# Zhijian-Mei/py-debruijn

Hardware: AMD Instinct MI355X
Metric: k-mers/s hashed+graph-built at k=31 (higher is better)
Workload: dtype u64; 1 GPU; 10000000 x 150 bp synthetic reads (10000000 per GPU): BASELINE.json configs[1]; k=31, 30x coverage of a 50000000 bp uniform genome, 1% substitutions, seed 1; k=31, reads_per_gpu=10000000, reads_total=10000000, read_len=150, parallelism=single table

## Files before the change

### py-debruijn_amd/_dbg.py

```python
from __future__ import annotations

import ctypes as C
import os

import numpy as np

_HERE = os.path.dirname(os.path.abspath(__file__))
LIB_PATH = os.environ.get("DBG_LIB") or os.path.join(_HERE, "libdbg_hip.so")

DBG_OK, DBG_E_ARG, DBG_E_HIP, DBG_E_ALPHABET, DBG_E_CAPACITY, DBG_E_NOMEM = 0, -1, -2, -3, -4, -5
F_INDEG, F_KEEP_MASK, F_KEEP_SHIFT, F_BRANCH, F_PULLED = 0x01, 0x1E, 1, 0x20, 0x40
NO_NODE = 0xFFFFFFFF
ABI_VERSION = 6

SYMBOLS = (
    "dbg_create", "dbg_destroy", "dbg_last_error", "dbg_abi_version", "dbg_set_option", "dbg_set_reads", "dbg_set_reads_fasta",
    "dbg_set_reads_fasta_file", "dbg_fasta_ingest_stats", "dbg_set_reads_device",
    "dbg_synth_reads", "dbg_reads_checksum", "dbg_copy_reads", "dbg_reads_device", "dbg_build", "dbg_refine_edge_order", "dbg_export_orders",
    "dbg_get_alphabet", "dbg_export_keepmask", "dbg_export_dict_order",
    "dbg_prune", "dbg_remove_tips",
    "dbg_mark_pull_reads", "dbg_walk", "dbg_get_sizes", "dbg_get_stats", "dbg_get_counter", "dbg_export_nodes", "dbg_export_keys_hi",
    "dbg_export_succ",
    "dbg_export_csr", "dbg_export_pull_ranks", "dbg_export_pull_reads", "dbg_export_contigs",
    "dbg_export_contig_index", "dbg_export_contig_text", "dbg_device_views", "dbg_shard_extract", "dbg_shard_bucket_counts", "dbg_shard_record_layout", "dbg_shard_build", "dbg_shard_answer", "dbg_shard_apply",
    "dbg_import_graph", "dbg_device_keys_hi",
    "dbg_support_read_scores", "dbg_export_sorted_fasta", "dbg_build_multipass", "dbg_part_count", "dbg_part_sizes", "dbg_export_part", "dbg_part_device_views",
    "dbg_shard_build_multipass", "dbg_shard_build_multipass_from", "dbg_shard_extract_part", "dbg_part_queries", "dbg_part_answer", "dbg_part_apply", "dbg_multipass_finish",
    "dbg_export_marked", "dbg_part_keys_hi", "dbg_take_reads",
    "dbg_part_prune", "dbg_part_select", "dbg_part_gather", "dbg_part_mark", "dbg_part_clear", "dbg_part_cross_targets",
    "dbg_part_segments", "dbg_part_pflags", "dbg_scan_reads_for_keys", "dbg_set_orders", "dbg_part_segment_text",
    "dbg_build_from_walk", "dbg_build_from_walks",
    "dbg_lookup_nodes", "dbg_lookup_nodes_device", "dbg_gather_nodes", "dbg_score_sequences",
    "dbg_part_lookup_nodes", "dbg_part_lookup_nodes_device", "dbg_part_score_sequences",
    "dbg_export_contig_texts", "dbg_write_contigs_fasta", "dbg_contig_output_stats",
    "dbg_part_set_skeleton", "dbg_part_contig_window", "dbg_part_export_contig_texts", "dbg_part_write_contigs_fasta",
)


class Sizes(C.Structure):
    _fields_ = [("k", C.c_int32), ("abi_version", C.c_int32)] + [
        (n, C.c_uint64) for n in (
            "n_reads", "n_bytes", "n_kmer_instances", "n_edge_instances", "table_capacity", "n_nodes", "n_edges",
            "n_branch", "n_pulled", "n_pull_reads", "n_starts", "n_contigs", "contig_chars", "tip_rounds",
            "contigs_materialised", "max_degree")]

    def as_dict(self):
        return {n: getattr(self, n) for n, _ in self._fields_}


class Stats(C.Structure):
    _fields_ = [(n, C.c_double) for n in (
        "ms_startbits", "ms_table_init", "ms_count", "ms_compact", "ms_succ", "ms_csr", "ms_build_total", "ms_prune",
        "ms_tips", "ms_pull_reads", "ms_walk", "ms_h2d", "ms_extract", "ms_partition")] + [
        (n, C.c_uint64) for n in ("count_launches", "n_records", "n_buckets", "n_queries")]

    def as_dict(self):
        return {n: getattr(self, n) for n, _ in self._fields_}


class IngestStats(C.Structure):
    _fields_ = [(n, C.c_uint64) for n in (
        "bytes_read", "chunks", "chunk_bytes", "peak_device_bytes", "n_reads", "n_bases")] + [
        (n, C.c_double) for n in ("ms_total", "ms_io_wait", "ms_h2d", "ms_parse")]

    def as_dict(self):
        return {n: getattr(self, n) for n, _ in self._fields_}


class ContigOutStats(C.Structure):
    _fields_ = [(n, C.c_uint64) for n in (
        "bytes_written", "chunks", "chunk_bytes", "peak_device_bytes", "lift_bytes")] + [
        (n, C.c_double) for n in ("ms_total", "ms_io_wait", "ms_fill", "ms_d2h")]

    def as_dict(self):
        return {n: getattr(self, n) for n, _ in self._fields_}


class WalkBlock(C.Structure):
    _fields_ = [("src", C.c_void_p), ("contigs", C.c_void_p), ("n", C.c_uint64)]


COUNTERS = ("extract_presplit_fallbacks", "extract_presplit_rehists", "resolve_direct_hits", "resolve_keyed",
            "refine_crowded", "pull_crowded", "lookup_index_builds", "lookup_dir_calls", "lookup_index_calls",
            "part_lookup_calls")


class DbgError(RuntimeError):
    def __init__(self, code, msg):
        super().__init__(f"dbg error {code}: {msg}")
        self.code = code


class AlphabetError(DbgError, ValueError):
    pass


_lib = None


def load_library():
    global _lib
    if _lib is not None:
        return _lib
    if not os.path.exists(LIB_PATH):
        raise OSError(f"{LIB_PATH} not found: build it with py-debruijn_amd/csrc/build.sh "
                      f"(there is no CPU fallback for the device path)")
    try:
        import torch
    except ImportError:
        pass
    lib = C.CDLL(LIB_PATH)
    H = C.c_void_p
    u64p, u32p, u8p = C.POINTER(C.c_uint64), C.POINTER(C.c_uint32), C.POINTER(C.c_uint8)
    vp = C.c_void_p
    sig = {
        "dbg_create": (C.c_int, [C.c_int, C.POINTER(H)]),
        "dbg_destroy": (None, [H]),
        "dbg_last_error": (C.c_char_p, [H]),
        "dbg_abi_version": (C.c_int, []),
        "dbg_set_option": (C.c_int, [H, C.c_char_p, C.c_int64]),
        "dbg_set_reads": (C.c_int, [H, vp, vp, C.c_uint64]),
        "dbg_set_reads_fasta": (C.c_int, [H, vp, C.c_uint64]),
        "dbg_set_reads_fasta_file": (C.c_int, [H, C.c_char_p, C.c_uint64, C.c_uint64, C.c_uint64]),
        "dbg_fasta_ingest_stats": (C.c_int, [H, C.POINTER(IngestStats)]),
        "dbg_set_reads_device": (C.c_int, [H, vp, C.c_uint64, vp, C.c_uint64]),
        "dbg_synth_reads": (C.c_int, [H, C.c_uint64, C.c_uint64, C.c_uint64, C.c_uint64, C.c_uint32, C.c_uint32]),
        "dbg_reads_checksum": (C.c_int, [H, u64p]),
        "dbg_copy_reads": (C.c_int, [H, vp, vp]),
        "dbg_build": (C.c_int, [H, C.c_int, C.c_uint64]),
        "dbg_refine_edge_order": (C.c_int, [H]),
        "dbg_export_orders": (C.c_int, [H, vp, vp]),
        "dbg_get_alphabet": (C.c_int, [H, vp, C.POINTER(C.c_int), C.POINTER(C.c_int)]),
        "dbg_export_keepmask": (C.c_int, [H, vp]),
        "dbg_prune": (C.c_int, [H, C.c_double]),
        "dbg_remove_tips": (C.c_int, [H]),
        "dbg_mark_pull_reads": (C.c_int, [H]),
        "dbg_walk": (C.c_int, [H, C.c_int, C.c_uint64]),
        "dbg_get_sizes": (C.c_int, [H, C.POINTER(Sizes)]),
        "dbg_get_stats": (C.c_int, [H, C.POINTER(Stats)]),
        "dbg_get_counter": (C.c_int, [H, C.c_char_p, C.POINTER(C.c_uint64)]),
        "dbg_export_nodes": (C.c_int, [H, vp, vp, vp, vp]),
        "dbg_export_keys_hi": (C.c_int, [H, vp]),
        "dbg_export_dict_order": (C.c_int, [H, vp]),
        "dbg_export_succ": (C.c_int, [H, vp]),
        "dbg_export_csr": (C.c_int, [H, vp, vp, vp]),
        "dbg_export_pull_ranks": (C.c_int, [H, vp]),
        "dbg_export_pull_reads": (C.c_int, [H, vp]),
        "dbg_export_contigs": (C.c_int, [H, vp, vp, vp, vp, vp]),
        "dbg_export_contig_index": (C.c_int, [H, vp, vp, vp, vp]),
        "dbg_export_contig_text": (C.c_int, [H, C.c_uint64, vp, C.c_uint64]),
        "dbg_device_views": (C.c_int, [H] + [C.POINTER(vp)] * 5),
        "dbg_shard_extract": (C.c_int, [H, C.c_int, C.c_int, u64p, C.POINTER(vp), C.POINTER(vp), C.POINTER(vp)]),
        "dbg_shard_bucket_counts": (C.c_int, [H, u64p]),
        "dbg_shard_record_layout": (C.c_int, [H, C.POINTER(C.c_int), C.POINTER(C.c_int)]),
        "dbg_shard_build": (C.c_int, [H, C.c_int, C.c_int, C.c_int, vp, vp, vp, u64p, u64p, u64p, u64p, C.POINTER(vp), u64p, C.c_int]),
        "dbg_shard_answer": (C.c_int, [H, vp, C.c_uint64, vp]),
        "dbg_build_multipass": (C.c_int, [H, C.c_int, C.c_int]),
        "dbg_export_sorted_fasta": (C.c_int, [H, vp, vp, C.c_uint64, u64p]),
        "dbg_support_read_scores": (C.c_int, [H, vp, vp, C.c_uint64, vp, vp, vp, vp, C.c_uint64, vp, vp]),
        "dbg_part_count": (C.c_int, [H, C.POINTER(C.c_int)]),
        "dbg_shard_build_multipass": (C.c_int, [H, C.c_int, C.c_int, C.c_int, C.c_int, vp, vp, vp, C.c_int, u64p, u64p, u64p]),
        "dbg_shard_build_multipass_from": (C.c_int, [H, C.c_int, C.c_int, C.c_int, C.c_int, C.c_int, vp, vp, vp, C.c_int, u64p, u64p, u64p]),
        "dbg_shard_extract_part": (C.c_int, [H, C.c_int, C.c_int, C.c_int, C.c_int, u64p, C.POINTER(C.c_void_p), C.POINTER(C.c_void_p), C.POINTER(C.c_void_p)]),
        "dbg_part_queries": (C.c_int, [H, C.c_int, u64p, u64p, C.POINTER(vp)]),
        "dbg_part_answer": (C.c_int, [H, C.c_int, vp, C.c_uint64, vp]),
        "dbg_part_apply": (C.c_int, [H, C.c_int, C.c_int, vp]),
        "dbg_multipass_finish": (C.c_int, [H]),
# ... 825 lines not shown
```

### py-debruijn_amd/csrc/dbg_hip.hip

```cpp
#include <hip/hip_runtime.h>

#include <algorithm>
#include <chrono>
#include <cstdlib>
#include <cstdio>
#include <cstring>
#include <string>
#include <vector>

#include <cerrno>
#include <fcntl.h>
#include <sys/stat.h>
#include <unistd.h>

#include <rocprim/device/device_radix_sort.hpp>

#include "../../include/dbg.h"
#include "dbg_device.h"
#include "dbg_sk.h"
#include "dbg_sk2.h"
#include "dbg_sk3.h"
#include "dbg_wsk2.h"
#include "dbg_generic.h"
#include "dbg_genref.h"
#include "dbg_wide.h"
#include "dbg_support.h"
#include "dbg_wsk.h"
#include "dbg_fasta.h"
#include "dbg_lookup.h"
#include "dbg_ctgout.h"

using namespace dbgk;

enum MiscSlot {
    MISC_SEGMENTS,
    MISC_L1_CHILDREN,
    MISC_MS_SCPRE,
    MISC_MS_CMAT,
    MISC_MS_OFFS,
    MISC_BUCKETS,
    MISC_RANGES,
    MISC_QUERY_SEGS,
    MISC_ESTIMATE_SET,
    MISC_SLOTS
};

#ifndef DBG_L1_WIDE_FROM
#define DBG_L1_WIDE_FROM 20
#endif
#ifndef DBG_PS_WG_PER_CU
#define DBG_PS_WG_PER_CU DBG_EXW_WAVES
#endif
#ifndef DBG_EXTRACT_PRESPLIT
#define DBG_EXTRACT_PRESPLIT 4
#endif

struct dbg {
    int device = 0;
    hipStream_t stream = nullptr;
    std::string err;

    char *d_bases = nullptr;
    bool own_bases = false;
    uint64_t n_bytes = 0;
    uint64_t *d_offsets = nullptr;
    bool own_offsets = false;
    uint64_t n_reads = 0;
    uint32_t *d_startbits = nullptr;
    uint64_t startbits_words = 0;

    int k = 0;
    Slot *d_tab = nullptr;
    uint64_t cap = 0;
    int cap_log2 = 0;
    uint32_t *d_occ = nullptr;
    uint64_t *d_scalars = nullptr;
    uint64_t n_kmer_inst = 0, n_edge_inst = 0;
    uint64_t n_nodes = 0, n_edges = 0;
    uint64_t *d_keys = nullptr, *d_stamps = nullptr;
    uint64_t *d_keys_hi = nullptr;
    uint32_t *d_cnt = nullptr;
    uint8_t *d_flags = nullptr;
    uint8_t *d_order = nullptr;
    uint8_t *d_deg = nullptr;
    uint8_t *d_fsorder = nullptr;
    bool order_exact = false;
    uint32_t *d_succ = nullptr;
    bool nodes_in_arena = false;
    bool csr_built = false;
    uint64_t *d_rowptr = nullptr;
    uint32_t *d_col = nullptr, *d_ecnt = nullptr;
    bool dense_pending = false;
    uint32_t *d_rowptr32 = nullptr;
    void *d_stamps_st = nullptr;
    int stamps_st_bytes = 0;

    bool pruned = false, tipped = false;
    uint64_t n_branch = 0, n_pulled = 0, tip_rounds = 0;
    uint64_t *d_pull_rank = nullptr;

    uint8_t *d_read_flags = nullptr;
    uint64_t n_pull_reads = 0;
    bool pull_reads_done = false;

    uint64_t n_starts = 0, n_contigs = 0, contig_chars = 0;
    bool starts_known = false;
    struct { const uint64_t *w0 = nullptr, *w1 = nullptr; const void *st = nullptr; int st_bytes = 0;
             const uint64_t *b_start = nullptr, *b_cnt = nullptr; bool valid = false; } sk_src;
    uint64_t *d_ctg_off = nullptr;
    char *d_ctg_chars = nullptr;
    uint64_t *d_ctg_score = nullptr, *d_ctg_stamp = nullptr;
    uint32_t *d_ctg_seq = nullptr;
    uint32_t *d_ctg_start = nullptr;
    uint32_t *d_lift = nullptr;
    int lift_levels = 0;
    bool walked = false;
    bool walk_final = false;
    bool walk_indexed = false;
    bool walk_sizes_only = false;
    uint64_t walk_jump_min = 1ull << 14;

    int D = 4, sym_bits = 2, n_sym = 0;
    bool alpha_known = false, is_dna = true;
    uint8_t alphabet[32] = {0};
    uint8_t *d_lut = nullptr;
    char *d_alpha = nullptr;
    uint32_t *d_keepmask = nullptr;
    uint8_t *d_rank_mc = nullptr, *d_rank_fs = nullptr;

    int engine = 0;
    int bucket_bits = 0;
    int lds_slots = 4096;
    int phase_limit = 0;
    int est_scale_pct = 100;
    int wide_engine = 1;
    int count_kernel_u64 = 3;
    int stamp64 = 0;
    int resolve_sorted = 0;
    int resolve_direct = 1;
    int resolve_count = 0;
    uint64_t resolve_direct_hits = 0, resolve_keyed = 0;
    int wcount_kernel = 2;
    int count_kernel = 2;

    struct Buf {
        void *p = nullptr;
        uint64_t bytes = 0;
    };
    Buf ar_rec[2][3], ar_q[2][3], ar_node[8], ar_misc[MISC_SLOTS], ar_csr[4], ar_dir, ar_l2, ar_scan, ar_shard[6], ar_walk[3], ar_wide[6], ar_refine[4], ar_tips[4], ar_part[4][3] ;
    int sk_T = 0, sk_l1 = 0, sk_l2 = 0, sk_nb2 = 0 , sk_cap = 0;
    bool refine_streaming = false;
    int target_distinct = 0;
    int shard_stamp64 = 0;
    int extract_generic = 0;
    int extract_presplit = DBG_EXTRACT_PRESPLIT;
    uint64_t presplit_rehists = 0;
    uint64_t presplit_fallbacks = 0;
    uint64_t refine_crowded = 0, pull_crowded = 0;
    uint64_t sk_n_ranges = 0, sk_n_buckets = 0;
    SkGeom sk_geom{};
    void *shard_state = nullptr;
    void *multipass = nullptr;
    bool dropping_parts = false;
    dbg *spare_part = nullptr;
    bool wide_owner = false;
    bool borrowed_stream = false;
    bool arena_freed = false;
    std::vector<uint64_t> host_seg_cnt;
    std::vector<uint64_t> host_scpre;
    uint64_t shard_node_limit = 0;
    bool partial_graph = false;
    uint64_t *d_btab = nullptr;
    uint64_t btab_cap = 0;
    struct NkBlock {
        uint64_t n_src = 0, n_reads = 0;
        uint32_t *next = nullptr, *z = nullptr, *start = nullptr;
    };
    bool nk_graph = false;
    uint64_t nk_reads = 0, nk_bytes = 0;
    std::vector<NkBlock> nk_blocks;
    uint8_t *d_nk_read_flags = nullptr;

    bool dir_valid = false;
    int lookup_index = 0;
    Buf ar_lookup[3];
    bool lookup_built = false;
    uint64_t lookup_index_builds = 0, lookup_dir_calls = 0, lookup_index_calls = 0;
    bool part_dir_ok = false;
    uint64_t part_lookup_calls = 0;

    dbg_stats_t stats{};
    dbg_ingest_stats_t ingest{};
    dbg_contig_out_stats_t ctgout{};
    uint64_t ctgout_chunk = 0;
};

struct ShardState {
    int n_shards = 0, my_shard = 0, shard_bits = 0, k = 0;
    std::vector<uint64_t> q_start, q_cnt;
    uint64_t n_remote = 0;
    uint64_t n_kmer_inst_local = 0;
    std::vector<uint64_t> l1_counts;
    int rec_words = 1, rec_stamp_bytes = 4;
};
static ShardState &shard_of(dbg *h);
static void multipass_free(dbg *h);
static void drop_spare_part(dbg *h);

static int buf_ensure(dbg *h, dbg::Buf &b, uint64_t bytes) {
    if (bytes == 0) bytes = 16;
    if (b.bytes >= bytes) return DBG_OK;
    if (b.p) { (void)hipFreeAsync(b.p, h->stream); h->arena_freed = true; }
    b.p = nullptr;
    b.bytes = 0;
    static const bool trace = getenv("DBG_TRACE_ALLOC") != nullptr;
    const auto t_alloc = std::chrono::steady_clock::now();
    hipError_t e = hipMallocAsync(&b.p, bytes, h->stream);
    if (trace) {
        const double ms = std::chrono::duration<double, std::milli>(std::chrono::steady_clock::now() - t_alloc).count();
        if (ms > 5.0) fprintf(stderr, "[dbg] hipMallocAsync(%.3f GB) took %.1f ms (buffer %p of handle %p)\n", bytes / 1e9, ms, (void *)&b, (void *)h);
    }
    if (e != hipSuccess) {
        (void)hipGetLastError();
        (void)hipStreamSynchronize(h->stream);
        hipMemPool_t pool;
        if (hipDeviceGetDefaultMemPool(&pool, h->device) == hipSuccess) (void)hipMemPoolTrimTo(pool, 0);
        e = hipMallocAsync(&b.p, bytes, h->stream);
    }
    if (e != hipSuccess) {
        (void)hipGetLastError();
        h->err = std::string("hipMallocAsync(") + std::to_string(bytes) + "): " + hipGetErrorString(e);
        b.p = nullptr;
        return DBG_E_NOMEM;
    }
    b.bytes = bytes;
    return DBG_OK;
}
static void buf_free(dbg *h, dbg::Buf &b) {
    if (b.p) { (void)hipFreeAsync(b.p, h->stream); h->arena_freed = true; }
    b.p = nullptr;
    b.bytes = 0;
}
static void pool_trim(dbg *h) {
    if (!h->arena_freed) return;
    (void)hipStreamSynchronize(h->stream);
    hipMemPool_t pool;
    if (hipDeviceGetDefaultMemPool(&pool, h->device) == hipSuccess) (void)hipMemPoolTrimTo(pool, 0);
    (void)hipGetLastError();
    h->arena_freed = false;
}

#define HIPCHK(h, call)                                                                      \
    do {                                                                                     \
        hipError_t e_ = (call);                                                              \
        if (e_ != hipSuccess) {                                                              \
            (h)->err = std::string(#call) + ": " + hipGetErrorString(e_);                    \
            return e_ == hipErrorOutOfMemory ? DBG_E_NOMEM : DBG_E_HIP;                      \
        }                                                                                    \
    } while (0)

#define CHK(expr)                 \
    do {                          \
        int rc_ = (expr);         \
        if (rc_ != DBG_OK) return rc_; \
    } while (0)

template <class T>
static int dev_alloc(dbg *h, T **p, uint64_t count) {
    *p = nullptr;
    if (count == 0) count = 1;
    HIPCHK(h, hipMalloc((void **)p, count * sizeof(T)));
    return DBG_OK;
}
template <class T>
static void dev_free(T *&p) {
    if (p) (void)hipFree(p);
    p = nullptr;
}

static inline unsigned grid_for(uint64_t n, unsigned block) { return (unsigned)((n + block - 1) / block); }

struct Timer {
    hipEvent_t a = nullptr, b = nullptr;
    hipStream_t s;
    explicit Timer(hipStream_t st) : s(st) {
        (void)hipEventCreate(&a);
        (void)hipEventCreate(&b);
        (void)hipEventRecord(a, s);
    }
    double stop() {
        (void)hipEventRecord(b, s);
        (void)hipEventSynchronize(b);
        float ms = 0;
        (void)hipEventElapsedTime(&ms, a, b);
        return ms;
    }
    ~Timer() {
        (void)hipEventDestroy(a);
        (void)hipEventDestroy(b);
    }
};

constexpr int SCAN_ITEMS = 16;
constexpr int SCAN_TILE = 256 * SCAN_ITEMS;

template <class F>
__global__ __launch_bounds__(256) void k_scan_reduce(uint64_t n, F f, uint64_t *partial) {
    uint64_t base = (uint64_t)blockIdx.x * SCAN_TILE + (uint64_t)threadIdx.x * SCAN_ITEMS;
    uint64_t s = 0;
#pragma unroll
    for (int i = 0; i < SCAN_ITEMS; ++i)
        if (base + i < n) s += f(base + i);
    uint64_t tot;
    (void)block_exscan_256(s, &tot);
    if (threadIdx.x == 0) partial[blockIdx.x] = tot;
}

__global__ __launch_bounds__(256) void k_scan_partials(uint64_t *partial, uint64_t nblk, uint64_t *total) {
    uint64_t carry = 0;
    for (uint64_t base = 0; base < nblk; base += 256) {
        uint64_t i = base + threadIdx.x;
        uint64_t v = i < nblk ? partial[i] : 0;
        uint64_t tot;
        uint64_t ex = block_exscan_256(v, &tot);
        if (i < nblk) partial[i] = carry + ex;
        carry += tot;
    }
    if (threadIdx.x == 0) *total = carry;
}

template <class F, class OutT>
__global__ __launch_bounds__(256) void k_scan_write(uint64_t n, F f, const uint64_t *partial, OutT *out) {
    uint64_t base = (uint64_t)blockIdx.x * SCAN_TILE + (uint64_t)threadIdx.x * SCAN_ITEMS;
    uint64_t v[SCAN_ITEMS];
    uint64_t s = 0;
#pragma unroll
    for (int i = 0; i < SCAN_ITEMS; ++i) {
        v[i] = (base + i < n) ? f(base + i) : 0;
        s += v[i];
    }
    uint64_t tot;
    uint64_t run = partial[blockIdx.x] + block_exscan_256(s, &tot);
#pragma unroll
    for (int i = 0; i < SCAN_ITEMS; ++i) {
        if (base + i < n) out[base + i] = (OutT)run;
        run += v[i];
    }
}

template <class F, class OutT>
static int exclusive_scan(dbg *h, uint64_t n, F f, OutT *out, uint64_t *h_total) {
    uint64_t nblk = (n + SCAN_TILE - 1) / SCAN_TILE;
    if (nblk == 0) nblk = 1;
    CHK(buf_ensure(h, h->ar_scan, (nblk + 1) * 8));
    uint64_t *partial = (uint64_t *)h->ar_scan.p;
    uint64_t *d_total = partial + nblk;
    hipLaunchKernelGGL(HIP_KERNEL_NAME(k_scan_reduce<F>), dim3((unsigned)nblk), dim3(256), 0, h->stream, n, f, partial);
    hipLaunchKernelGGL(k_scan_partials, dim3(1), dim3(256), 0, h->stream, partial, nblk, d_total);
    hipLaunchKernelGGL(HIP_KERNEL_NAME(k_scan_write<F, OutT>), dim3((unsigned)nblk), dim3(256), 0, h->stream, n, f,
                       partial, out);
    if (!h_total) return DBG_OK;
    hipError_t e = hipMemcpyAsync(h_total, d_total, 8, hipMemcpyDeviceToHost, h->stream);
    if (e == hipSuccess) e = hipStreamSynchronize(h->stream);
    if (e != hipSuccess) {
        h->err = std::string("exclusive_scan: ") + hipGetErrorString(e);
        return DBG_E_HIP;
    }
    return DBG_OK;
}

template <class F>
static int reduce_sum(dbg *h, uint64_t n, F f, uint64_t *h_total) {
    uint64_t nblk = (n + SCAN_TILE - 1) / SCAN_TILE;
    if (nblk == 0) nblk = 1;
    CHK(buf_ensure(h, h->ar_scan, (nblk + 1) * 8));
    uint64_t *partial = (uint64_t *)h->ar_scan.p;
    hipLaunchKernelGGL(HIP_KERNEL_NAME(k_scan_reduce<F>), dim3((unsigned)nblk), dim3(256), 0, h->stream, n, f, partial);
    hipLaunchKernelGGL(k_scan_partials, dim3(1), dim3(256), 0, h->stream, partial, nblk, partial + nblk);
    hipError_t e = hipMemcpyAsync(h_total, partial + nblk, 8, hipMemcpyDeviceToHost, h->stream);
    if (e == hipSuccess) e = hipStreamSynchronize(h->stream);
    if (e != hipSuccess) {
        h->err = std::string("reduce_sum: ") + hipGetErrorString(e);
        return DBG_E_HIP;
    }
    return DBG_OK;
}

struct OccBytes32 {
    const uint8_t *occ;
    __device__ uint64_t operator()(uint64_t w) const {
        const uint4 a = reinterpret_cast<const uint4 *>(occ)[2 * w], b = reinterpret_cast<const uint4 *>(occ)[2 * w + 1];
        return __popc(a.x) + __popc(a.y) + __popc(a.z) + __popc(a.w) + __popc(b.x) + __popc(b.y) + __popc(b.z) + __popc(b.w);
    }
};
struct PopcWords {
    const uint32_t *w;
    __device__ uint64_t operator()(uint64_t i) const { return __popc(w[i]); }
};
struct DegOf {
    const uint8_t *deg;
    __device__ uint64_t operator()(uint64_t i) const { return deg[i]; }
};
struct U64At {
    const uint64_t *p;
    __device__ uint64_t operator()(uint64_t i) const { return p[i]; }
};
struct KmerInstances {
    const uint64_t *off;
    uint64_t k;
    __device__ uint64_t operator()(uint64_t i) const { const uint64_t len = off[i + 1] - off[i]; return len >= k ? len - k + 1 : 0; }
};
struct WRecLenAt {
    const uint64_t *w1;
    __device__ uint64_t operator()(uint64_t i) const { return (uint64_t)wrec_len(w1[i]); }
};
struct WRecSuccAt {
    const uint64_t *w1;
    __device__ uint64_t operator()(uint64_t i) const { return (uint64_t)wrec_has_succ(w1[i]); }
};
struct FlagSet {
    const uint8_t *f;
    uint8_t mask, want;
    __device__ uint64_t operator()(uint64_t i) const { return (f[i] & mask) == want; }
};

__device__ inline uint64_t synth_draw(uint64_t key, uint64_t ctr) { return mix64(key ^ (ctr * 0xD6E8FEB86659FD93ull)); }

__global__ __launch_bounds__(256) void k_synth(char *bases, uint64_t *offsets, uint64_t kg, uint64_t ks, uint64_t ke,
                                               uint64_t genome_len, uint64_t first_read, uint64_t n_reads,
                                               uint32_t read_len, uint32_t err_thr) {
    const uint64_t total = n_reads * read_len;
    for (uint64_t i = (uint64_t)blockIdx.x * blockDim.x + threadIdx.x; i < total; i += (uint64_t)gridDim.x * blockDim.x) {
        const uint64_t r = i / read_len, j = i - r * read_len, gr = first_read + r;
        const uint64_t start = synth_draw(ks, gr) % (genome_len - read_len + 1);
        uint32_t code = (uint32_t)(synth_draw(kg, start + j) & 3);
        if (err_thr) {
            const uint64_t e = synth_draw(ke, gr * read_len + j);
            if ((uint32_t)(e & 0xFFFFFFu) < err_thr) code = (code + 1 + (uint32_t)((e >> 24) % 3)) & 3;
        }
        bases[i] = "ACGT"[code];
        if (j == 0) offsets[r] = i;
    }
    if (blockIdx.x == 0 && threadIdx.x == 0) offsets[n_reads] = total;
}
// ... 1008 lines not shown
    h->d_rowptr32 = nullptr; h->d_stamps_st = nullptr; h->stamps_st_bytes = 0;
    h->dense_pending = false;
    h->csr_built = false;
    h->d_pull_rank = nullptr;
    dev_free(h->d_read_flags);
    dev_free(h->d_ctg_off); dev_free(h->d_ctg_chars); dev_free(h->d_ctg_score); dev_free(h->d_ctg_stamp);
    dev_free(h->d_ctg_seq); dev_free(h->d_ctg_start); dev_free(h->d_lift);
    h->lift_levels = 0;
    h->partial_graph = false;
    h->sk_src.valid = false;
    h->k = 0; h->cap = 0; h->n_nodes = h->n_edges = 0;
    h->pruned = h->tipped = h->pull_reads_done = h->walked = h->walk_indexed = h->walk_sizes_only = false;
    h->n_branch = h->n_pulled = h->tip_rounds = h->n_pull_reads = 0;
    h->n_starts = h->n_contigs = h->contig_chars = 0;
    h->starts_known = false;
    h->n_kmer_inst = h->n_edge_inst = 0;
    for (auto &b : h->nk_blocks) { dev_free(b.next); dev_free(b.z); dev_free(b.start); }
    h->nk_blocks.clear();
    dev_free(h->d_nk_read_flags);
    h->nk_graph = false;
    h->nk_reads = h->nk_bytes = 0;
}

static void free_reads(dbg *h) {
    if (h->own_bases) dev_free(h->d_bases);
    if (h->own_offsets) dev_free(h->d_offsets);
    h->d_bases = nullptr; h->d_offsets = nullptr;
    h->own_bases = h->own_offsets = false;
    dev_free(h->d_startbits);
    dev_free(h->d_lut); dev_free(h->d_alpha);
    h->alpha_known = false;
    h->n_bytes = h->n_reads = 0;
}

extern "C" int dbg_abi_version(void) { return DBG_ABI_VERSION; }

extern "C" int dbg_create(int device, dbg_t **out) {
    if (!out) return DBG_E_ARG;
    *out = nullptr;
    int n = 0;
    if (hipGetDeviceCount(&n) != hipSuccess || device < 0 || device >= n) return DBG_E_HIP;
    dbg *h = new (std::nothrow) dbg();
    if (!h) return DBG_E_NOMEM;
    h->device = device;
    if (hipSetDevice(device) != hipSuccess || hipStreamCreate(&h->stream) != hipSuccess ||
        hipMalloc((void **)&h->d_scalars, 128 * sizeof(uint64_t)) != hipSuccess) {
        delete h;
        return DBG_E_HIP;
    }
    {
        hipMemPool_t pool;
        if (hipDeviceGetDefaultMemPool(&pool, device) == hipSuccess) {
            uint64_t keep = ~0ull;
            (void)hipMemPoolSetAttribute(pool, hipMemPoolAttrReleaseThreshold, &keep);
        }
        (void)hipGetLastError();
    }
    *out = h;
    return DBG_OK;
}

extern "C" void dbg_destroy(dbg_t *h) {
    if (!h) return;
    (void)hipSetDevice(h->device);
    (void)hipStreamSynchronize(h->stream);
    h->dropping_parts = true;
    free_build(h);
    if (h->spare_part) { dbg_destroy(h->spare_part); h->spare_part = nullptr; }
    free_reads(h);
    for (auto &lvl : h->ar_rec) for (auto &b : lvl) buf_free(h, b);
    for (auto &lvl : h->ar_q) for (auto &b : lvl) buf_free(h, b);
    for (auto &b : h->ar_node) buf_free(h, b);
    for (auto &b : h->ar_misc) buf_free(h, b);
    for (auto &b : h->ar_csr) buf_free(h, b);
    buf_free(h, h->ar_dir);
    buf_free(h, h->ar_l2);
    for (auto &b : h->ar_shard) buf_free(h, b);
    for (auto &b : h->ar_walk) buf_free(h, b);
    for (auto &b : h->ar_wide) buf_free(h, b);
    for (auto &b : h->ar_refine) buf_free(h, b);
    for (auto &b : h->ar_tips) buf_free(h, b);
    for (auto &lvl : h->ar_part) for (auto &b : lvl) buf_free(h, b);
    buf_free(h, h->ar_scan);
    dev_free(h->d_scalars);
    delete (ShardState *)h->shard_state;
    (void)hipStreamSynchronize(h->stream);
    if (!h->borrowed_stream) (void)hipStreamDestroy(h->stream);
    delete h;
}

extern "C" const char *dbg_last_error(const dbg_t *h) { return h ? h->err.c_str() : "null handle"; }

static int make_startbits(dbg *h) {
    Timer t(h->stream);
    dev_free(h->d_startbits);
    h->startbits_words = (h->n_bytes + 1 + 31) / 32 + SB_WORDS + 2;
    CHK(dev_alloc(h, &h->d_startbits, h->startbits_words));
    HIPCHK(h, hipMemsetAsync(h->d_startbits, 0, h->startbits_words * 4, h->stream));
    hipLaunchKernelGGL(k_startbits, dim3(grid_for(h->n_reads + 1, 256)), dim3(256), 0, h->stream, h->d_offsets,
                       h->n_reads, h->d_startbits);
    HIPCHK(h, hipGetLastError());
    h->stats.ms_startbits = t.stop();
    return DBG_OK;
}

extern "C" int dbg_set_reads(dbg_t *h, const char *bases, const uint64_t *offsets, uint64_t n_reads) {
    if (!h || !offsets || (n_reads && !bases && offsets[n_reads] != 0)) return DBG_E_ARG;
    HIPCHK(h, hipSetDevice(h->device));
    if (offsets[0] != 0) { h->err = "offsets[0] must be 0"; return DBG_E_ARG; }
    for (uint64_t i = 0; i < n_reads; ++i)
        if (offsets[i + 1] < offsets[i]) { h->err = "offsets must be non-decreasing"; return DBG_E_ARG; }
    free_build(h);
    free_reads(h);
    const uint64_t nb = offsets[n_reads];
    Timer t(h->stream);
    CHK(dev_alloc(h, &h->d_bases, nb + 64));
    h->own_bases = true;
    CHK(dev_alloc(h, &h->d_offsets, n_reads + 1));
    h->own_offsets = true;
    if (nb) HIPCHK(h, hipMemcpyAsync(h->d_bases, bases, nb, hipMemcpyHostToDevice, h->stream));
    HIPCHK(h, hipMemcpyAsync(h->d_offsets, offsets, (n_reads + 1) * 8, hipMemcpyHostToDevice, h->stream));
    h->stats.ms_h2d = t.stop();
    h->n_bytes = nb;
    h->n_reads = n_reads;
    return make_startbits(h);
}

extern "C" int dbg_set_reads_fasta(dbg_t *h, const char *text, uint64_t n_text) {
    if (!h || (n_text && !text)) return DBG_E_ARG;
    HIPCHK(h, hipSetDevice(h->device));
    free_build(h);
    free_reads(h);
    char *d_text = nullptr;
    uint32_t *bits = nullptr, *word_rank = nullptr, *len = nullptr;
    uint64_t *line_start = nullptr, *read_idx = nullptr, *byte_off = nullptr;
    uint8_t *is_read = nullptr;
    auto cleanup = [&]() {
        dev_free(d_text); dev_free(bits); dev_free(word_rank); dev_free(len); dev_free(line_start); dev_free(read_idx);
        dev_free(byte_off); dev_free(is_read);
    };
    int rc = DBG_OK;
    uint64_t n_lines = 0, n_reads = 0, n_bases = 0;
    do {
        Timer t(h->stream);
        if ((rc = dev_alloc(h, &d_text, n_text + 64)) != DBG_OK) break;
        if (n_text && hipMemcpyAsync(d_text, text, n_text, hipMemcpyHostToDevice, h->stream) != hipSuccess) { h->err = "H2D copy failed"; rc = DBG_E_HIP; break; }
        h->stats.ms_h2d = t.stop();
        const uint64_t n_words = (n_text + 31) / 32;
        if ((rc = dev_alloc(h, &bits, n_words)) != DBG_OK) break;
        if ((rc = dev_alloc(h, &word_rank, n_words)) != DBG_OK) break;
        if (n_words) {
            hipLaunchKernelGGL(k_fa_mark, dim3(grid_for(n_words, 256)), dim3(256), 0, h->stream, d_text, n_text, bits);
            if ((rc = exclusive_scan(h, n_words, PopcWords{bits}, word_rank, &n_lines)) != DBG_OK) break;
        }
        if ((rc = dev_alloc(h, &line_start, n_lines)) != DBG_OK) break;
        if ((rc = dev_alloc(h, &is_read, n_lines)) != DBG_OK) break;
        if ((rc = dev_alloc(h, &len, n_lines)) != DBG_OK) break;
        if ((rc = dev_alloc(h, &read_idx, n_lines)) != DBG_OK) break;
        if ((rc = dev_alloc(h, &byte_off, n_lines)) != DBG_OK) break;
        if (n_lines) {
            hipLaunchKernelGGL(k_fa_line_starts, dim3(grid_for(n_words, 256)), dim3(256), 0, h->stream, bits, word_rank, n_words,
                               line_start);
            hipLaunchKernelGGL(k_fa_lines, dim3(grid_for(n_lines, 256)), dim3(256), 0, h->stream, d_text, n_text, line_start,
                               n_lines, is_read, len);
            if ((rc = exclusive_scan(h, n_lines, ByteSet{is_read}, read_idx, &n_reads)) != DBG_OK) break;
            if ((rc = exclusive_scan(h, n_lines, U32At{len}, byte_off, &n_bases)) != DBG_OK) break;
        }
        if ((rc = dev_alloc(h, &h->d_bases, n_bases + 64)) != DBG_OK) break;
        h->own_bases = true;
// ... 601 lines not shown
    unsigned long long *estamp = nullptr;
    auto cleanup = [&]() { dev_free(nodes); dev_free(edges); dev_free(occ); dev_free(eocc); dev_free(word_rank); dev_free(estamp); };
    int rc = DBG_OK;
    do {
        if ((rc = dev_alloc(h, &nodes, cap)) != DBG_OK) break;
        if ((rc = dev_alloc(h, &edges, cap)) != DBG_OK) break;
        if ((rc = dev_alloc(h, &occ, cap / 32)) != DBG_OK) break;
        if ((rc = dev_alloc(h, &eocc, cap / 32)) != DBG_OK) break;
        (void)hipMemsetAsync(occ, 0, cap / 8, h->stream);
        (void)hipMemsetAsync(eocc, 0, cap / 8, h->stream);
        (void)hipMemsetAsync(h->d_scalars, 0, 64 * 8, h->stream);
        hipLaunchKernelGGL(k_g_init_tables, dim3(grid_for(cap, 256)), dim3(256), 0, h->stream, nodes, edges, cap);
        if (h->n_bytes) {
            const unsigned grid = (unsigned)std::min<uint64_t>((h->n_bytes + 255) / 256, 1u << 16);
            hipLaunchKernelGGL(k_g_insert, dim3(grid), dim3(256), 0, h->stream, h->d_bases, h->n_bytes, h->d_startbits, k,
                               h->d_lut, nodes, occ, edges, eocc, cap - 1, (unsigned long long *)h->d_scalars);
        }
        uint64_t sc[4] = {0, 0, 0, 0};
        if (hipMemcpyAsync(sc, h->d_scalars, 32, hipMemcpyDeviceToHost, h->stream) != hipSuccess ||
            hipStreamSynchronize(h->stream) != hipSuccess) { h->err = "generic count failed"; rc = DBG_E_HIP; break; }
        if (sc[0] & STATUS_TABLE_FULL) { h->err = "generic engine: hash table full"; rc = DBG_E_CAPACITY; break; }
        h->n_kmer_inst = sc[1];
        h->n_edge_inst = sc[2];
        h->stats.ms_count = t_count.stop();
        h->stats.count_launches = 1;
        Timer t_c(h->stream);
        const uint64_t n_words = cap / 32;
        if ((rc = dev_alloc(h, &word_rank, n_words)) != DBG_OK) break;
        uint64_t n = 0;
        if ((rc = exclusive_scan(h, n_words, PopcWords{occ}, word_rank, &n)) != DBG_OK) break;
        h->n_nodes = n;
        if ((rc = dev_alloc(h, &h->d_keys, n)) != DBG_OK) break;
        if ((rc = dev_alloc(h, &h->d_stamps, n)) != DBG_OK) break;
        if ((rc = dev_alloc(h, &h->d_flags, n)) != DBG_OK) break;
        if ((rc = dev_alloc(h, &h->d_cnt, n * GEN_D)) != DBG_OK) break;
        if ((rc = dev_alloc(h, &h->d_succ, n * GEN_D)) != DBG_OK) break;
        if ((rc = dev_alloc(h, &h->d_deg, n)) != DBG_OK) break;
        if ((rc = dev_alloc(h, &h->d_keepmask, n)) != DBG_OK) break;
        if ((rc = dev_alloc(h, &h->d_rank_mc, n * GEN_D)) != DBG_OK) break;
        if ((rc = dev_alloc(h, &h->d_rank_fs, n * GEN_D)) != DBG_OK) break;
        if ((rc = dev_alloc(h, &estamp, n * GEN_D)) != DBG_OK) break;
        if (n) {
            (void)hipMemsetAsync(h->d_cnt, 0, n * GEN_D * 4, h->stream);
            (void)hipMemsetAsync(h->d_succ, 0xFF, n * GEN_D * 4, h->stream);
            (void)hipMemsetAsync(estamp, 0xFF, n * GEN_D * 8, h->stream);
            (void)hipMemsetAsync(h->d_keepmask, 0, n * 4, h->stream);
            hipLaunchKernelGGL(k_g_gather, dim3(grid_for(n_words, 256)), dim3(256), 0, h->stream, nodes, occ, word_rank, n_words,
                               h->d_keys, h->d_stamps, h->d_flags);
            hipLaunchKernelGGL(k_g_edges, dim3(grid_for(cap, 256)), dim3(256), 0, h->stream, edges, cap, nodes, cap - 1, k,
                               h->d_cnt, h->d_succ, estamp, (unsigned long long *)h->d_scalars);
            hipLaunchKernelGGL(k_g_rank, dim3(grid_for(n, 256)), dim3(256), 0, h->stream, n, h->d_cnt, estamp, h->d_rank_mc,
                               h->d_rank_fs, h->d_deg);
        }
        if (hipMemcpyAsync(sc, h->d_scalars, 8, hipMemcpyDeviceToHost, h->stream) != hipSuccess ||
            hipStreamSynchronize(h->stream) != hipSuccess) { h->err = "generic graph assembly failed"; rc = DBG_E_HIP; break; }
        if (sc[0] & STATUS_SUCC_MISSING) { h->err = "internal: edge endpoint missing from the node table"; rc = DBG_E_HIP; break; }
        h->stats.ms_succ = t_c.stop();
        h->order_exact = true;
    } while (0);
    cleanup();
    return rc;
}

extern "C" int dbg_set_option(dbg_t *h, const char *name, int64_t value) {
    if (!h || !name) return DBG_E_ARG;
    const std::string n(name);
    if (n == "engine" && (value == 0 || value == 1)) { h->engine = (int)value; return DBG_OK; }
    if (n == "bucket_bits" && value >= 0 && value <= SK_BUCKET_BITS) { h->bucket_bits = (int)value; return DBG_OK; }
    if (n == "lds_slots" && (value == 2048 || value == 4096)) { h->lds_slots = (int)value; return DBG_OK; }
    if (n == "phase_limit" && value >= 0 && value <= 5) { h->phase_limit = (int)value; return DBG_OK; }
    if (n == "estimate_scale_pct" && value >= 1 && value <= 1000) { h->est_scale_pct = (int)value; return DBG_OK; }
    if (n == "target_distinct" && value >= 0 && value <= 4096) { h->target_distinct = (int)value; return DBG_OK; }
    if (n == "shard_stamp64" && (value == 0 || value == 1)) { h->shard_stamp64 = (int)value; return DBG_OK; }
    if (n == "extract_generic" && (value == 0 || value == 1)) { h->extract_generic = (int)value; return DBG_OK; }
    if (n == "extract_presplit" && value >= 0 && value <= SK_PS_MAX_F0) { h->extract_presplit = (int)value; return DBG_OK; }
    if (n == "refine_streaming" && (value == 0 || value == 1)) { h->refine_streaming = value != 0; return DBG_OK; }
    if (n == "walk_jump_min_nodes" && value >= 0) { h->walk_jump_min = (uint64_t)value; return DBG_OK; }
    if (n == "wide_engine" && (value == 0 || value == 1)) { h->wide_engine = (int)value; return DBG_OK; }
    if (n == "count_kernel" && value >= 1 && value <= 3) { h->count_kernel = (int)value; return DBG_OK; }
    if (n == "stamp64" && (value == 0 || value == 1)) { h->stamp64 = (int)value; return DBG_OK; }
    if (n == "resolve_sorted" && value >= 0 && value <= 2) { h->resolve_sorted = (int)value; return DBG_OK; }
    if (n == "resolve_direct" && (value == 0 || value == 1)) { h->resolve_direct = (int)value; return DBG_OK; }
    if (n == "resolve_count" && (value == 0 || value == 1)) { h->resolve_count = (int)value; return DBG_OK; }
    if (n == "wcount_kernel" && (value == 1 || value == 2)) { h->wcount_kernel = (int)value; return DBG_OK; }
    if (n == "count_kernel_u64" && value >= 1 && value <= 3) { h->count_kernel_u64 = (int)value; return DBG_OK; }
    if (n == "lookup_index" && (value == 0 || value == 1)) { h->lookup_index = (int)value; return DBG_OK; }
    if (n == "ctgout_chunk_bytes" && value >= 0 && dbgk::co_chunk_ok((uint64_t)value)) { h->ctgout_chunk = (uint64_t)value; return DBG_OK; }
    if (n == "shard_node_limit" && value >= 0 && value < (1ll << 29)) { h->shard_node_limit = (uint64_t)value; return DBG_OK; }
    h->err = "unknown option or value out of range: " + n;
    return DBG_E_ARG;
}

static int build_wide_once(dbg *h, int k, uint64_t table_capacity_hint, bool packed, bool *overflow) {
    if (h->n_bytes >= (1ull << 43)) { h->err = "reads too large for the 44-bit positions of the table's protocol word"; return DBG_E_CAPACITY; }
    uint64_t want = table_capacity_hint;
    if (!want) {
        uint64_t inst = 0;
        CHK(reduce_sum(h, h->n_reads, KmerInstances{h->d_offsets, (uint64_t)k}, &inst));
        want = (uint64_t)((double)(inst + 1) / 0.7);
    }
    const uint64_t cap = std::max<uint64_t>(1024, (want + 1023) / 1024 * 1024);
    const uint64_t pk_words = (h->n_bytes + 31) / 32, n_occ = cap / 32;
    uint64_t *pk = nullptr;
    WSlot *tab = nullptr;
    uint32_t *tcnt = nullptr, *word_rank = nullptr;
    uint8_t *occ = nullptr;
    auto cleanup = [&]() {};
    int rc = DBG_OK;
    uint64_t sc[4] = {0, 0, 0, 0};
    do {
        Timer t(h->stream);
        if ((rc = buf_ensure(h, h->ar_wide[0], (pk_words + 3) * 8)) != DBG_OK) break;
        if ((rc = buf_ensure(h, h->ar_wide[1], cap * sizeof(WSlot))) != DBG_OK) break;
        if (!packed && (rc = buf_ensure(h, h->ar_wide[2], cap * 16)) != DBG_OK) break;
        if ((rc = buf_ensure(h, h->ar_wide[3], cap)) != DBG_OK) break;
        if ((rc = buf_ensure(h, h->ar_wide[4], n_occ * 4)) != DBG_OK) break;
        pk = (uint64_t *)h->ar_wide[0].p;
        tab = (WSlot *)h->ar_wide[1].p;
        tcnt = packed ? nullptr : (uint32_t *)h->ar_wide[2].p;
        occ = (uint8_t *)h->ar_wide[3].p;
        word_rank = (uint32_t *)h->ar_wide[4].p;
        (void)hipMemsetAsync(pk + pk_words, 0, 3 * 8, h->stream);
        hipLaunchKernelGGL(k_wtab_init, dim3(grid_for(cap, 256)), dim3(256), 0, h->stream, tab, cap);
        if (tcnt) (void)hipMemsetAsync(tcnt, 0, cap * 16, h->stream);
        (void)hipMemsetAsync(occ, 0, cap, h->stream);
        (void)hipMemsetAsync(h->d_scalars, 0, 64 * 8, h->stream);
        if (pk_words)
            hipLaunchKernelGGL(k_wpack, dim3(grid_for(pk_words, 256)), dim3(256), 0, h->stream, h->d_bases, h->n_bytes,
                               pk_words, pk);
        h->stats.ms_table_init = t.stop();
        Timer tc(h->stream);
        const uint64_t tiles = (h->n_bytes + TILE - 1) / TILE;
        if (tiles)
            hipLaunchKernelGGL(k_wcount, dim3((unsigned)tiles), dim3(256), 0, h->stream, h->d_bases, h->n_bytes,
                               h->d_startbits, k, pk, tab, tcnt, cap, occ, (unsigned long long *)h->d_scalars);
        h->stats.count_launches = tiles ? 1 : 0;
        hipError_t e = hipMemcpyAsync(sc, h->d_scalars, 32, hipMemcpyDeviceToHost, h->stream);
        h->stats.ms_count = tc.stop();
        if (e != hipSuccess || hipGetLastError() != hipSuccess) { h->err = "k_wcount failed"; rc = DBG_E_HIP; break; }
        if (sc[0] & STATUS_BAD_BASE) { h->err = "reads hold a byte outside ACGT"; rc = DBG_E_ALPHABET; break; }
        if (sc[0] & STATUS_TABLE_FULL) { h->err = "hash table capacity exceeded"; rc = DBG_E_CAPACITY; break; }
        if (sc[0] & STATUS_WIDE_COUNTER16) { *overflow = true; rc = DBG_E_CAPACITY; h->err = "successor counter overflow"; break; }
        h->n_kmer_inst = sc[1];
        h->n_edge_inst = sc[2];

        Timer tg(h->stream);
        uint64_t total = 0;
        if ((rc = exclusive_scan(h, n_occ, OccBytes32{occ}, word_rank, &total)) != DBG_OK) break;
        if (total >= 0xFFFFFFFFull) { h->err = "more than 2^32-1 nodes"; rc = DBG_E_CAPACITY; break; }
        h->n_nodes = total;
        if ((rc = buf_ensure(h, h->ar_node[0], total * 8)) != DBG_OK) break;
        if ((rc = buf_ensure(h, h->ar_node[1], total * 8)) != DBG_OK) break;
        if ((rc = buf_ensure(h, h->ar_node[2], total * 16)) != DBG_OK) break;
        if ((rc = buf_ensure(h, h->ar_node[3], total)) != DBG_OK) break;
        if ((rc = buf_ensure(h, h->ar_node[4], total)) != DBG_OK) break;
        if ((rc = buf_ensure(h, h->ar_node[5], total * 16)) != DBG_OK) break;
        if ((rc = buf_ensure(h, h->ar_node[6], total)) != DBG_OK) break;
        if ((rc = buf_ensure(h, h->ar_wide[5], total * 8)) != DBG_OK) break;
        h->d_keys = (uint64_t *)h->ar_node[0].p;
        h->d_stamps = (uint64_t *)h->ar_node[1].p;
        h->d_cnt = (uint32_t *)h->ar_node[2].p;
        h->d_flags = (uint8_t *)h->ar_node[3].p;
        h->d_order = (uint8_t *)h->ar_node[4].p;
        h->d_succ = (uint32_t *)h->ar_node[5].p;
        h->d_deg = (uint8_t *)h->ar_node[6].p;
        h->d_keys_hi = (uint64_t *)h->ar_wide[5].p;
        h->nodes_in_arena = true;
        hipLaunchKernelGGL(k_wgather, dim3(grid_for(n_occ * 32, 256)), dim3(256), 0, h->stream, tab, tcnt, occ, word_rank, n_occ,
                           h->d_keys, h->d_keys_hi, h->d_stamps, h->d_cnt, h->d_flags, 1);
        h->stats.ms_compact = tg.stop();
        Timer ts(h->stream);
        if (total)
            hipLaunchKernelGGL(k_wsucc, dim3(grid_for(total, 256)), dim3(256), 0, h->stream, tab, cap, k, total,
                               h->d_keys, h->d_keys_hi, h->d_cnt, h->d_succ, h->d_order, h->d_deg);
        e = hipStreamSynchronize(h->stream);
        h->stats.ms_succ = ts.stop();
        if (e != hipSuccess || hipGetLastError() != hipSuccess) { h->err = std::string("wide build: ") + hipGetErrorString(e); rc = DBG_E_HIP; break; }
    } while (false);
    cleanup();
    return rc;
}

static int build_wide(dbg *h, int k, uint64_t table_capacity_hint) {
    bool overflow = false;
    int rc = build_wide_once(h, k, table_capacity_hint, true, &overflow);
    if (rc != DBG_OK && overflow) {
        rc = build_wide_once(h, k, table_capacity_hint, false, &overflow);
        if (rc == DBG_OK) h->err.clear();
    }
    return rc;
}

extern "C" int dbg_build(dbg_t *h, int k, uint64_t table_capacity_hint) {
    if (!h) return DBG_E_ARG;
    if (k < 1 || k > 63) { h->err = "k must be in 1..63 (k-mers of at most two 64-bit words)"; return DBG_E_ARG; }
    if (!h->d_offsets) { h->err = "no reads set"; return DBG_E_ARG; }
    HIPCHK(h, hipSetDevice(h->device));
    h->dropping_parts = true;
    free_build(h);
    h->dropping_parts = false;
    drop_spare_part(h);
    h->k = k;
    h->stats = dbg_stats_t{};
    const bool tentative = !h->alpha_known && h->engine == 0 && h->n_bytes > 0;
    if (tentative) h->is_dna = true;
    else CHK(compute_alphabet(h));
    if (tentative) {
        Timer t_total(h->stream);
        int rc;
        bool lds_engine = true;
        if (k > 31) {
            bool fallback = true;
            rc = h->wide_engine == 1 ? build_wsk(h, k, &fallback) : DBG_E_CAPACITY;
            if (fallback && rc != DBG_E_ALPHABET) {
                lds_engine = false;
                free_build(h);
                h->k = k;
                h->stats = dbg_stats_t{};
                CHK(compute_alphabet(h));
                rc = h->is_dna ? build_wide(h, k, table_capacity_hint) : DBG_E_ALPHABET;
            }
        } else {
            rc = build_sk(h, k, table_capacity_hint);
        }
        if (rc == DBG_OK) {
            rc = finish_graph(h);
            if (rc != DBG_OK) { const std::string keep = h->err; free_build(h); h->err = keep; return rc; }
            h->alpha_known = true;
            h->is_dna = true;
            h->dir_valid = lds_engine;
            h->stats.ms_build_total = t_total.stop();
            if (k <= 31) pool_trim(h);
            return DBG_OK;
        }
        if (rc != DBG_E_ALPHABET) { const std::string keep = h->err; free_build(h); h->err = keep; return rc; }
        free_build(h);
        h->k = k;
        h->stats = dbg_stats_t{};
        h->err.clear();
        CHK(compute_alphabet(h));
        if (h->is_dna) { h->err = "internal: the extraction refused reads the alphabet scan calls ACGT"; return DBG_E_HIP; }
    }
    if (!h->is_dna) {
        Timer t_total(h->stream);
        int rc = build_generic(h, k);
        if (rc == DBG_OK) rc = finish_graph(h);
        if (rc != DBG_OK) { const std::string keep = h->err; free_build(h); h->err = keep; return rc; }
        h->stats.ms_build_total = t_total.stop();
        return DBG_OK;
    }
    if (k > 31) {
        Timer t_total(h->stream);
        int rc;
        bool fallback = true;
        if (h->wide_engine == 1 && h->engine == 0) rc = build_wsk(h, k, &fallback);
        if (fallback) {
            free_build(h);
            h->k = k;
            h->stats = dbg_stats_t{};
            rc = build_wide(h, k, table_capacity_hint);
        }
        if (rc == DBG_OK) rc = finish_graph(h);
        if (rc != DBG_OK) { const std::string keep = h->err; free_build(h); h->err = keep; return rc; }
        h->dir_valid = !fallback;
        h->stats.ms_build_total = t_total.stop();
        return DBG_OK;
    }
    if (h->engine == 0) {
        Timer t_total(h->stream);
        int rc = build_sk(h, k, table_capacity_hint);
        if (rc == DBG_OK) rc = finish_graph(h);
        if (rc != DBG_OK) { const std::string keep = h->err; free_build(h); h->err = keep; return rc; }
        h->dir_valid = true;
        h->stats.ms_build_total = t_total.stop();
        pool_trim(h);
        return DBG_OK;
    }
    Timer t_total(h->stream);

    uint64_t want = table_capacity_hint ? table_capacity_hint : (uint64_t)((double)(h->n_bytes + 1) / 0.7);
    uint64_t cap = 1024;
    int lg = 10;
    while (cap < want) { cap <<= 1; ++lg; }
    h->cap = cap;
    h->cap_log2 = lg;
    {
        Timer t(h->stream);
        CHK(dev_alloc(h, &h->d_tab, cap));
        CHK(dev_alloc(h, &h->d_occ, cap / 32));
        HIPCHK(h, hipMemsetAsync(h->d_occ, 0, cap / 8, h->stream));
        HIPCHK(h, hipMemsetAsync(h->d_scalars, 0, 64 * 8, h->stream));
        hipLaunchKernelGGL(k_table_init, dim3(grid_for(cap, 256)), dim3(256), 0, h->stream, h->d_tab, cap);
        HIPCHK(h, hipGetLastError());
        h->stats.ms_table_init = t.stop();
    }
    uint64_t sc[4] = {0, 0, 0, 0};
    {
        Timer t(h->stream);
        const uint64_t tiles = (h->n_bytes + TILE - 1) / TILE;
        if (tiles) {
            hipLaunchKernelGGL(k_count, dim3((unsigned)tiles), dim3(256), 0, h->stream, h->d_bases, h->n_bytes,
                               h->d_startbits, k, h->d_tab, cap - 1, 64 - lg, h->d_occ,
                               (unsigned long long *)h->d_scalars);
            HIPCHK(h, hipGetLastError());
        }
        h->stats.count_launches = tiles ? 1 : 0;
        HIPCHK(h, hipMemcpyAsync(sc, h->d_scalars, 32, hipMemcpyDeviceToHost, h->stream));
        h->stats.ms_count = t.stop();
    }
    if (sc[0] & STATUS_BAD_BASE) { h->err = "reads hold a byte outside ACGT"; free_build(h); return DBG_E_ALPHABET; }
    if (sc[0] & STATUS_TABLE_FULL) { h->err = "hash table capacity exceeded"; free_build(h); return DBG_E_CAPACITY; }
    h->n_kmer_inst = sc[1];
    h->n_edge_inst = sc[2];

    {
        Timer t(h->stream);
        uint32_t *word_rank = nullptr;
        const uint64_t n_words = cap / 32;
        CHK(dev_alloc(h, &word_rank, n_words));
        uint64_t total = 0;
        int rc = exclusive_scan(h, n_words, PopcWords{h->d_occ}, word_rank, &total);
        if (rc != DBG_OK) { (void)hipFree(word_rank); return rc; }
        if (total >= 0xFFFFFFFFull) { (void)hipFree(word_rank); h->err = "more than 2^32-1 nodes"; return DBG_E_CAPACITY; }
        h->n_nodes = total;
        CHK(dev_alloc(h, &h->d_keys, total));
        CHK(dev_alloc(h, &h->d_stamps, total));
        CHK(dev_alloc(h, &h->d_cnt, total * 4));
        CHK(dev_alloc(h, &h->d_flags, total));
        CHK(dev_alloc(h, &h->d_order, total));
        CHK(dev_alloc(h, &h->d_succ, total * 4));
        CHK(dev_alloc(h, &h->d_deg, total));
        hipLaunchKernelGGL(k_gather, dim3(grid_for(n_words, 256)), dim3(256), 0, h->stream, h->d_tab, h->d_occ,
                           word_rank, n_words, h->d_keys, h->d_stamps, h->d_cnt, h->d_flags);
        HIPCHK(h, hipGetLastError());
        h->stats.ms_compact = t.stop();
        (void)hipFree(word_rank);
    }
    {
        Timer t(h->stream);
        if (h->n_nodes) {
            hipLaunchKernelGGL(k_succ, dim3(grid_for(h->n_nodes, 256)), dim3(256), 0, h->stream, h->d_tab, cap - 1,
                               64 - lg, k, h->n_nodes, h->d_keys, h->d_cnt, h->d_succ, h->d_order, h->d_deg);
            HIPCHK(h, hipGetLastError());
        }
        h->stats.ms_succ = t.stop();
    }
    CHK(finish_graph(h));
    h->stats.ms_build_total = t_total.stop();
    return DBG_OK;
}

extern "C" int dbg_refine_edge_order(dbg_t *h) {
    if (!h || !h->k) return DBG_E_ARG;
    if (h->partial_graph) { h->err = kPartialGraph; return DBG_E_ARG; }
    HIPCHK(h, hipSetDevice(h->device));
    CHK(ensure_dense(h));
    if (h->D == GEN_D) return DBG_OK;
// ... 539 lines not shown
            h->walk_indexed = true;
            if (n_chr > max_chars) break;
            const uint64_t longest = h->n_nodes + (uint64_t)h->k;
            int levels = 1;
            while ((1ull << levels) <= longest) ++levels;
            if (n_ctg && (uint64_t)levels * h->n_nodes * 4 <= (8ull << 30)) {
                if ((rc = dev_alloc(h, &h->d_ctg_chars, n_chr)) != DBG_OK) break;
                if ((rc = dev_alloc(h, &lift, (uint64_t)levels * h->n_nodes)) != DBG_OK) break;
                const dim3 ngrid(grid_for(h->n_nodes, 256));
                hipLaunchKernelGGL(HIP_KERNEL_NAME(k_lift_init<G>), ngrid, dim3(256), 0, h->stream, h->n_nodes, g, lift);
                for (int l = 1; l < levels; ++l)
                    hipLaunchKernelGGL(k_lift_step, ngrid, dim3(256), 0, h->stream, h->n_nodes, lift + (uint64_t)(l - 1) * h->n_nodes,
                                       lift + (uint64_t)l * h->n_nodes);
                hipLaunchKernelGGL(HIP_KERNEL_NAME(k_text_fill<G>), dim3(grid_for(n_chr, 256)), dim3(256), 0, h->stream, n_chr, g,
                                   h->d_ctg_off, n_ctg, ctg_start, lift, h->n_nodes, levels, h->d_ctg_chars);
                text_done = true;
            }
        }
        if (!text_done) {
            if ((rc = dev_alloc(h, &h->d_ctg_chars, n_chr)) != DBG_OK) break;
            launch(1);
        }
        if (hipGetLastError() != hipSuccess) { h->err = "walk pass 1 launch failed"; rc = DBG_E_HIP; break; }
        hipError_t e = hipStreamSynchronize(h->stream);
        if (e != hipSuccess) { h->err = std::string("walk: ") + hipGetErrorString(e); rc = DBG_E_HIP; break; }
        h->walked = true;
        h->walk_indexed = true;
    } while (0);
    cleanup();
    h->stats.ms_walk = t.stop();
    return rc;
}

extern "C" int dbg_walk(dbg_t *h, int final_mode, uint64_t max_chars) {
    if (!h || !h->pruned) { if (h) h->err = "dbg_prune must run first"; return DBG_E_ARG; }
    HIPCHK(h, hipSetDevice(h->device));
    if (h->D == GEN_D) return walk_impl(h, gen_view(h), final_mode, max_chars);
    return walk_impl(h, dna_view(h), final_mode, max_chars);
}

extern "C" int dbg_get_sizes(dbg_t *h, dbg_sizes_t *o) {
    if (!h || !o) return DBG_E_ARG;
    if (h->k && h->n_nodes && !h->starts_known) {
        HIPCHK(h, hipSetDevice(h->device));
        CHK(ensure_starts(h));
    }
    memset(o, 0, sizeof(*o));
    o->k = h->k;
    o->abi_version = DBG_ABI_VERSION;
    o->n_reads = h->n_reads + h->nk_reads;
    o->n_bytes = h->n_bytes + h->nk_bytes;
    o->n_kmer_instances = h->n_kmer_inst;
    o->n_edge_instances = h->n_edge_inst;
    o->table_capacity = h->cap;
    o->n_nodes = h->n_nodes;
    o->n_edges = h->n_edges;
    o->n_branch = h->n_branch;
    o->n_pulled = h->n_pulled;
    o->n_pull_reads = h->n_pull_reads;
    o->n_starts = h->n_starts;
    o->n_contigs = h->n_contigs;
    o->contig_chars = h->contig_chars;
    o->tip_rounds = h->tip_rounds;
    o->contigs_materialised = h->walked ? 1 : 0;
    o->max_degree = (uint64_t)h->D;
    return DBG_OK;
}

extern "C" int dbg_get_stats(dbg_t *h, dbg_stats_t *o) {
    if (!h || !o) return DBG_E_ARG;
    *o = h->stats;
    return DBG_OK;
}

extern "C" int dbg_get_counter(dbg_t *h, const char *name, uint64_t *out) {
    if (!h || !name || !out) return DBG_E_ARG;
    const std::string n(name);
    if (n == "extract_presplit_rehists") { *out = h->presplit_rehists; return DBG_OK; }
    if (n == "extract_presplit_fallbacks") { *out = h->presplit_fallbacks; return DBG_OK; }
    if (n == "refine_crowded") { *out = h->refine_crowded; return DBG_OK; }
    if (n == "pull_crowded") { *out = h->pull_crowded; return DBG_OK; }
    if (n == "resolve_direct_hits") { *out = h->resolve_direct_hits; return DBG_OK; }
    if (n == "resolve_keyed") { *out = h->resolve_keyed; return DBG_OK; }
    if (n == "lookup_index_builds") { *out = h->lookup_index_builds; return DBG_OK; }
    if (n == "lookup_dir_calls") { *out = h->lookup_dir_calls; return DBG_OK; }
    if (n == "lookup_index_calls") { *out = h->lookup_index_calls; return DBG_OK; }
    if (n == "part_lookup_calls") { *out = h->part_lookup_calls; return DBG_OK; }
    h->err = "unknown counter: " + n;
    return DBG_E_ARG;
}

#define D2H(h, dst, src, bytes)                                                                       do {                                                                                                  if ((dst) && (bytes)) HIPCHK(h, hipMemcpyAsync((dst), (src), (bytes), hipMemcpyDeviceToHost, (h)->stream));     } while (0)

extern "C" int dbg_export_nodes(dbg_t *h, uint64_t *keys, uint64_t *stamps, uint32_t *counts, uint8_t *flags) {
    if (!h || !h->k) return DBG_E_ARG;
    HIPCHK(h, hipSetDevice(h->device));
    CHK(ensure_dense(h));
    if (keys && !h->d_keys) memset(keys, 0, h->n_nodes * 8);
    else D2H(h, keys, h->d_keys, h->n_nodes * 8);
    D2H(h, stamps, h->d_stamps, h->n_nodes * 8);
    D2H(h, counts, h->d_cnt, h->n_nodes * 4 * h->D);
    D2H(h, flags, h->d_flags, h->n_nodes);
    HIPCHK(h, hipStreamSynchronize(h->stream));
    return DBG_OK;
}

extern "C" int dbg_export_keys_hi(dbg_t *h, uint64_t *keys_hi) {
    if (!h || !h->k || !keys_hi) return DBG_E_ARG;
    HIPCHK(h, hipSetDevice(h->device));
    if (!h->d_keys_hi) {
        memset(keys_hi, 0, h->n_nodes * 8);
        return DBG_OK;
    }
    D2H(h, keys_hi, h->d_keys_hi, h->n_nodes * 8);
    HIPCHK(h, hipStreamSynchronize(h->stream));
    return DBG_OK;
}

extern "C" int dbg_export_succ(dbg_t *h, uint32_t *succ) {
    if (!h || !h->k) return DBG_E_ARG;
    HIPCHK(h, hipSetDevice(h->device));
    CHK(ensure_dense(h));
    D2H(h, succ, h->d_succ, h->n_nodes * 4 * h->D);
    HIPCHK(h, hipStreamSynchronize(h->stream));
    return DBG_OK;
}

extern "C" int dbg_export_csr(dbg_t *h, uint64_t *row_ptr, uint32_t *col, uint32_t *cnt) {
    if (!h || !h->k) return DBG_E_ARG;
    HIPCHK(h, hipSetDevice(h->device));
    CHK(ensure_dense(h));
    D2H(h, row_ptr, h->d_rowptr, (h->n_nodes + 1) * 8);
    D2H(h, col, h->d_col, h->n_edges * 4);
    D2H(h, cnt, h->d_ecnt, h->n_edges * 4);
    HIPCHK(h, hipStreamSynchronize(h->stream));
    return DBG_OK;
}

extern "C" int dbg_export_pull_ranks(dbg_t *h, uint64_t *ranks) {
    if (!h || !h->tipped) { if (h) h->err = "dbg_remove_tips must run first"; return DBG_E_ARG; }
    HIPCHK(h, hipSetDevice(h->device));
    D2H(h, ranks, h->d_pull_rank, h->n_nodes * 8);
    HIPCHK(h, hipStreamSynchronize(h->stream));
    return DBG_OK;
}

extern "C" int dbg_export_pull_reads(dbg_t *h, uint8_t *read_flags) {
    if (!h || !h->pull_reads_done) { if (h) h->err = "dbg_mark_pull_reads must run first"; return DBG_E_ARG; }
    HIPCHK(h, hipSetDevice(h->device));
    if (h->nk_graph) {
        D2H(h, read_flags, h->d_nk_read_flags, h->nk_reads);
        if (read_flags) read_flags += h->nk_reads;
    }
    D2H(h, read_flags, h->d_read_flags, h->n_reads);
    HIPCHK(h, hipStreamSynchronize(h->stream));
    return DBG_OK;
}

extern "C" int dbg_export_contig_index(dbg_t *h, uint64_t *offsets, uint64_t *scores, uint64_t *start_stamp,
                                       uint32_t *seq_in_start) {
    if (!h || !h->walk_indexed) { if (h) h->err = "dbg_walk must run first"; return DBG_E_ARG; }
    HIPCHK(h, hipSetDevice(h->device));
    D2H(h, offsets, h->d_ctg_off, (h->n_contigs + 1) * 8);
    D2H(h, scores, h->d_ctg_score, h->n_contigs * 8);
    D2H(h, start_stamp, h->d_ctg_stamp, h->n_contigs * 8);
    D2H(h, seq_in_start, h->d_ctg_seq, h->n_contigs * 4);
// ... 274 lines not shown
        auto dev = [&](int i) -> void * { return outs[i].host ? (void *)(blk + outs[i].at) : nullptr; };
        LkGatherArgs a{h->d_keys, h->d_keys_hi, h->d_stamps, h->d_cnt, h->d_flags, gen ? h->d_keepmask : nullptr,
                       gen ? h->d_rank_mc : h->d_order, gen ? h->d_rank_fs : h->d_fsorder,
                       (uint64_t *)dev(0), (uint64_t *)dev(1), (uint64_t *)dev(2), (uint32_t *)dev(3), (uint8_t *)dev(5),
                       (uint32_t *)dev(4), (uint8_t *)dev(6), (uint8_t *)dev(7), h->n_nodes, h->D};
        hipLaunchKernelGGL(k_gather_nodes, dim3(grid_for(n, 256)), dim3(256), 0, h->stream, a, (const uint32_t *)(blk + 16), n,
                           (unsigned long long *)blk);
        unsigned long long bad = 0;
        e = hipGetLastError();
        if (e == hipSuccess) e = hipMemcpyAsync(&bad, blk, 8, hipMemcpyDeviceToHost, h->stream);
        if (e == hipSuccess) e = hipStreamSynchronize(h->stream);
        if (e != hipSuccess) { h->err = std::string("dbg_gather_nodes: ") + hipGetErrorString(e); rc = DBG_E_HIP; break; }
        if (bad) { h->err = "dbg_gather_nodes: a node id is not below n_nodes"; rc = DBG_E_ARG; break; }
        for (auto &o : outs)
            if (o.host && e == hipSuccess) e = hipMemcpyAsync(o.host, blk + o.at, o.bytes, hipMemcpyDeviceToHost, h->stream);
        if (e == hipSuccess) e = hipStreamSynchronize(h->stream);
        if (e != hipSuccess) { h->err = std::string("dbg_gather_nodes: ") + hipGetErrorString(e); rc = DBG_E_HIP; }
    } while (0);
    dev_free(blk);
    return rc;
}

extern "C" int dbg_score_sequences(dbg_t *h, const char *chars, const uint64_t *offsets, uint64_t n_seq, uint64_t *scores,
                                   uint64_t *first_missing) {
    if (!h) return DBG_E_ARG;
    if (!n_seq) return DBG_OK;
    if (!offsets || !scores || !first_missing) { h->err = "dbg_score_sequences: null offsets, scores or first_missing"; return DBG_E_ARG; }
    if (offsets[0] != 0) { h->err = "offsets[0] must be 0"; return DBG_E_ARG; }
    for (uint64_t i = 0; i < n_seq; ++i)
        if (offsets[i + 1] < offsets[i]) { h->err = "offsets must be non-decreasing"; return DBG_E_ARG; }
    const uint64_t n_chars = offsets[n_seq];
    if (n_chars && !chars) { h->err = "dbg_score_sequences: null chars"; return DBG_E_ARG; }
    CHK(lookup_ready(h));
    HIPCHK(h, hipSetDevice(h->device));
    CHK(ensure_dense(h));
    for (uint64_t i = 0; i < n_seq; ++i) { scores[i] = 0; first_missing[i] = ~0ull; }
    if (n_chars <= (uint64_t)h->k) return DBG_OK;
    uint8_t lut[256];
    memset(lut, LK_BAD_CODE, sizeof(lut));
    if (h->D == GEN_D) for (int c = 0; c < h->n_sym && c < 32; ++c) lut[h->alphabet[c]] = (uint8_t)c;
    else { lut['A'] = 0; lut['C'] = 1; lut['T'] = 2; lut['G'] = 3; }
    const uint64_t at_miss = n_seq * 8, at_off = at_miss + n_seq * 8, at_lut = at_off + (n_seq + 1) * 8, at_txt = at_lut + 256;
    uint8_t *blk = nullptr;
    CHK(dev_alloc(h, &blk, at_txt + n_chars));
    int rc = DBG_OK;
    do {
        hipError_t e = hipMemsetAsync(blk, 0, n_seq * 8, h->stream);
        if (e == hipSuccess) e = hipMemsetAsync(blk + at_miss, 0xFF, n_seq * 8, h->stream);
        if (e == hipSuccess) e = hipMemcpyAsync(blk + at_off, offsets, (n_seq + 1) * 8, hipMemcpyHostToDevice, h->stream);
        if (e == hipSuccess) e = hipMemcpyAsync(blk + at_lut, lut, 256, hipMemcpyHostToDevice, h->stream);
        if (e == hipSuccess) e = hipMemcpyAsync(blk + at_txt, chars, n_chars, hipMemcpyHostToDevice, h->stream);
        if (e != hipSuccess) { h->err = std::string("dbg_score_sequences: ") + hipGetErrorString(e); rc = DBG_E_HIP; break; }
        const unsigned grid = grid_for(n_chars - (uint64_t)h->k, LK_TILE);
        rc = with_finder(h, [&](auto f) -> int {
            hipLaunchKernelGGL(HIP_KERNEL_NAME(k_score_sequences<decltype(f)>), dim3(grid), dim3(LK_NT), 0, h->stream, f,
                               (const char *)(blk + at_txt), n_chars, (const uint64_t *)(blk + at_off), n_seq,
                               (const uint8_t *)(blk + at_lut), h->k, h->sym_bits, h->D, (const uint32_t *)h->d_cnt,
                               (unsigned long long *)blk, (unsigned long long *)(blk + at_miss));
            HIPCHK(h, hipGetLastError());
            return DBG_OK;
        });
        if (rc != DBG_OK) break;
        e = hipMemcpyAsync(scores, blk, n_seq * 8, hipMemcpyDeviceToHost, h->stream);
        if (e == hipSuccess) e = hipMemcpyAsync(first_missing, blk + at_miss, n_seq * 8, hipMemcpyDeviceToHost, h->stream);
        if (e == hipSuccess) e = hipStreamSynchronize(h->stream);
        if (e != hipSuccess) { h->err = std::string("dbg_score_sequences: ") + hipGetErrorString(e); rc = DBG_E_HIP; }
    } while (0);
    dev_free(blk);
    return rc;
}

struct CeilDiv {
    const uint64_t *cnt;
    uint64_t d;
    __device__ uint64_t operator()(uint64_t i) const { return (cnt[i] + d - 1) / d; }
};

template <class ST, bool HAS_ST, class STI = ST, int STHI = 0>
static int multisplit_level(dbg *h, const uint64_t *p_start, const uint64_t *p_cnt, uint32_t n_seg, uint32_t spg,
                            uint64_t total, const uint64_t *in_w0, const uint64_t *in_w1, const STI *in_st,
                            uint64_t *out_w0, uint64_t *out_w1, ST *out_st, int shift, int nb, uint64_t *c_start,
                            uint64_t *c_cnt, dbg::Buf &b_scpre, dbg::Buf &b_cmat, dbg::Buf &b_offs, int fbits = 0,
                            const uint64_t *seg_add = nullptr, unsigned long long *d_sums = nullptr,
                            const uint64_t *host_cnt = nullptr, const uint32_t *ready_cmat = nullptr) {
    CHK(buf_ensure(h, b_scpre, (uint64_t)(n_seg + 1) * 8));
    uint64_t *sc_pre = (uint64_t *)b_scpre.p;
    uint64_t nsc = 0;
    if (ready_cmat) {
        std::vector<uint64_t> &pre = h->host_scpre;
        pre.resize((size_t)n_seg + 1);
        for (uint32_t i = 0; i <= n_seg; ++i) pre[i] = i;
        nsc = n_seg;
        HIPCHK(h, hipMemcpyAsync(sc_pre, pre.data(), pre.size() * 8, hipMemcpyHostToDevice, h->stream));
    } else if (host_cnt) {
        std::vector<uint64_t> &pre = h->host_scpre;
        pre.resize((size_t)n_seg + 1);
        for (uint32_t i = 0; i < n_seg; ++i) { pre[i] = nsc; nsc += (host_cnt[i] + MS_SC - 1) / MS_SC; }
        pre[n_seg] = nsc;
        HIPCHK(h, hipMemcpyAsync(sc_pre, pre.data(), pre.size() * 8, hipMemcpyHostToDevice, h->stream));
    } else {
        CHK(exclusive_scan(h, n_seg, CeilDiv{p_cnt, (uint64_t)MS_SC}, sc_pre, &nsc));
        HIPCHK(h, hipMemcpyAsync(sc_pre + n_seg, &nsc, 8, hipMemcpyHostToDevice, h->stream));
    }
    MsParents P{p_start, p_cnt, sc_pre, n_seg, spg};
    const uint64_t n_log = nsc * (uint64_t)nb;
    if (!ready_cmat) CHK(buf_ensure(h, b_cmat, n_log * 4));
    CHK(buf_ensure(h, b_offs, n_log * 8));
    const uint32_t *cmat = ready_cmat ? ready_cmat : (const uint32_t *)b_cmat.p;
    uint64_t *offs = (uint64_t *)b_offs.p;
    if (nsc) {
        if (ready_cmat)
            ;
        else if (d_sums)
            hipLaunchKernelGGL(HIP_KERNEL_NAME(k_ms_hist<true>), dim3((unsigned)nsc), dim3(256), 0, h->stream, P, in_w1, shift, nb,
                               fbits, (uint32_t *)b_cmat.p, d_sums);
        else
            hipLaunchKernelGGL(HIP_KERNEL_NAME(k_ms_hist<false>), dim3((unsigned)nsc), dim3(256), 0, h->stream, P, in_w1, shift, nb,
                               fbits, (uint32_t *)b_cmat.p, (unsigned long long *)nullptr);
        HIPCHK(h, hipGetLastError());
        CHK(exclusive_scan(h, n_log, MsLogical{P, cmat, nb}, offs, (uint64_t *)nullptr));
    }
    const uint64_t n_child = (uint64_t)(n_seg / spg) * nb;
    hipLaunchKernelGGL(k_ms_children, dim3(grid_for(n_child, 256)), dim3(256), 0, h->stream, P, offs, nb, total, c_start,
                       c_cnt);
    if (nsc) {
        auto kern = k_ms_scatter<ST, HAS_ST, STI, STHI>;
        const size_t lds = sizeof(MsLds<ST>);
        HIPCHK(h, hipFuncSetAttribute((const void *)kern, hipFuncAttributeMaxDynamicSharedMemorySize, (int)lds));
        hipLaunchKernelGGL(kern, dim3((unsigned)nsc), dim3(MS_NT), lds, h->stream, P, in_w0, in_w1, in_st, seg_add, shift, nb,
                           fbits, offs, out_w0, out_w1, out_st);
    }
    HIPCHK(h, hipGetLastError());
    return DBG_OK;
}

static void sk_provisional_bits(const dbg *h, uint64_t n_inst, double own, double target, int shard_bits, bool presplit_senders,
                                int l1_wide_from, int *T_out, int *l1_out) {
    constexpr int T_MAX = 20;
    int T = h->bucket_bits;
    if (T == 0) {
        const double want = (double)n_inst * own * 0.4 / target;
        while (T < T_MAX && (double)(1ull << T) < want) ++T;
    }
    if (T < shard_bits) T = shard_bits;
    if (presplit_senders) T = std::max(9, T);
    *T_out = T;
    *l1_out = T < 9 ? T : (T >= l1_wide_from && !presplit_senders ? 10 : 9);
}

template <int CAP> constexpr double SK_TARGET_DISTINCT = CAP * 0.36;

struct ExtractSplit {
    double target = 0.0;
    int f0 = 0;
    uint32_t n_wg = 0;
    int l1 = 0;
    const uint32_t *cmat = nullptr;
};

template <class ST>
static int sk_extract(dbg *h, int k, uint64_t *w0[2], uint64_t *w1[2], ST *st[2], uint64_t **seg_start_out,
                      uint64_t **seg_cnt_out, uint32_t *n_seg_out, uint64_t *n_rec_out, int part = 0, int n_parts = 1,
                      ExtractSplit *xs = nullptr) {
    const int m = sk_m_for_k(k), w = k - m + 1;
    unsigned long long *sc_dev = (unsigned long long *)h->d_scalars;
    const uint64_t all_tiles = (h->n_bytes + TILE - 1) / TILE;
    const uint64_t tile_first = all_tiles * (uint64_t)part / (uint64_t)n_parts;
    const uint64_t tiles = all_tiles * (uint64_t)(part + 1) / (uint64_t)n_parts - tile_first;
    uint64_t sc[8] = {0};
    uint32_t n_wg = (uint32_t)std::min<uint64_t>(std::max<uint64_t>(tiles, 1), 2048);
    uint64_t tiles_per_wg = (tiles + n_wg - 1) / n_wg;
    const double density = std::min(1.0, 2.6 / (double)(w + 1) + 1.3 * (double)(h->n_reads + 1) / (double)(h->n_bytes + 1) + 0.01);
    uint64_t seg_cap = (w == 1) ? tiles_per_wg * TILE : (uint64_t)((double)(tiles_per_wg * TILE) * density) + 256;
    int f0 = (xs && n_parts == 1 && tiles && m == SK_MAX_M && w <= 19 && !h->extract_generic) ? h->extract_presplit : 0;
    constexpr double PS_SLACK = 1.5;
    const uint32_t n_wg_plain = n_wg;
    const uint64_t seg_cap_plain = seg_cap;
    uint64_t n_seg = n_wg;
    int ps_l1 = 0;
    if (f0) {
        const uint64_t F0 = 1ull << f0;
        const double per_tile = (w == 1 ? 1.0 : density) * TILE * PS_SLACK / (double)F0;
        const uint64_t tpw_max = std::max<uint64_t>(1, (uint64_t)((double)(MS_SC - 64) / per_tile));
        int n_cu = 0;
        HIPCHK(h, hipDeviceGetAttribute(&n_cu, hipDeviceAttributeMultiprocessorCount, h->device));
        n_wg = (uint32_t)std::max<uint64_t>(std::min<uint64_t>(tiles, (uint64_t)n_cu * DBG_PS_WG_PER_CU), (tiles + tpw_max - 1) / tpw_max);
        tiles_per_wg = (tiles + n_wg - 1) / n_wg;
        seg_cap = std::min<uint64_t>(MS_SC, (uint64_t)((double)tiles_per_wg * per_tile) + 64);
        n_seg = (uint64_t)n_wg * F0;
        const uint64_t cut = h->n_reads * (uint64_t)(k - 1);
        int T_guess = 0;
        sk_provisional_bits(h, h->n_bytes > cut ? h->n_bytes - cut : 0, 1.0, xs->target, 0, false, DBG_L1_WIDE_FROM, &T_guess, &ps_l1);
        if (ps_l1 < f0) ps_l1 = 0;
    }
    std::vector<uint64_t> hseg;
    uint64_t *seg_start = nullptr, *seg_cnt = nullptr, *seg_nk = nullptr, *seg_ne = nullptr;
    uint32_t *ps_cmat = nullptr;
    uint64_t n_rec = 0;
    Timer t(h->stream);
    for (int attempt = 0; attempt < 3; ++attempt) {
        CHK(buf_ensure(h, h->ar_misc[MISC_SEGMENTS], (n_seg * 2 + (uint64_t)n_wg * 2) * 8));
        seg_start = (uint64_t *)h->ar_misc[MISC_SEGMENTS].p; seg_cnt = seg_start + n_seg; seg_nk = seg_cnt + n_seg; seg_ne = seg_nk + n_wg;
        hseg.assign((size_t)(n_seg * 2 + (uint64_t)n_wg * 2), 0);
        if (f0 && ps_l1) {
            CHK(buf_ensure(h, h->ar_misc[MISC_MS_CMAT], n_seg * 4 << (ps_l1 - f0)));
            ps_cmat = (uint32_t *)h->ar_misc[MISC_MS_CMAT].p;
        }
        const uint64_t rec_cap = seg_cap * n_seg;
        for (int set = 0; set < 2; ++set) {
            CHK(buf_ensure(h, h->ar_rec[set][0], rec_cap * 8));
            CHK(buf_ensure(h, h->ar_rec[set][1], rec_cap * 8));
            CHK(buf_ensure(h, h->ar_rec[set][2], rec_cap * sizeof(ST)));
            w0[set] = (uint64_t *)h->ar_rec[set][0].p;
            w1[set] = (uint64_t *)h->ar_rec[set][1].p;
            st[set] = (ST *)h->ar_rec[set][2].p;
        }
        for (uint64_t g = 0; g < n_seg; ++g) hseg[g] = g * seg_cap;
        HIPCHK(h, hipMemcpyAsync(seg_start, hseg.data(), (size_t)n_seg * 8, hipMemcpyHostToDevice, h->stream));
        HIPCHK(h, hipMemsetAsync(seg_cnt, 0, (size_t)(n_seg + (uint64_t)n_wg * 2) * 8, h->stream));
        HIPCHK(h, hipMemsetAsync(h->d_scalars, 0, 64 * 8, h->stream));
        if (tiles) {
            bool launched = false;
            if (m == SK_MAX_M && !h->extract_generic) {
#define DBG_EXW_CASE(W_) case W_: \
                if (f0) hipLaunchKernelGGL(HIP_KERNEL_NAME(k_sk_extract_w<ST, W_, true>), dim3(n_wg), dim3(256), 0, h->stream, \
                                           h->d_bases, h->n_bytes, h->d_startbits, tiles, w0[0], w1[0], st[0], seg_cap, seg_cnt, \
                                           seg_nk, seg_ne, sc_dev, tile_first, f0, ps_l1, ps_l1 ? ps_cmat : (uint32_t *)nullptr); \
                else hipLaunchKernelGGL(HIP_KERNEL_NAME(k_sk_extract_w<ST, W_, false>), dim3(n_wg), dim3(256), 0, h->stream, \
                                        h->d_bases, h->n_bytes, h->d_startbits, tiles, w0[0], w1[0], st[0], seg_cap, seg_cnt, \
                                        seg_nk, seg_ne, sc_dev, tile_first, 0, 0, (uint32_t *)nullptr); \
                launched = true; break;
                switch (w) {
                    DBG_EXW_CASE(1) DBG_EXW_CASE(2) DBG_EXW_CASE(3) DBG_EXW_CASE(4) DBG_EXW_CASE(5) DBG_EXW_CASE(6) DBG_EXW_CASE(7)
                    DBG_EXW_CASE(8) DBG_EXW_CASE(9) DBG_EXW_CASE(10) DBG_EXW_CASE(11) DBG_EXW_CASE(12) DBG_EXW_CASE(13)
                    DBG_EXW_CASE(14) DBG_EXW_CASE(15) DBG_EXW_CASE(16) DBG_EXW_CASE(17) DBG_EXW_CASE(18) DBG_EXW_CASE(19)
                    default: break;
                }
#undef DBG_EXW_CASE
            }
            if (!launched)
                hipLaunchKernelGGL(HIP_KERNEL_NAME(k_sk_extract<ST>), dim3(n_wg), dim3(256), 0, h->stream, h->d_bases,
                                   h->n_bytes, h->d_startbits, k, m, tiles, w0[0], w1[0], st[0], seg_cap, seg_cnt, seg_nk,
                                   seg_ne, sc_dev, tile_first);
            HIPCHK(h, hipGetLastError());
        }
        HIPCHK(h, hipMemcpyAsync(sc, h->d_scalars, 8, hipMemcpyDeviceToHost, h->stream));
        HIPCHK(h, hipMemcpyAsync(hseg.data() + n_seg, seg_cnt, (size_t)(n_seg + (uint64_t)n_wg * 2) * 8, hipMemcpyDeviceToHost,
                                 h->stream));
        HIPCHK(h, hipStreamSynchronize(h->stream));
        if (sc[0] & STATUS_BAD_BASE) { h->err = "reads hold a byte outside ACGT"; return DBG_E_ALPHABET; }
        if (!(sc[0] & STATUS_SEGMENT_FULL)) break;
        if (f0) {
            f0 = 0; ps_l1 = 0; ps_cmat = nullptr;
            ++h->presplit_fallbacks;
            n_wg = n_wg_plain; n_seg = n_wg;
            tiles_per_wg = (tiles + n_wg - 1) / n_wg;
            seg_cap = seg_cap_plain;
            continue;
        }
        if (seg_cap == tiles_per_wg * TILE) { h->err = "super-k-mer record buffer overflow"; return DBG_E_CAPACITY; }
        seg_cap = tiles_per_wg * TILE;
    }
    h->n_kmer_inst = h->n_edge_inst = 0;
    for (uint64_t g = 0; g < n_seg; ++g) n_rec += hseg[n_seg + g];
    for (uint32_t g = 0; g < n_wg; ++g) {
        h->n_kmer_inst += hseg[2 * n_seg + g];
        h->n_edge_inst += hseg[2 * n_seg + n_wg + g];
    }
    h->stats.ms_extract = t.stop();
    h->stats.n_records = n_rec;
    h->host_seg_cnt.assign(hseg.begin() + n_seg, hseg.begin() + 2 * (size_t)n_seg);
    if (xs) { xs->f0 = f0; xs->n_wg = n_wg; xs->l1 = ps_l1; xs->cmat = ps_l1 ? ps_cmat : nullptr; }
    *seg_start_out = seg_start;
    *seg_cnt_out = seg_cnt;
    *n_seg_out = (uint32_t)n_seg;
    *n_rec_out = n_rec;
    return DBG_OK;
}


struct Presplit {
    int n_senders = 0;
    const uint64_t *counts = nullptr;
    const uint64_t *recv_off = nullptr;
    const uint64_t *stamp_add = nullptr;
    const void *in_st = nullptr;
};

template <class Est>
struct SkPartitionParams {
    double target;
    int l1_wide_from;
    bool probe_first_owned;
    bool sum_instances;
    Est estimate;
};

struct SkPartition {
    uint64_t *b_start = nullptr, *b_cnt = nullptr;
    uint64_t n_buckets = 0;
    int where = 0;
    int l1 = 0, nb2 = 1, fb2 = 0, l2_pow = 0, nb3 = 1, fb3 = 0;
    double est_distinct = 0.0;
    uint64_t n_inst = 0, n_edge_inst = 0;
};

template <class ST, class STI, int STHI, class Est>
static int sk_partition(dbg *h, const SkPartitionParams<Est> &pp, const uint64_t *seg_start, const uint64_t *seg_cnt,
                        uint32_t n_seg, const uint64_t *host_cnt, const Presplit *pre, const ExtractSplit *xs, const uint64_t *in_w0,
                        const uint64_t *in_w1, const ST *in_st, uint64_t *w0[2], uint64_t *w1[2], ST *st[2], int shard_bits,
                        int my_shard, uint64_t n_rec, uint64_t n_inst, uint64_t n_edge_inst, SkPartition *out) {
    const double own = shard_bits ? (double)(1 << shard_bits) : 1.0;
    const bool auto_T = (h->bucket_bits == 0);
    int T = 0, l1 = 0;
    sk_provisional_bits(h, n_inst, own, pp.target, shard_bits, pre != nullptr, pp.l1_wide_from, &T, &l1);
    int l2 = std::min(10, T - l1);
    int nb2 = 0;
    int nb3 = (T - l1 - l2) > 0 ? 1 << (T - l1 - l2) : 1;
    const int nb1 = 1 << l1;
    CHK(buf_ensure(h, h->ar_misc[MISC_L1_CHILDREN], (uint64_t)nb1 * 16));
    uint64_t *c1_start = (uint64_t *)h->ar_misc[MISC_L1_CHILDREN].p, *c1_cnt = c1_start + nb1;
    dbg::Buf &ms_scpre = h->ar_misc[MISC_MS_SCPRE], &ms_cmat = h->ar_misc[MISC_MS_CMAT], &ms_offs = h->ar_misc[MISC_MS_OFFS];
    int where = 0;
    double est_distinct = 0.0;
    const int top = 6 + SK_BUCKET_BITS;
    Timer t_part(h->stream);
    const int bps = pre ? nb1 >> shard_bits : 0;
    const uint64_t b_lo = pre ? (uint64_t)my_shard * bps : 0;
    uint64_t *ps_start = nullptr, *ps_cnt = nullptr, *ps_add = nullptr;
    uint32_t ps_n = 0;
    if (pre) {
        ps_n = (uint32_t)(bps * pre->n_senders);
        std::vector<uint64_t> &hs = h->host_scpre;
        hs.assign((size_t)ps_n * 3, 0);
        for (int r = 0; r < pre->n_senders; ++r) {
            uint64_t at = pre->recv_off[r];
            for (int b = 0; b < bps; ++b) {
                const size_t i = (size_t)b * pre->n_senders + r;
                hs[i] = at;
                hs[ps_n + i] = pre->counts[(size_t)r * bps + b];
                hs[2 * (size_t)ps_n + i] = pre->stamp_add[r];
                at += pre->counts[(size_t)r * bps + b];
            }
        }
        CHK(buf_ensure(h, h->ar_misc[MISC_SEGMENTS], (uint64_t)ps_n * 3 * 8));
        ps_start = (uint64_t *)h->ar_misc[MISC_SEGMENTS].p; ps_cnt = ps_start + ps_n; ps_add = ps_cnt + ps_n;
        HIPCHK(h, hipMemcpyAsync(ps_start, hs.data(), hs.size() * 8, hipMemcpyHostToDevice, h->stream));
        HIPCHK(h, hipStreamSynchronize(h->stream));
    } else {
        if (xs && xs->f0 && l1 >= xs->f0) {
            if (xs->l1 != l1) ++h->presplit_rehists;
            CHK((multisplit_level<ST, true>(h, seg_start, seg_cnt, n_seg, xs->n_wg, n_rec, in_w0, in_w1, in_st, w0[1], w1[1], st[1],
                                            top - l1, nb1 >> xs->f0, c1_start, c1_cnt, ms_scpre, ms_cmat, ms_offs, 0, nullptr, nullptr,
                                            host_cnt, xs->l1 == l1 ? xs->cmat : nullptr)));
        } else {
            CHK((multisplit_level<ST, true>(h, seg_start, seg_cnt, n_seg, n_seg, n_rec, in_w0, in_w1, in_st, w0[1], w1[1], st[1],
                                            top - l1, nb1, c1_start, c1_cnt, ms_scpre, ms_cmat, ms_offs, 0, nullptr, nullptr, host_cnt)));
        }
        where = 1;
    }
    if (auto_T && l1 >= 9 && n_rec) {
        const uint32_t probe_bucket = (pp.probe_first_owned && shard_bits) ? (uint32_t)my_shard << (l1 - shard_bits) : 0u;
        const uint64_t inst_bucket = (uint64_t)((double)n_inst * own / nb1) * 2 + 1024;
        uint64_t set_cap = 1024;
        while (set_cap < inst_bucket * 2) set_cap <<= 1;
        CHK(buf_ensure(h, h->ar_misc[MISC_ESTIMATE_SET], set_cap * 8));
        unsigned long long *set = (unsigned long long *)h->ar_misc[MISC_ESTIMATE_SET].p;
        unsigned long long *d_est = (unsigned long long *)(h->d_scalars + SC_ESTIMATE);
        HIPCHK(h, hipMemsetAsync(set, 0xFF, set_cap * 8, h->stream));
        HIPCHK(h, hipMemsetAsync(d_est, 0, 16, h->stream));
        if (pre) {
            for (int r = 0; r < pre->n_senders; ++r) pp.estimate(128u, ps_start, ps_cnt, (uint32_t)r, in_w0, in_w1, set, set_cap - 1, d_est);
        } else {
            pp.estimate(512u, c1_start, c1_cnt, probe_bucket, w0[1], w1[1], set, set_cap - 1, d_est);
        }
        uint64_t est[2] = {0, 0};
        HIPCHK(h, hipMemcpyAsync(est, d_est, 16, hipMemcpyDeviceToHost, h->stream));
        HIPCHK(h, hipStreamSynchronize(h->stream));
        if (est[0]) {
            double distinct = (double)n_inst * own * (double)est[1] / (double)est[0];
            if (pre) {
                uint64_t probe_recs = 0;
                for (int r = 0; r < pre->n_senders; ++r) probe_recs += pre->counts[(size_t)r * bps];
                distinct = probe_recs ? (double)est[1] * (double)n_rec / (double)probe_recs * own : 0.0;
            }
            est_distinct = distinct / own;
            const double want = distinct / ((double)h->target_distinct > 0 ? (double)h->target_distinct : pp.target);
            const double want2 = std::max<double>(1.0, std::ceil(want / nb1));
            if (want2 <= 1024.0) {
                nb2 = (int)want2;
                nb3 = 1;
            } else {
                nb2 = 1024;
                nb3 = (int)std::min<double>((double)(1 << (SK_BUCKET_BITS - l1 - 10)), std::ceil(want2 / 1024.0));
            }
            l2 = nb2 > 1 ? 1 : 0;
        }
    }
    if (nb2 == 0 && l2 > 0) nb2 = 1 << l2;
    if (pre && l2 == 0) { l2 = 1; nb2 = 1; }
    if (l2 == 0) nb3 = 1;
    const int fb2 = (nb3 == 1 && ((nb2 > 0 && (nb2 & (nb2 - 1)) != 0) || (auto_T && l1 >= 9 && nb2 > 1))) ? SK_BUCKET_BITS - l1 : 0;
    const uint64_t n_l2 = l2 > 0 ? (uint64_t)nb1 * (uint64_t)nb2 : (uint64_t)nb1;
    const uint64_t n_buckets = n_l2 * (uint64_t)nb3;
    const int l2_pow = (fb2 || l2 == 0) ? 0 : (int)std::lround(std::log2((double)nb2));
    const int fb3 = nb3 > 1 ? SK_BUCKET_BITS - l1 - l2_pow : 0;
    CHK(buf_ensure(h, h->ar_misc[MISC_BUCKETS], n_buckets * 16));
    uint64_t *b_start = (uint64_t *)h->ar_misc[MISC_BUCKETS].p, *b_cnt = b_start + n_buckets;
    uint64_t *l2_start = b_start, *l2_cnt = b_cnt;
    if (nb3 > 1) {
        CHK(buf_ensure(h, h->ar_l2, n_l2 * 16));
        l2_start = (uint64_t *)h->ar_l2.p;
        l2_cnt = l2_start + n_l2;
    }
    if (l2 > 0) {
        const int sh2 = fb2 ? top - SK_BUCKET_BITS : top - l1 - l2_pow;
        if (pre) {
            unsigned long long *d_sums = (unsigned long long *)(h->d_scalars + SC_L2_SUMS);
            HIPCHK(h, hipMemsetAsync(b_start, 0, n_buckets * 16, h->stream));
            if (nb3 > 1) HIPCHK(h, hipMemsetAsync(l2_start, 0, n_l2 * 16, h->stream));
            HIPCHK(h, hipMemsetAsync(d_sums, 0, 16, h->stream));
            CHK((multisplit_level<ST, true, STI, STHI>(h, ps_start, ps_cnt, ps_n, (uint32_t)pre->n_senders, n_rec, in_w0, in_w1,
                                                       (const STI *)pre->in_st, w0[0], w1[0], st[0], sh2, nb2, l2_start + b_lo * nb2,
                                                       l2_cnt + b_lo * nb2, ms_scpre, ms_cmat, ms_offs, fb2, ps_add,
                                                       pp.sum_instances ? d_sums : (unsigned long long *)nullptr)));
            if (pp.sum_instances) {
                uint64_t sums[2] = {0, 0};
                HIPCHK(h, hipMemcpyAsync(sums, d_sums, 16, hipMemcpyDeviceToHost, h->stream));
                HIPCHK(h, hipStreamSynchronize(h->stream));
                n_inst = sums[0];
                n_edge_inst = sums[1];
                h->n_kmer_inst = n_inst;
                h->n_edge_inst = n_edge_inst;
            }
        } else {
            CHK((multisplit_level<ST, true>(h, c1_start, c1_cnt, (uint32_t)nb1, 1, n_rec, w0[1], w1[1], st[1], w0[0], w1[0],
                                            st[0], sh2, nb2, l2_start, l2_cnt, ms_scpre, ms_cmat, ms_offs, fb2)));
        }
        where = 0;
        if (nb3 > 1) {
            if (!w0[1]) {
                CHK(buf_ensure(h, h->ar_rec[1][0], (n_rec + 16) * 8));
                CHK(buf_ensure(h, h->ar_rec[1][1], (n_rec + 16) * 8));
                CHK(buf_ensure(h, h->ar_rec[1][2], (n_rec + 16) * sizeof(ST)));
                w0[1] = (uint64_t *)h->ar_rec[1][0].p; w1[1] = (uint64_t *)h->ar_rec[1][1].p; st[1] = (ST *)h->ar_rec[1][2].p;
            }
            const uint64_t p_lo = pre ? b_lo * nb2 : 0, p_n = pre ? (uint64_t)bps * nb2 : n_l2;
            CHK((multisplit_level<ST, true>(h, l2_start + p_lo, l2_cnt + p_lo, (uint32_t)p_n, 1, n_rec, w0[0], w1[0], st[0], w0[1],
                                            w1[1], st[1], top - SK_BUCKET_BITS, nb3, b_start + p_lo * nb3, b_cnt + p_lo * nb3,
                                            ms_scpre, ms_cmat, ms_offs, fb3)));
            where = 1;
        }
    } else {
        HIPCHK(h, hipMemcpyAsync(b_start, c1_start, (size_t)nb1 * 8, hipMemcpyDeviceToDevice, h->stream));
        HIPCHK(h, hipMemcpyAsync(b_cnt, c1_cnt, (size_t)nb1 * 8, hipMemcpyDeviceToDevice, h->stream));
    }
    h->stats.ms_partition = t_part.stop();
    h->stats.n_buckets = n_buckets;
    *out = SkPartition{b_start, b_cnt, n_buckets, where, l1, l2 > 0 ? nb2 : 1, fb2, l2_pow, nb3, fb3, est_distinct, n_inst, n_edge_inst};
    return DBG_OK;
}

static int resolve_counts_in(dbg *h) {
    if (!h->resolve_count) return DBG_OK;
    uint64_t c[2] = {0, 0};
    HIPCHK(h, hipMemcpyAsync(c, h->d_scalars + SC_RESOLVE_COUNTS, 16, hipMemcpyDeviceToHost, h->stream));
    HIPCHK(h, hipStreamSynchronize(h->stream));
    h->resolve_direct_hits += c[0];
    h->resolve_keyed += c[1];
    return DBG_OK;
}

template <class ST, int CAP, class STI = ST>
static int sk_count_from_segments(dbg *h, int k, const uint64_t *seg_start, const uint64_t *seg_cnt, uint32_t n_seg,
                                  const uint64_t *host_cnt, uint64_t n_rec, uint64_t n_inst, uint64_t n_edge_inst,
                                  const uint64_t *in_w0, const uint64_t *in_w1, const ST *in_st, uint64_t *w0[2], uint64_t *w1[2],
                                  ST *st[2], uint64_t node_capacity_hint, int shard_bits, int my_shard,
                                  const Presplit *pre = nullptr, const ExtractSplit *xs = nullptr) {
    const int m = sk_m_for_k(k);
    unsigned long long *sc_dev = (unsigned long long *)h->d_scalars;
    uint64_t sc[8] = {0};
    auto estimate = [h, k](unsigned grid, const uint64_t *s_start, const uint64_t *s_cnt, uint32_t seg, const uint64_t *rw0,
                           const uint64_t *rw1, unsigned long long *set, uint64_t set_mask, unsigned long long *d_est) {
        hipLaunchKernelGGL(HIP_KERNEL_NAME(k_estimate_distinct<ST>), dim3(grid), dim3(256), 0, h->stream, s_start, s_cnt, seg, rw0,
                           rw1, k, set, set_mask, d_est);
    };
    const SkPartitionParams<decltype(estimate)> pp{SK_TARGET_DISTINCT<CAP>, DBG_L1_WIDE_FROM, true, true, estimate};
    SkPartition P;
    CHK((sk_partition<ST, STI, 0>(h, pp, seg_start, seg_cnt, n_seg, host_cnt, pre, xs, in_w0, in_w1, in_st, w0, w1, st, shard_bits,
                                  my_shard, n_rec, n_inst, n_edge_inst, &P)));
    n_inst = P.n_inst;
    n_edge_inst = P.n_edge_inst;
    uint64_t *const b_start = P.b_start, *const b_cnt = P.b_cnt;
    const uint64_t n_buckets = P.n_buckets;
    const int where = P.where;
    const double est_distinct = P.est_distinct;

    const uint64_t id_limit = (shard_bits && !h->wide_owner) ? (h->shard_node_limit ? h->shard_node_limit : (1ull << 29) - 16)
                                                             : 0xFFFFFFF0ull;
    const uint32_t id_tag = (shard_bits && !h->wide_owner) ? ((uint32_t)my_shard << 29) : 0u;
    const uint64_t node_cap_max = std::min<uint64_t>(n_inst, id_limit);
    const uint64_t edge_cap_max = std::min<uint64_t>(n_edge_inst + 16, 0xFFFFFFF0ull);
    uint64_t node_cap = node_capacity_hint ? std::min<uint64_t>(node_capacity_hint, id_limit) : node_cap_max;
    if (!node_capacity_hint && est_distinct > 0.0)
        node_cap = std::min<uint64_t>(node_cap_max, (uint64_t)(est_distinct * 1.2 * h->est_scale_pct / 100.0) +
                                                        (h->est_scale_pct == 100 ? (1u << 20) : 1024u));
    uint64_t edge_cap = std::min<uint64_t>(edge_cap_max, node_cap + node_cap / 4 + 16);
    auto ensure_node_arrays = [&]() -> int {
        CHK(buf_ensure(h, h->ar_node[0], node_cap * 8));
        CHK(buf_ensure(h, h->ar_node[sizeof(ST) == 8 ? 1 : 7], node_cap * sizeof(ST)));
        CHK(buf_ensure(h, h->ar_node[3], node_cap));
        h->d_keys = (uint64_t *)h->ar_node[0].p;
        h->d_stamps_st = h->ar_node[sizeof(ST) == 8 ? 1 : 7].p;
        h->stamps_st_bytes = (int)sizeof(ST);
        h->d_stamps = sizeof(ST) == 8 ? (uint64_t *)h->d_stamps_st : nullptr;
        h->d_flags = (uint8_t *)h->ar_node[3].p;
        h->nodes_in_arena = true;
        CHK(buf_ensure(h, h->ar_csr[3], (node_cap + 1) * 4));
        CHK(buf_ensure(h, h->ar_csr[1], edge_cap * 4));
        CHK(buf_ensure(h, h->ar_csr[2], edge_cap * 4));
        h->d_rowptr32 = (uint32_t *)h->ar_csr[3].p;
        h->d_col = (uint32_t *)h->ar_csr[1].p;
        h->d_ecnt = (uint32_t *)h->ar_csr[2].p;
        return DBG_OK;
    };
    uint64_t q_cap = n_rec + 1024;
    uint64_t *qk[2], *qm[2];
    uint32_t *qc[2];
    const uint64_t range_cap = n_buckets + 4096 + n_inst / (CAP / 4);
    CHK(buf_ensure(h, h->ar_misc[MISC_RANGES], range_cap * sizeof(SkRange)));
    SkRange *ranges = (SkRange *)h->ar_misc[MISC_RANGES].p;
    const uint64_t own_cnt = n_buckets >> shard_bits, own_lo = (uint64_t)my_shard * own_cnt;
    h->dir_valid = false;
    CHK(buf_ensure(h, h->ar_dir, (own_cnt + (range_cap - n_buckets)) * (CAP / 64) * sizeof(SkDirEnt)));
    SkDirEnt *dirs = (SkDirEnt *)h->ar_dir.p;
    bool use_count2 = CAP == 4096 && h->count_kernel >= 2 && !h->phase_limit && (sizeof(ST) == 4 || h->count_kernel_u64 >= 2);
    const bool use_count3 = use_count2 && ((sizeof(ST) == 8 && h->count_kernel_u64 == 3) || h->count_kernel == 3);
    int extra_attempts = 0;
    for (int attempt = 0; attempt < 3 + extra_attempts; ++attempt) {
        CHK(ensure_node_arrays());
        for (int set = 0; set < 2; ++set) {
            CHK(buf_ensure(h, h->ar_q[set][0], q_cap * 8));
            CHK(buf_ensure(h, h->ar_q[set][2], q_cap * 4));
            if (shard_bits || h->resolve_sorted) CHK(buf_ensure(h, h->ar_q[set][1], q_cap * 8));
            qk[set] = (uint64_t *)h->ar_q[set][0].p;
            qm[set] = (uint64_t *)h->ar_q[set][1].p;
            qc[set] = (uint32_t *)h->ar_q[set][2].p;
            if (!shard_bits && !h->resolve_sorted) break;
        }
        Timer t(h->stream);
        HIPCHK(h, hipMemsetAsync(h->d_scalars, 0, 64 * 8, h->stream));
        HIPCHK(h, hipMemsetAsync(ranges, 0, n_buckets * sizeof(SkRange), h->stream));
        HIPCHK(h, hipMemsetAsync(dirs, 0, own_cnt * (CAP / 64) * sizeof(SkDirEnt), h->stream));
        SkCountOut out{h->d_keys, h->d_stamps_st, h->d_flags, node_cap, h->d_rowptr32, h->d_col, h->d_ecnt, edge_cap,
                       qk[0], qc[0], q_cap, ranges, n_buckets, range_cap, dirs, own_lo, own_cnt, id_tag, sc_dev};
        uint32_t split_recs = 0;
        if (est_distinct > 0.0 && n_rec)
            split_recs = (uint32_t)std::min<double>(1e9, std::max<double>(64.0, (CAP * 0.80) / (est_distinct / (double)n_rec)));
        if (use_count2 && n_rec) {
            auto kern2 = use_count3 ? k_sk_count3<ST> : k_sk_count2<ST>;
            const size_t lds2 = use_count3 ? sizeof(Cnt3Lds<ST>) : sizeof(Cnt2Lds<ST>);
            HIPCHK(h, hipFuncSetAttribute((const void *)kern2, hipFuncAttributeMaxDynamicSharedMemorySize, (int)lds2));
            int n_cu = 256;
            (void)hipDeviceGetAttribute(&n_cu, hipDeviceAttributeMultiprocessorCount, h->device);
            const unsigned grid = (unsigned)std::min<uint64_t>(n_buckets, (uint64_t)n_cu);
            SkCount2Args a2{out, b_start, b_cnt, w0[where], w1[where], (const void *)st[where], n_buckets, split_recs, k};
            SkCount2Args *d_a2 = (SkCount2Args *)(h->d_scalars + SC_DESCRIPTOR);
            static_assert(sizeof(SkCount2Args) <= (SK2_QUERY_CURSOR - SC_DESCRIPTOR) * 8, "the query cursor sits behind the descriptor");
            HIPCHK(h, hipMemcpyAsync(d_a2, &a2, sizeof(a2), hipMemcpyHostToDevice, h->stream));
            HIPCHK(h, hipMemsetAsync(h->d_scalars + SK2_QUERY_CURSOR, 0, 8, h->stream));
            hipLaunchKernelGGL(kern2, dim3(grid), dim3(Cnt2Cfg<ST>::NT), lds2, h->stream, (const SkCount2Args *)d_a2);
            HIPCHK(h, hipGetLastError());
        }
        auto kern = k_sk_count<ST, CAP>;
        const size_t lds = sizeof(CntLds<ST, CAP>);
        HIPCHK(h, hipFuncSetAttribute((const void *)kern, hipFuncAttributeMaxDynamicSharedMemorySize, (int)lds));
        if (n_rec && !use_count2) {
            int n_cu = 256;
            (void)hipDeviceGetAttribute(&n_cu, hipDeviceAttributeMultiprocessorCount, h->device);
            constexpr int NT = CntCfg<ST, CAP>::NT;
            const uint64_t per_cu = std::max<uint64_t>(1, std::min<uint64_t>(2048 / NT, (160 * 1024) / lds));
            const unsigned grid = (unsigned)std::min<uint64_t>(n_buckets, (uint64_t)n_cu * per_cu);
            static_assert(sizeof(SkCountOut) <= 64 * 8, "descriptor slot");
            SkCountOut *d_out = (SkCountOut *)(h->d_scalars + SC_DESCRIPTOR);
            HIPCHK(h, hipMemcpyAsync(d_out, &out, sizeof(out), hipMemcpyHostToDevice, h->stream));
            hipLaunchKernelGGL(kern, dim3(grid), dim3(NT), lds, h->stream, b_start, b_cnt, w0[where], w1[where],
                               st[where], k, m, n_buckets, (const SkCountOut *)d_out, split_recs, h->phase_limit);
            HIPCHK(h, hipGetLastError());
        }
        h->stats.count_launches = n_rec ? (uint64_t)(attempt + 1) : 0;
        HIPCHK(h, hipMemcpyAsync(sc, h->d_scalars, 64, hipMemcpyDeviceToHost, h->stream));
        uint64_t q2 = 0;
        if (use_count2 && n_rec) HIPCHK(h, hipMemcpyAsync(&q2, h->d_scalars + SK2_QUERY_CURSOR, 8, hipMemcpyDeviceToHost, h->stream));
        h->stats.ms_count = t.stop();
        if (use_count2 && n_rec) sc[5] = q2;
        if (h->phase_limit) { h->err = "ablation run (phase_limit set): timing only"; return DBG_E_ARG; }
        if (sc[0] & (STATUS_BUCKET_TOO_BIG | STATUS_RANGE_CAP)) break;
        bool again = false;
        if (use_count2 && (sc[0] & (STATUS_COUNTER16 | STATUS_INCONSISTENT))) {
            if ((sc[0] & STATUS_INCONSISTENT) && !(sc[0] & STATUS_COUNTER16)) { h->err = "internal: k_sk_count2 / k_sk_count3 counted a bucket's nodes, edges or queries inconsistently"; return DBG_E_HIP; }
            use_count2 = false;
            ++extra_attempts;
            again = true;
        }
        if ((sc[0] & STATUS_NODE_EDGE_CAP) && (node_cap < node_cap_max || edge_cap < edge_cap_max) && !node_capacity_hint) {
            node_cap = node_cap_max;
            edge_cap = edge_cap_max;
            again = true;
        }
        if ((sc[0] & STATUS_QUERY_CAP) && q_cap < n_edge_inst + 1024) { q_cap = n_edge_inst + 1024; again = true; }
        if (!again || attempt == 2 + extra_attempts) break;
    }
    if (sc[0] & STATUS_BUCKET_TOO_BIG) { h->err = "a bucket could not be split to fit the LDS table"; return DBG_E_CAPACITY; }
    if (sc[0] & STATUS_NODE_EDGE_CAP) { h->err = "node/edge capacity exceeded"; return DBG_E_CAPACITY; }
    if (sc[0] & (STATUS_RANGE_CAP | STATUS_QUERY_CAP)) { h->err = "range/query list overflow"; return DBG_E_CAPACITY; }
    h->n_nodes = sc[4] & 0xFFFFFFFFull;
    h->n_edges = sc[4] >> 32;
    {
        const uint32_t ne32 = (uint32_t)h->n_edges;
        HIPCHK(h, hipMemcpyAsync(h->d_rowptr32 + h->n_nodes, &ne32, 4, hipMemcpyHostToDevice, h->stream));
    }
    h->csr_built = true;
    h->dense_pending = true;
    uint64_t n_q = sc[5];
    const uint64_t n_ranges = n_buckets + sc[6];
    h->stats.n_queries = n_q;
    SkGeom geom{k, m, P.l1, P.nb2, P.fb2, P.l2_pow, P.nb3, P.fb3, shard_bits, my_shard, own_lo, own_cnt};

    {
        Timer t(h->stream);
        uint64_t root[2] = {0, n_q};
        int qset = 0;
        if (shard_bits && n_q) {
            hipLaunchKernelGGL(k_q_bucket, dim3(grid_for(n_q, 256)), dim3(256), 0, h->stream, qk[0], qm[0], n_q, k, m);
            HIPCHK(h, hipGetLastError());
            CHK(buf_ensure(h, h->ar_misc[MISC_QUERY_SEGS], 512 * 16 + 16));
            uint64_t *q_seg = (uint64_t *)h->ar_misc[MISC_QUERY_SEGS].p;
            const int nsh = 1 << shard_bits;
            HIPCHK(h, hipMemcpyAsync(q_seg, root, 16, hipMemcpyHostToDevice, h->stream));
            uint64_t *o_start = q_seg + 2, *o_cnt = o_start + nsh;
            CHK((multisplit_level<uint32_t, true>(h, q_seg, q_seg + 1, 1, 1, n_q, qk[0], qm[0], qc[0], qk[1], qm[1], qc[1],
                                                  40 + SK_BUCKET_BITS - shard_bits, nsh, o_start, o_cnt, h->ar_misc[MISC_MS_SCPRE],
                                                  h->ar_misc[MISC_MS_CMAT], h->ar_misc[MISC_MS_OFFS])));
            ShardState &sh = shard_of(h);
            sh.q_start.assign(nsh, 0);
            sh.q_cnt.assign(nsh, 0);
            HIPCHK(h, hipMemcpyAsync(sh.q_start.data(), o_start, (size_t)nsh * 8, hipMemcpyDeviceToHost, h->stream));
            HIPCHK(h, hipMemcpyAsync(sh.q_cnt.data(), o_cnt, (size_t)nsh * 8, hipMemcpyDeviceToHost, h->stream));
            HIPCHK(h, hipStreamSynchronize(h->stream));
            CHK(buf_ensure(h, h->ar_shard[0], n_q * 8));
            CHK(buf_ensure(h, h->ar_shard[3], n_q * 4));
            HIPCHK(h, hipMemcpyAsync(h->ar_shard[0].p, qk[1], n_q * 8, hipMemcpyDeviceToDevice, h->stream));
            HIPCHK(h, hipMemcpyAsync(h->ar_shard[3].p, qc[1], n_q * 4, hipMemcpyDeviceToDevice, h->stream));
            root[0] = sh.q_start[my_shard];
            root[1] = sh.q_cnt[my_shard];
            sh.n_remote = n_q - root[1];
            sh.q_cnt[my_shard] = 0;
            n_q = root[1];
            qset = 1;
        }
        const uint64_t *q_meta = nullptr;
        if (!shard_bits && h->resolve_sorted && (n_q >= (1u << 20) || (h->resolve_sorted == 2 && n_q))) {
            hipLaunchKernelGGL(k_q_bucket, dim3(grid_for(n_q, 256)), dim3(256), 0, h->stream, qk[0], qm[0], n_q, k, m);
            HIPCHK(h, hipGetLastError());
            CHK(buf_ensure(h, h->ar_misc[MISC_QUERY_SEGS], 1024 * 16 + 16));
            uint64_t *q_seg = (uint64_t *)h->ar_misc[MISC_QUERY_SEGS].p;
            HIPCHK(h, hipMemcpyAsync(q_seg, root, 16, hipMemcpyHostToDevice, h->stream));
            uint64_t *o_start = q_seg + 2, *o_cnt = o_start + 512;
            CHK((multisplit_level<uint32_t, true>(h, q_seg, q_seg + 1, 1, 1, n_q, qk[0], qm[0], qc[0], qk[1], qm[1], qc[1],
                                                  40 + SK_BUCKET_BITS - 9, 512, o_start, o_cnt, h->ar_misc[MISC_MS_SCPRE], h->ar_misc[MISC_MS_CMAT],
                                                  h->ar_misc[MISC_MS_OFFS])));
            qset = 1;
            q_meta = qm[1];
        }
        if (n_q) {
            const bool direct = !shard_bits && h->resolve_direct;
            auto resolver = direct ? k_succ_resolve<CAP, true, false> : k_succ_resolve<CAP, false, false>;
            if (h->resolve_count) {
                resolver = direct ? k_succ_resolve<CAP, true, true> : k_succ_resolve<CAP, false, true>;
                HIPCHK(h, hipMemsetAsync(sc_dev + SC_RESOLVE_COUNTS, 0, 16, h->stream));
            }
            hipLaunchKernelGGL(resolver, dim3(grid_for(n_q, 256)), dim3(256), 0, h->stream,
                               qk[qset] + root[0], qc[qset] + root[0], n_q, geom, ranges, n_buckets, n_ranges, dirs, h->d_keys,
                               h->n_nodes, h->d_col, id_tag, sc_dev, q_meta, sc_dev + SC_RESOLVE_COUNTS);
            HIPCHK(h, hipGetLastError());
            HIPCHK(h, hipMemcpyAsync(sc, h->d_scalars, 8, hipMemcpyDeviceToHost, h->stream));
            CHK(resolve_counts_in(h));
            HIPCHK(h, hipStreamSynchronize(h->stream));
            if (sc[0] & STATUS_SUCC_MISSING) { h->err = "internal: a successor k-mer was not found in its bucket"; return DBG_E_HIP; }
        }
        h->stats.ms_succ = t.stop();
    }
    int T = 0;
    while ((1ull << T) < n_buckets) ++T;
    h->sk_T = T; h->sk_l1 = P.l1; h->sk_l2 = P.l2_pow; h->sk_nb2 = P.fb2 ? P.nb2 : 0; h->sk_n_ranges = n_ranges; h->sk_cap = CAP;
    h->sk_geom = geom; h->sk_n_buckets = n_buckets;
    if (!shard_bits) {
        h->sk_src.w0 = w0[where]; h->sk_src.w1 = w1[where]; h->sk_src.st = st[where]; h->sk_src.st_bytes = (int)sizeof(ST);
        h->sk_src.b_start = b_start; h->sk_src.b_cnt = b_cnt;
        h->sk_src.valid = n_rec != 0;
    }
    return DBG_OK;
}


__global__ __launch_bounds__(256) void k_wsk_iota128(uint64_t n, uint64_t *w0) {
    const uint64_t i = (uint64_t)blockIdx.x * blockDim.x + threadIdx.x;
    if (i < n) w0[i] = i * 128;
}

template <class ST>
static int wsk_extract(dbg *h, int k, uint64_t **pk_out, uint64_t *w0[2], uint64_t *w1[2], ST *st[2], uint64_t **seg_start_out,
                       uint64_t **seg_cnt_out, uint32_t *n_seg_out, uint64_t *n_rec_out, int part = 0, int n_parts = 1) {
    const int m = SK_MAX_M, w = k - m + 1;
    unsigned long long *sc_dev = (unsigned long long *)h->d_scalars;
    uint64_t sc[8] = {0};
    const uint64_t pk_words = (h->n_bytes + 31) / 32;
    CHK(buf_ensure(h, h->ar_wide[0], (pk_words + 8) * 8));
    uint64_t *pk = (uint64_t *)h->ar_wide[0].p;
    HIPCHK(h, hipMemsetAsync(pk + pk_words, 0, 8 * 8, h->stream));
    if (pk_words)
        hipLaunchKernelGGL(k_wpack, dim3(grid_for(pk_words, 256)), dim3(256), 0, h->stream, h->d_bases, h->n_bytes, pk_words, pk);
    const uint64_t all_tiles = (h->n_bytes + TILE - 1) / TILE;
    const uint64_t tile_first = all_tiles * (uint64_t)part / (uint64_t)n_parts;
    const uint64_t tiles = all_tiles * (uint64_t)(part + 1) / (uint64_t)n_parts - tile_first;
    const bool reg_kernel = (w >= 20 && w <= 51) && !h->extract_generic;
    const uint32_t n_wg = (uint32_t)std::min<uint64_t>(std::max<uint64_t>(tiles, 1), reg_kernel ? 2048 : 1024);
    CHK(buf_ensure(h, h->ar_misc[MISC_SEGMENTS], (uint64_t)n_wg * 4 * 8));
    uint64_t *seg_start = (uint64_t *)h->ar_misc[MISC_SEGMENTS].p, *seg_cnt = seg_start + n_wg, *seg_nk = seg_cnt + n_wg, *seg_ne = seg_nk + n_wg;
    std::vector<uint64_t> hseg((size_t)n_wg * 4);
    uint64_t n_rec = 0;
    Timer t(h->stream);
    const uint64_t tiles_per_wg = (tiles + n_wg - 1) / n_wg;
    const double density = std::min(1.0, 2.6 / (double)(w + 1) + 1.3 * (double)(h->n_reads + 1) / (double)(h->n_bytes + 1) + 0.01);
    uint64_t seg_cap = (uint64_t)((double)(tiles_per_wg * TILE) * density) + 256;
    for (int attempt = 0; attempt < 2; ++attempt) {
        const uint64_t rec_cap = seg_cap * n_wg;
        for (int set = 0; set < 2; ++set) {
            CHK(buf_ensure(h, h->ar_rec[set][0], rec_cap * 8));
            CHK(buf_ensure(h, h->ar_rec[set][1], rec_cap * 8));
            CHK(buf_ensure(h, h->ar_rec[set][2], rec_cap * sizeof(ST)));
            w0[set] = (uint64_t *)h->ar_rec[set][0].p;
            w1[set] = (uint64_t *)h->ar_rec[set][1].p;
            st[set] = (ST *)h->ar_rec[set][2].p;
        }
        for (uint32_t g = 0; g < n_wg; ++g) hseg[g] = (uint64_t)g * seg_cap;
        HIPCHK(h, hipMemcpyAsync(seg_start, hseg.data(), (size_t)n_wg * 8, hipMemcpyHostToDevice, h->stream));
        HIPCHK(h, hipMemsetAsync(seg_cnt, 0, (size_t)n_wg * 3 * 8, h->stream));
        HIPCHK(h, hipMemsetAsync(h->d_scalars, 0, 64 * 8, h->stream));
        if (tiles && reg_kernel) {
#define DBG_WEXW_CASE(W_) case W_: hipLaunchKernelGGL(HIP_KERNEL_NAME(k_wsk_extract_w<ST, W_>), dim3(n_wg), dim3(256), 0, h->stream, \
                                                       h->d_bases, h->n_bytes, h->d_startbits, tiles, w0[0], w1[0], st[0], seg_cap, seg_cnt, \
                                                       seg_nk, seg_ne, sc_dev, tile_first); break;
            switch (w) {
                DBG_WEXW_CASE(20) DBG_WEXW_CASE(21) DBG_WEXW_CASE(22) DBG_WEXW_CASE(23) DBG_WEXW_CASE(24) DBG_WEXW_CASE(25)
                DBG_WEXW_CASE(26) DBG_WEXW_CASE(27) DBG_WEXW_CASE(28) DBG_WEXW_CASE(29) DBG_WEXW_CASE(30) DBG_WEXW_CASE(31)
                DBG_WEXW_CASE(32) DBG_WEXW_CASE(33) DBG_WEXW_CASE(34) DBG_WEXW_CASE(35) DBG_WEXW_CASE(36) DBG_WEXW_CASE(37)
                DBG_WEXW_CASE(38) DBG_WEXW_CASE(39) DBG_WEXW_CASE(40) DBG_WEXW_CASE(41) DBG_WEXW_CASE(42) DBG_WEXW_CASE(43)
                DBG_WEXW_CASE(44) DBG_WEXW_CASE(45) DBG_WEXW_CASE(46) DBG_WEXW_CASE(47) DBG_WEXW_CASE(48) DBG_WEXW_CASE(49)
                DBG_WEXW_CASE(50) DBG_WEXW_CASE(51)
                default: break;
            }
#undef DBG_WEXW_CASE
        } else if (tiles) {
            auto ekern = k_wsk_extract<ST>;
            HIPCHK(h, hipFuncSetAttribute((const void *)ekern, hipFuncAttributeMaxDynamicSharedMemorySize, (int)sizeof(WSkLds)));
            hipLaunchKernelGGL(ekern, dim3(n_wg), dim3(WSK_NT), sizeof(WSkLds), h->stream, h->d_bases, h->n_bytes,
                               h->d_startbits, k, tiles, w0[0], w1[0], st[0], seg_cap, seg_cnt, seg_nk, seg_ne, sc_dev, tile_first);
        }
        HIPCHK(h, hipGetLastError());
        HIPCHK(h, hipMemcpyAsync(sc, h->d_scalars, 8, hipMemcpyDeviceToHost, h->stream));
        HIPCHK(h, hipMemcpyAsync(hseg.data(), seg_start, (size_t)n_wg * 4 * 8, hipMemcpyDeviceToHost, h->stream));
        HIPCHK(h, hipStreamSynchronize(h->stream));
        if (sc[0] & STATUS_BAD_BASE) { h->err = "reads hold a byte outside ACGT"; return DBG_E_ALPHABET; }
// ... 163 lines not shown
            uint64_t *s_lo = (uint64_t *)h->ar_q[1][0].p, *s_meta = (uint64_t *)h->ar_q[1][1].p;
            uint32_t *s_col = (uint32_t *)h->ar_q[1][2].p;
            hipLaunchKernelGGL(k_wq_bucket, dim3(grid_for(n_q, 256)), dim3(256), 0, h->stream, q_lo, q_hi, q_meta, n_q, k, m);
            HIPCHK(h, hipGetLastError());
            CHK(buf_ensure(h, h->ar_misc[MISC_QUERY_SEGS], 512 * 16 + 16));
            uint64_t *q_seg = (uint64_t *)h->ar_misc[MISC_QUERY_SEGS].p;
            const int nsh = 1 << shard_bits;
            const uint64_t root[2] = {0, n_q};
            HIPCHK(h, hipMemcpyAsync(q_seg, root, 16, hipMemcpyHostToDevice, h->stream));
            uint64_t *o_start = q_seg + 2, *o_cnt = o_start + nsh;
            CHK((multisplit_level<uint32_t, true>(h, q_seg, q_seg + 1, 1, 1, n_q, q_lo, q_meta, q_col, s_lo, s_meta, s_col,
                                                  40 + SK_BUCKET_BITS - shard_bits, nsh, o_start, o_cnt, h->ar_misc[MISC_MS_SCPRE],
                                                  h->ar_misc[MISC_MS_CMAT], h->ar_misc[MISC_MS_OFFS])));
            ShardState &sh = shard_of(h);
            sh.q_start.assign(nsh, 0);
            sh.q_cnt.assign(nsh, 0);
            HIPCHK(h, hipMemcpyAsync(sh.q_start.data(), o_start, (size_t)nsh * 8, hipMemcpyDeviceToHost, h->stream));
            HIPCHK(h, hipMemcpyAsync(sh.q_cnt.data(), o_cnt, (size_t)nsh * 8, hipMemcpyDeviceToHost, h->stream));
            CHK(buf_ensure(h, h->ar_shard[0], n_q * 16));
            CHK(buf_ensure(h, h->ar_shard[3], n_q * 4));
            uint64_t *pairs = (uint64_t *)h->ar_shard[0].p;
            hipLaunchKernelGGL(k_wq_park, dim3(grid_for(n_q, 256)), dim3(256), 0, h->stream, n_q, s_lo, s_meta, q_hi, pairs);
            HIPCHK(h, hipGetLastError());
            HIPCHK(h, hipMemcpyAsync(h->ar_shard[3].p, s_col, n_q * 4, hipMemcpyDeviceToDevice, h->stream));
            HIPCHK(h, hipStreamSynchronize(h->stream));
            const uint64_t mine_at = sh.q_start[my_shard], mine_n = sh.q_cnt[my_shard];
            sh.n_remote = n_q - mine_n;
            sh.q_cnt[my_shard] = 0;
            r_lo = pairs + 2 * mine_at;
            r_hi = r_lo + 1;
            r_col = (const uint32_t *)h->ar_shard[3].p + mine_at;
            stride = 2;
            n_q = mine_n;
        }
        if (n_q) {
            const bool direct = !shard_bits && h->resolve_direct;
            auto resolver = direct ? k_wsucc_resolve<true, false> : k_wsucc_resolve<false, false>;
            if (h->resolve_count) {
                resolver = direct ? k_wsucc_resolve<true, true> : k_wsucc_resolve<false, true>;
                HIPCHK(h, hipMemsetAsync(sc_dev + SC_RESOLVE_COUNTS, 0, 16, h->stream));
            }
            hipLaunchKernelGGL(resolver, dim3(grid_for(n_q, 256)), dim3(256), 0, h->stream, r_lo, r_hi, stride, r_col, n_q, geom,
                               ranges, n_buckets, n_ranges, dirs, h->d_keys, h->d_keys_hi, h->n_nodes, h->d_col, id_tag, sc_dev,
                               sc_dev + SC_RESOLVE_COUNTS);
            HIPCHK(h, hipGetLastError());
            HIPCHK(h, hipMemcpyAsync(sc, h->d_scalars, 8, hipMemcpyDeviceToHost, h->stream));
            CHK(resolve_counts_in(h));
            HIPCHK(h, hipStreamSynchronize(h->stream));
            if (sc[0] & STATUS_SUCC_MISSING) { h->err = "internal: a successor k-mer was not found in its bucket"; return DBG_E_HIP; }
        }
        h->stats.ms_succ = t.stop();
    }
    h->sk_geom = geom; h->sk_n_buckets = n_buckets; h->sk_n_ranges = n_ranges; h->sk_cap = WCAP;
    h->sk_src.valid = false;
    (void)w;
    return DBG_OK;
}

template <class ST>
static int build_wsk_t(dbg *h, int k) {
    uint64_t *pk = nullptr, *w0[2], *w1[2], *seg_start = nullptr, *seg_cnt = nullptr, n_rec = 0;
    ST *st[2];
    uint32_t n_seg = 0;
    CHK(wsk_extract<ST>(h, k, &pk, w0, w1, st, &seg_start, &seg_cnt, &n_seg, &n_rec));
    return wsk_count<ST, ST>(h, k, pk, seg_start, seg_cnt, n_seg, h->host_seg_cnt.data(), n_rec, h->n_kmer_inst, h->n_edge_inst, w0[0], w1[0], st[0], w0, w1, st,
                             0, 0, nullptr);
}

static int build_wsk(dbg *h, int k, bool *fallback) {
    *fallback = false;
    int rc = (h->n_bytes >= (1ull << 31) || h->stamp64) ? build_wsk_t<uint64_t>(h, k) : build_wsk_t<uint32_t>(h, k);
    if (rc == DBG_E_CAPACITY && h->err == "16-bit successor counter overflow") *fallback = true;
    return rc;
}

template <class ST, int CAP>
static int build_sk_t(dbg *h, int k, uint64_t node_capacity_hint) {
    uint64_t *w0[2], *w1[2], *seg_start = nullptr, *seg_cnt = nullptr, n_rec = 0;
    ST *st[2];
    uint32_t n_seg = 0;
    ExtractSplit xs;
    xs.target = SK_TARGET_DISTINCT<CAP>;
    CHK(sk_extract<ST>(h, k, w0, w1, st, &seg_start, &seg_cnt, &n_seg, &n_rec, 0, 1, &xs));
    return sk_count_from_segments<ST, CAP>(h, k, seg_start, seg_cnt, n_seg, h->host_seg_cnt.data(), n_rec, h->n_kmer_inst, h->n_edge_inst, w0[0],
                                           w1[0], st[0], w0, w1, st, node_capacity_hint, 0, 0, nullptr, &xs);
}

static int build_sk(dbg *h, int k, uint64_t node_capacity_hint) {
    const bool small = (h->n_bytes < (1ull << 31)) && !h->stamp64;
    if (!small) return build_sk_t<uint64_t, 4096>(h, k, node_capacity_hint);
    if (h->lds_slots == 2048) return build_sk_t<uint32_t, 2048>(h, k, node_capacity_hint);
    return build_sk_t<uint32_t, 4096>(h, k, node_capacity_hint);
}

static ShardState &shard_of(dbg *h) {
    if (!h->shard_state) h->shard_state = new ShardState();
    return *(ShardState *)h->shard_state;
}

__global__ __launch_bounds__(256) void k_stamp_globalize(const uint32_t *__restrict__ st32, const uint64_t *__restrict__ w1,
                                                         uint64_t n, uint64_t base2, uint64_t *st64,
                                                         unsigned long long *sums ) {
    const uint64_t stride = (uint64_t)gridDim.x * blockDim.x;
    uint64_t n_inst = 0, n_edge = 0;
    for (uint64_t i = (uint64_t)blockIdx.x * blockDim.x + threadIdx.x; i < n; i += stride) {
        st64[i] = base2 + st32[i];
        const uint64_t x = w1[i];
        n_inst += ((x >> 1) & 31) + 1;
        n_edge += ((x >> 1) & 31) + (x & 1);
    }
    n_inst = wave_sum_u64(n_inst);
    n_edge = wave_sum_u64(n_edge);
    if ((threadIdx.x & 63) == 0) {
        if (n_inst) atomicAdd(&sums[0], (unsigned long long)n_inst);
        if (n_edge) atomicAdd(&sums[1], (unsigned long long)n_edge);
    }
}

__global__ __launch_bounds__(256) void k_apply_remote(const uint32_t *__restrict__ qcol, const uint32_t *__restrict__ ans,
                                                      uint64_t n, uint32_t tag, uint32_t *col, unsigned long long *scalars) {
    uint64_t i = (uint64_t)blockIdx.x * blockDim.x + threadIdx.x;
    if (i >= n) return;
    const uint32_t a = ans[i];
    if (a == NO_NODE || a >= (1u << 29)) { atomicOr(&scalars[0], STATUS_REMOTE_UNRESOLVED); return; }
    col[qcol[i]] = tag | a;
}

static int shard_args_ok(dbg *h, int k, int n_shards) {
    if (!h) return DBG_E_ARG;
    if (k < 1 || k > 63) { h->err = "k must be in 1..63"; return DBG_E_ARG; }
    if (n_shards < 1 || n_shards > 8 || (n_shards & (n_shards - 1))) {
        h->err = "n_shards must be 1, 2, 4 or 8 (owner = top bits of the bucket hash; node ids keep 29 bits)";
        return DBG_E_ARG;
    }
    if (h->engine != 0) { h->err = "sharded builds use the super-k-mer engine"; return DBG_E_ARG; }
    return DBG_OK;
}

struct HasSuccBit {
    const uint64_t *t_st;
    __device__ uint64_t operator()(uint64_t i) const { return (t_st[i] >> 32) & 1ull; }
};

static int shard_extract_wide(dbg *h, int k, int n_shards, uint64_t *send_counts, const void **d_lo, const void **d_hi,
                              const void **d_st) {
    free_build(h);
    h->stats = dbg_stats_t{};
    CHK(compute_alphabet(h));
    if (!h->is_dna) { h->err = "sharded builds take ACGT reads"; return DBG_E_ALPHABET; }
    int shard_bits = 0;
    while ((1 << shard_bits) < n_shards) ++shard_bits;
    Timer t(h->stream);
    unsigned long long *cursor = (unsigned long long *)(h->d_scalars + 48);
    HIPCHK(h, hipMemsetAsync(h->d_scalars, 0, 64 * 8, h->stream));
    const uint64_t tiles = (h->n_bytes + TILE - 1) / TILE;
    if (tiles)
        hipLaunchKernelGGL(HIP_KERNEL_NAME(k_ws_extract<false>), dim3((unsigned)tiles), dim3(256), 0, h->stream, h->d_bases,
                           h->n_bytes, h->d_startbits, k, shard_bits, cursor, (uint64_t *)nullptr, (uint64_t *)nullptr,
                           (uint64_t *)nullptr, (unsigned long long *)h->d_scalars);
    uint64_t sc[64];
    HIPCHK(h, hipMemcpyAsync(sc, h->d_scalars, 64 * 8, hipMemcpyDeviceToHost, h->stream));
    HIPCHK(h, hipStreamSynchronize(h->stream));
    HIPCHK(h, hipGetLastError());
    if (sc[0] & STATUS_BAD_BASE) { h->err = "reads hold a byte outside ACGT"; return DBG_E_ALPHABET; }
    h->n_kmer_inst = sc[1];
    h->n_edge_inst = sc[2];
    uint64_t offs[8] = {0}, total = 0;
// ... 2628 lines not shown
```

### py-debruijn_amd/csrc/dbg_sk.h

```cpp
#pragma once
#include <cstddef>
#include "dbg_device.h"
#include "dbg_dir.h"
#include "dbg_minwin.h"

namespace dbgk {

constexpr int SK_MAX_M = 13;
constexpr int SK_BUCKET_BITS = 22;
constexpr int SK_META_BITS = 28;

__host__ __device__ inline int sk_m_for_k(int k) { return k < SK_MAX_M ? k : SK_MAX_M; }

__host__ __device__ inline uint32_t fmix32(uint32_t x) {
    x ^= x >> 16; x *= 0x85EBCA6Bu;
    x ^= x >> 13; x *= 0xC2B2AE35u;
    x ^= x >> 16;
    return x;
}
__device__ inline uint32_t bucket_hash22(uint32_t mmer) { return fmix32(mmer * 0x9E3779B1u + 0x7F4A7C15u) >> (32 - SK_BUCKET_BITS); }

__device__ inline uint32_t kmer_bucket22(uint64_t kmer, int k, int m) {
    const int w = k - m + 1;
    const uint32_t mmask = (uint32_t)((1ull << (2 * m)) - 1);
// ... 297 lines not shown
            uint64_t w0 = window32(s.t, j);
            uint64_t hi = window32(s.t, j + 32);
            if (nb < 32) { w0 &= ~0ull << (64 - 2 * nb); hi = 0; }
            else if (nb == 32) hi = 0;
            else hi &= ~0ull << (64 - 2 * (nb - 32));
            const uint32_t mp = (j & ~31) + s.minp[(j & ~31) + index_byte_at(j & 31)];
            const uint32_t bh = bucket_hash22((uint32_t)(window32(s.t, mp) >> (64 - 2 * M)));
            const uint64_t w1 = (hi & (~0ull << SK_META_BITS)) | ((uint64_t)bh << 6) | ((uint64_t)(len - 1) << 1) | has_succ;
            uint64_t o = gbase + r;
            if constexpr (PS) {
                const uint32_t c = bh >> (SK_BUCKET_BITS - f0);
                const uint32_t rk = atomicAdd(&ps.cur[c], 1u);
                if (cmat) atomicAdd(&ps.h1[bh >> (SK_BUCKET_BITS - l1)], 1u);
                if (rk >= seg_cap) { ps.ovf = 1; continue; }
                o = ((uint64_t)c * gridDim.x + blockIdx.x) * seg_cap + rk;
            }
            rec_w0[o] = w0;
            rec_w1[o] = w1;
            rec_st[o] = (ST)((p << 1) | (s0 ^ 1u));
        }
    }
    n_k = wave_sum_u64(n_k);
    n_e = wave_sum_u64(n_e);
    __syncthreads();
    if constexpr (PS) {
        if (ps.ovf) overflow = true;
        if (threadIdx.x < (1 << f0))
            seg_cnt[(uint64_t)threadIdx.x * gridDim.x + blockIdx.x] = min(ps.cur[threadIdx.x], (uint32_t)seg_cap);
        if (cmat) {
            const int nbg = 1 << (l1 - f0);
            for (int d = threadIdx.x; d < (1 << l1); d += 256)
                cmat[((uint64_t)(d >> (l1 - f0)) * gridDim.x + blockIdx.x) * nbg + (d & (nbg - 1))] = ps.h1[d];
        }
    }
    if (overflow && threadIdx.x == 0) atomicOr(&scalars[0], STATUS_SEGMENT_FULL);
    if ((threadIdx.x & 63) == 0) { red[threadIdx.x >> 6] = n_k; red[4 + (threadIdx.x >> 6)] = n_e; }
    __syncthreads();
    if (threadIdx.x == 0) {
        if constexpr (!PS) seg_cnt[blockIdx.x] = cursor;
        seg_nk[blockIdx.x] = red[0] + red[1] + red[2] + red[3];
        seg_ne[blockIdx.x] = red[4] + red[5] + red[6] + red[7];
    }
}

#ifndef DBG_MS_CH
#define DBG_MS_CH 4096
#endif
constexpr int MS_CH = DBG_MS_CH;
template <class ST> struct MsChunk { static constexpr int CH = sizeof(ST) == 8 ? MS_CH : MS_CH + MS_CH / 2; };
constexpr int MS_SC = 32768;
constexpr int MS_MAX_NB = 1024;
#ifndef DBG_MS_NT
#define DBG_MS_NT 512
#endif
constexpr int MS_NT = DBG_MS_NT;

struct MsParents {
    const uint64_t *start;
    const uint64_t *cnt;
    const uint64_t *sc_pre;
    uint32_t n_seg;
    uint32_t spg;
};

__device__ inline void ms_locate(const MsParents &P, uint64_t g, uint32_t *seg, uint64_t *sidx) {
    uint32_t lo = 0, hi = P.n_seg;
    while (hi - lo > 1) {
        const uint32_t mid = (lo + hi) >> 1;
        if (P.sc_pre[mid] <= g) lo = mid; else hi = mid;
    }
    *seg = lo;
    *sidx = g - P.sc_pre[lo];
}

__device__ inline uint32_t ms_child(uint64_t w1, int shift, int nb, int fbits) {
    const uint32_t v = (uint32_t)(w1 >> shift);
    return fbits ? (uint32_t)(((uint64_t)(v & ((1u << fbits) - 1u)) * (uint32_t)nb) >> fbits) : (v & (uint32_t)(nb - 1));
}

template <bool SUMS>
__global__ __launch_bounds__(256) void k_ms_hist(MsParents P, const uint64_t *__restrict__ w1, int shift, int nb, int fbits,
                                                 uint32_t *cmat, unsigned long long *sums) {
    __shared__ uint32_t hist[MS_MAX_NB];
    uint32_t seg;
    uint64_t sidx;
    ms_locate(P, blockIdx.x, &seg, &sidx);
    for (int b = threadIdx.x; b < nb; b += 256) hist[b] = 0;
    __syncthreads();
    const uint64_t beg = P.start[seg] + sidx * MS_SC;
    const uint64_t end = min(P.start[seg] + P.cnt[seg], beg + (uint64_t)MS_SC);
    uint64_t n_inst = 0, n_edge = 0;
    for (uint64_t i = beg + threadIdx.x; i < end; i += 256) {
        const uint64_t x = w1[i];
        atomicAdd(&hist[ms_child(x, shift, nb, fbits)], 1u);
        if (SUMS) { n_inst += ((x >> 1) & 31) + 1; n_edge += ((x >> 1) & 31) + (x & 1); }
    }
    __syncthreads();
    for (int b = threadIdx.x; b < nb; b += 256) cmat[(uint64_t)blockIdx.x * nb + b] = hist[b];
    if (SUMS) {
        n_inst = wave_sum_u64(n_inst);
        n_edge = wave_sum_u64(n_edge);
        if ((threadIdx.x & 63) == 0) {
            if (n_inst) atomicAdd(&sums[0], (unsigned long long)n_inst);
            if (n_edge) atomicAdd(&sums[1], (unsigned long long)n_edge);
        }
    }
}

struct MsLogical {
    MsParents P;
    const uint32_t *cmat;
    int nb;
    __device__ uint64_t operator()(uint64_t L) const {
        const uint32_t n_groups = P.n_seg / P.spg;
        uint32_t lo = 0, hi = n_groups;
        while (hi - lo > 1) {
            const uint32_t mid = (lo + hi) >> 1;
            if ((uint64_t)nb * P.sc_pre[mid * P.spg] <= L) lo = mid; else hi = mid;
        }
        const uint64_t g_lo = P.sc_pre[lo * P.spg];
        const uint64_t nsc = P.sc_pre[(lo + 1) * P.spg] - g_lo;
        const uint64_t r = L - (uint64_t)nb * g_lo;
        const uint64_t b = r / nsc, sidx = r - b * nsc;
        return cmat[(g_lo + sidx) * nb + b];
    }
};

__global__ __launch_bounds__(256) void k_ms_children(MsParents P, const uint64_t *__restrict__ offs, int nb,
                                                     uint64_t total, uint64_t *c_start, uint64_t *c_cnt) {
    const uint64_t i = (uint64_t)blockIdx.x * blockDim.x + threadIdx.x;
    const uint32_t n_groups = P.n_seg / P.spg;
    const uint64_t n_child = (uint64_t)n_groups * nb;
    if (i >= n_child) return;
    const uint32_t g = (uint32_t)(i / nb), b = (uint32_t)(i % nb);
    const uint64_t g_lo = P.sc_pre[g * P.spg], g_hi = P.sc_pre[(g + 1) * P.spg];
    const uint64_t nsc = g_hi - g_lo;
    const uint64_t L = (uint64_t)nb * g_lo + (uint64_t)b * nsc;
    const uint64_t Ln = L + nsc;
    const uint64_t total_L = (uint64_t)nb * P.sc_pre[P.n_seg];
    const uint64_t a = (L < total_L) ? offs[L] : total;
    const uint64_t e = (Ln < total_L) ? offs[Ln] : total;
    c_start[i] = a;
    c_cnt[i] = (nsc == 0) ? 0 : e - a;
}

template <class ST>
struct MsLds {
    uint64_t w0[MsChunk<ST>::CH];
    uint64_t w1[MsChunk<ST>::CH];
    ST st[MsChunk<ST>::CH];
    uint32_t hist[MS_MAX_NB];
    uint32_t start[MS_MAX_NB];
    uint64_t run[MS_MAX_NB];
};

#ifdef DBG_MS_PROF
__device__ unsigned long long g_ms_prof[8];
#define MS_TICK(i) do { if (threadIdx.x == 0) { const unsigned long long now_ = clock64(); prof_[i] += now_ - last_; last_ = now_; } } while (0)
#else
#define MS_TICK(i) do {} while (0)
#endif

template <class ST, bool HAS_ST, class STI = ST, int STHI = 0>
__global__ __launch_bounds__(MS_NT) void k_ms_scatter(MsParents P, const uint64_t *__restrict__ in_w0,
                                                    const uint64_t *__restrict__ in_w1, const STI *__restrict__ in_st,
                                                    const uint64_t *__restrict__ seg_add,
                                                    int shift, int nb, int fbits, const uint64_t *__restrict__ offs,
                                                    uint64_t *out_w0, uint64_t *out_w1, ST *out_st) {
    extern __shared__ __attribute__((aligned(16))) unsigned char ms_raw[];
    MsLds<ST> &s = *reinterpret_cast<MsLds<ST> *>(ms_raw);
    constexpr int CH = MsChunk<ST>::CH;
    static_assert(CH % MS_NT == 0 && sizeof(MsLds<ST>) <= 160 * 1024, "multisplit chunk");
#ifdef DBG_MS_PROF
    unsigned long long prof_[8] = {0, 0, 0, 0, 0, 0, 0, 0}, last_ = clock64();
#endif
    uint32_t seg;
    uint64_t sidx;
    ms_locate(P, blockIdx.x, &seg, &sidx);
    const ST st_add = (HAS_ST && seg_add) ? (ST)seg_add[seg] : (ST)0;
    MS_TICK(0);
    const uint32_t grp = seg / P.spg;
    const uint64_t g_lo = P.sc_pre[grp * P.spg], g_hi = P.sc_pre[(grp + 1) * P.spg];
    const uint64_t nsc = g_hi - g_lo, gidx = (uint64_t)blockIdx.x - g_lo;
    const uint64_t lbase = (uint64_t)nb * g_lo;
    for (int b = threadIdx.x; b < nb; b += MS_NT) s.run[b] = offs[lbase + (uint64_t)b * nsc + gidx];
    const uint64_t beg = P.start[seg] + sidx * MS_SC;
    const uint64_t end = min(P.start[seg] + P.cnt[seg], beg + (uint64_t)MS_SC);
    for (uint64_t c0 = beg; c0 < end; c0 += CH) {
        const int n = (int)min((uint64_t)CH, end - c0);
        for (int b = threadIdx.x; b < nb; b += MS_NT) s.hist[b] = 0;
        __syncthreads();
        MS_TICK(1);
        uint64_t r0[CH / MS_NT], r1[CH / MS_NT];
        ST rs[CH / MS_NT];
        uint32_t rk[CH / MS_NT];
#pragma unroll
        for (int i = 0; i < CH / MS_NT; ++i) {
            const int q = i * MS_NT + threadIdx.x;
            if (q < n) {
                r0[i] = in_w0[c0 + q];
                r1[i] = in_w1[c0 + q];
                if constexpr (STHI > 0) {
                    static_assert(sizeof(ST) == 8 && sizeof(STI) == 4, "stamp high bits: 32-bit stamps in, 64-bit out");
                    rs[i] = (((ST)(r1[i] >> STHI) << 32) | (ST)in_st[c0 + q]) + st_add;
                    r1[i] &= (1ull << STHI) - 1;
                } else if (HAS_ST) {
                    rs[i] = (ST)in_st[c0 + q] + st_add;
                }
                rk[i] = atomicAdd(&s.hist[ms_child(r1[i], shift, nb, fbits)], 1u);
            }
        }
        __syncthreads();
        MS_TICK(2);
        {
            constexpr int EPT = MS_MAX_NB / MS_NT;
            const int b0 = threadIdx.x * EPT;
            uint32_t h4[EPT];
            uint64_t sum = 0;
#pragma unroll
            for (int j = 0; j < EPT; ++j) { h4[j] = (b0 + j < nb) ? s.hist[b0 + j] : 0; sum += h4[j]; }
            uint64_t tot;
            uint32_t ex = (uint32_t)block_exscan<MS_NT / 64>(sum, &tot);
#pragma unroll
            for (int j = 0; j < EPT; ++j) { if (b0 + j < nb) s.start[b0 + j] = ex; ex += h4[j]; }
        }
        __syncthreads();
        MS_TICK(3);
#pragma unroll
        for (int i = 0; i < CH / MS_NT; ++i) {
            const int q = i * MS_NT + threadIdx.x;
            if (q < n) {
                const uint32_t b = ms_child(r1[i], shift, nb, fbits);
                const uint32_t d = s.start[b] + rk[i];
                s.w0[d] = r0[i];
                s.w1[d] = r1[i];
                if (HAS_ST) s.st[d] = rs[i];
            }
        }
        __syncthreads();
        MS_TICK(4);
        for (int q = threadIdx.x; q < n; q += MS_NT) {
            const uint64_t x1 = s.w1[q];
            const uint32_t b = ms_child(x1, shift, nb, fbits);
            const uint64_t g = s.run[b] + (q - s.start[b]);
            out_w0[g] = s.w0[q];
            out_w1[g] = x1;
            if (HAS_ST) out_st[g] = s.st[q];
        }
        __syncthreads();
        MS_TICK(5);
        for (int b = threadIdx.x; b < nb; b += MS_NT) s.run[b] += s.hist[b];
        __syncthreads();
        MS_TICK(6);
    }
#ifdef DBG_MS_PROF
    if (threadIdx.x == 0) {
        for (int i = 0; i < 7; ++i) atomicAdd(&g_ms_prof[i], prof_[i]);
        atomicAdd(&g_ms_prof[7], 1ull);
    }
#endif
}


template <class ST>
__global__ __launch_bounds__(256) void k_estimate_distinct(const uint64_t *__restrict__ b_start,
                                                           const uint64_t *__restrict__ b_cnt, uint32_t bucket,
                                                           const uint64_t *__restrict__ rec_w0,
                                                           const uint64_t *__restrict__ rec_w1, int k,
                                                           unsigned long long *set, uint64_t set_mask,
                                                           unsigned long long *out ) {
    const uint64_t beg = b_start[bucket], n = b_cnt[bucket];
    uint64_t inst = 0, fresh = 0;
    for (uint64_t r = (uint64_t)blockIdx.x * blockDim.x + threadIdx.x; r < n; r += (uint64_t)gridDim.x * blockDim.x) {
        const uint64_t w0 = rec_w0[beg + r], w1 = rec_w1[beg + r];
        const uint64_t hi = w1 & (~0ull << SK_META_BITS);
        const int len = (int)((w1 >> 1) & 31) + 1;
        for (int i = 0; i < len; ++i) {
            const uint64_t kmer = (i ? (w0 << (2 * i)) | (hi >> (64 - 2 * i)) : w0) >> (64 - 2 * k);
            ++inst;
            uint64_t slot = mix64(kmer) & set_mask;
            for (uint64_t probe = 0; probe <= set_mask; ++probe) {
                unsigned long long cur = set[slot];
                if (cur == EMPTY_KEY) {
                    cur = atomicCAS(&set[slot], EMPTY_KEY, (unsigned long long)kmer);
                    if (cur == EMPTY_KEY) { ++fresh; break; }
                }
                if (cur == kmer) break;
                slot = (slot + 1) & set_mask;
            }
        }
    }
    inst = wave_sum_u64(inst);
    fresh = wave_sum_u64(fresh);
    if ((threadIdx.x & 63) == 0) {
        if (inst) atomicAdd(&out[0], (unsigned long long)inst);
        if (fresh) atomicAdd(&out[1], (unsigned long long)fresh);
    }
}

struct SkRange {
    uint32_t bucket;
    uint32_t mask, val;
    uint32_t node_cnt;
    uint64_t node_base;
    uint32_t next;
    uint32_t pad;
};

__device__ inline uint32_t fold32(uint64_t kmer) { return (uint32_t)kmer * 0x9E3779B1u ^ (uint32_t)(kmer >> 32) * 0x85EBCA77u; }
__device__ inline uint32_t sub_hash(uint64_t kmer) { return fmix32(fold32(kmer) ^ 0x27D4EB2Fu); }
__device__ inline uint32_t slot_hash(uint64_t kmer) {
    const uint32_t lo = (uint32_t)kmer, hi = (uint32_t)(kmer >> 32);
    return (lo ^ (hi << 11) ^ (hi >> 7) ^ (lo >> 15)) * 0x9E3779B1u;
}
template <int CAP>
__device__ inline uint32_t slot_of(uint64_t kmer) {
    static_assert(CAP == 2048 || CAP == 4096, "table size");
    return slot_hash(kmer) >> (CAP == 4096 ? 20 : 21);
}

template <class ST, int CAP>
struct CntCfg {
    #ifdef DBG_CNT_PROF
    static constexpr int QBUF = CAP == 4096 ? (sizeof(ST) == 8 ? 624 : 768) : 400;
#else
    static constexpr int QBUF = CAP == 4096 ? (sizeof(ST) == 8 ? 640 : 768) : 400;
#endif
    static constexpr int NT = CAP == 4096 ? 1024 : 512;
};
constexpr int CNT_STACK = 24;
constexpr int CNT_PROBE_LIMIT = 1024;

template <class ST, int CAP>
struct CntLds {
    static constexpr int CNT_QBUF = CntCfg<ST, CAP>::QBUF;
    unsigned long long keys[CAP];
    uint32_t cnt[CAP * 4];
    ST stamp[CAP];
    uint16_t list[CAP];
    uint16_t eoff[CAP];
    unsigned long long q_key[CNT_QBUF];
    unsigned long long q_meta[CNT_QBUF];
    ST st_stage[CNT_QBUF];
    uint32_t stk_mask[CNT_STACK], stk_val[CNT_STACK];
    int stk_n;
    uint32_t overflow, n_local , n_q, fail, n_flat;
    unsigned long long gbase, qbase, ebase, ri;
    unsigned long long dir_mask[CAP / 64];
    uint16_t dir_base[CAP / 64];
#ifdef DBG_CNT_PROF
    unsigned long long prof[64];
#endif
};

__device__ inline uint64_t rec_window(uint64_t w0, uint64_t hi, int i) {
    return (w0 << (2 * i)) | ((hi >> 1) >> (63 - 2 * i));
}

template <int CAP>
__device__ inline int lds_find(const unsigned long long *keys, uint64_t key) {
    uint32_t slot = slot_of<CAP>(key);
#pragma unroll 16
    for (int probe = 0; probe < CAP; ++probe) {
        const unsigned long long cur = keys[slot];
        if (cur == key) return (int)slot;
        if (cur == EMPTY_KEY) return -1;
        slot = (slot + 1) & (CAP - 1);
    }
    return -1;
}


struct SkCountOut {
    uint64_t *keys;
    void *stamps;
    uint8_t *flags;
    uint64_t node_cap;
    uint32_t *rowptr;
    uint32_t *col, *ecnt;
// ... 604 lines not shown
```

### py-debruijn_amd/csrc/dbg_sk2.h

```cpp
#pragma once
#include "dbg_sk.h"

#ifndef DBG_SK2_LANEQUAD
#define DBG_SK2_LANEQUAD 0
#endif
#ifndef DBG_SK2_UNROLL
#define DBG_SK2_UNROLL 8
#endif
#ifndef DBG_SK2_PROBE
#define DBG_SK2_PROBE 0
#endif

namespace dbgk {

struct SkCount2Args {
    SkCountOut out;
    const uint64_t *b_start, *b_cnt, *rec_w0, *rec_w1;
    const void *rec_st;
    uint64_t n_buckets;
    uint32_t split_recs;
    int k;
};
static_assert(sizeof(SkCount2Args) <= 64 * 8, "descriptor slot of the scalar block");

typedef const SkCount2Args __attribute__((address_space(4))) *SkArgs2ConstPtr;
__device__ inline SkArgs2ConstPtr fresh_args2(const SkCount2Args *p) {
    unsigned long long v = (unsigned long long)p;
    asm volatile("" : "+s"(v));
    return (SkArgs2ConstPtr)v;
}

template <class ST>
struct Cnt2Cfg {
    static constexpr int CAP = 4096;
    static constexpr int NT = 1024;
#ifdef DBG_CNT_PROF
    static constexpr int QBUF = sizeof(ST) == 8 ? 296 : 736;
#else
    static constexpr int QBUF = sizeof(ST) == 8 ? 320 : 768;
#endif
    static constexpr int QS = sizeof(ST) == 8 ? 256 : 512;
    static constexpr int PEND = sizeof(ST) == 8 ? 2048 : 4096;
};

constexpr int SC_ESTIMATE = 40;
constexpr int SC_RESOLVE_COUNTS = 48;
constexpr int SC_L2_SUMS = 56;
constexpr int SC_DESCRIPTOR = 64;
constexpr int SK2_QUERY_CURSOR = 120;
constexpr uint32_t HINT_VALID = 0x8000u;
constexpr uint32_t HINT_QUERY = 0x4000u;
constexpr int PEND_SEG = 256;

template <class ST>
struct Cnt2Lds {
    static constexpr int CAP = Cnt2Cfg<ST>::CAP;
    static constexpr int QBUF = Cnt2Cfg<ST>::QBUF;
    unsigned long long keys[CAP];
    uint32_t ch[CAP * 4];
    ST stamp[CAP];
    uint16_t list[CAP];
    uint16_t eoff[CAP];
    uint16_t pend[Cnt2Cfg<ST>::PEND];
    unsigned long long q_key[QBUF];
    unsigned long long q_meta[QBUF];
    ST st_stage[QBUF];
    unsigned long long qs_key[Cnt2Cfg<ST>::QS];
    uint32_t qs_col[Cnt2Cfg<ST>::QS];
    unsigned long long dir_mask[CAP / 64];
    uint16_t dir_base[CAP / 64];
    uint16_t pend_cnt[16];
    uint32_t dummy[64];
    uint32_t stk_mask[CNT_STACK], stk_val[CNT_STACK];
    uint32_t overflow, n_new , n_list , n_q, n_q2, n_q3, n_flat, fail, pend_over;
    unsigned long long gbase, ebase, qbase, ri;
#ifdef DBG_CNT_PROF
    unsigned long long prof[64];
#endif
};

__device__ inline uint32_t wave_sum_dpp(uint32_t v) {
    v += (uint32_t)__builtin_amdgcn_update_dpp(0, (int)v, 0x111 , 0xF, 0xF, true);
    v += (uint32_t)__builtin_amdgcn_update_dpp(0, (int)v, 0x112 , 0xF, 0xF, true);
    v += (uint32_t)__builtin_amdgcn_update_dpp(0, (int)v, 0x114 , 0xF, 0xF, true);
    v += (uint32_t)__builtin_amdgcn_update_dpp(0, (int)v, 0x118 , 0xF, 0xF, true);
    v += (uint32_t)__builtin_amdgcn_update_dpp(0, (int)v, 0x142 , 0xA, 0xF, false);
    v += (uint32_t)__builtin_amdgcn_update_dpp(0, (int)v, 0x143 , 0xC, 0xF, false);
    return v;
}

template <class ST>
__global__ __launch_bounds__(1024) void k_sk_count2(const SkCount2Args *__restrict__ argp) {
    constexpr int CAP = Cnt2Cfg<ST>::CAP, NT = Cnt2Cfg<ST>::NT, QBUF = Cnt2Cfg<ST>::QBUF, PEND = Cnt2Cfg<ST>::PEND, QS = Cnt2Cfg<ST>::QS;
    constexpr int NPT = CAP / NT;
    constexpr int PSEG = PEND / 16;
    constexpr uint32_t STAGE = QBUF;
    extern __shared__ __attribute__((aligned(16))) unsigned char cnt_raw[];
    using LdsT = Cnt2Lds<ST>;
    LdsT &s = *reinterpret_cast<LdsT *>(cnt_raw);
    static_assert(sizeof(LdsT) <= 160 * 1024, "LDS");
    static_assert(QBUF * 5 <= CAP && STAGE <= (uint32_t)NT && CAP / 2 >= 2 * QBUF, "quad list / dedupe scratch");
    static_assert(PSEG <= PEND_SEG && NT == 1024, "one pending segment per wave");
    constexpr uint64_t BH_FIELD = ((1ull << SK_BUCKET_BITS) - 1) << 6;
    uint16_t *flat = s.list;
    const int lane = threadIdx.x & 63, wave = threadIdx.x >> 6;
    const int k = fresh_args2(argp)->k;
    const uint32_t n_buckets = (uint32_t)fresh_args2(argp)->n_buckets;
    const uint32_t split_recs = fresh_args2(argp)->split_recs;

#ifdef DBG_CNT_PROF
    unsigned long long clast_ = clock64(), csub_ = clast_;
    if (threadIdx.x < 64) s.prof[threadIdx.x] = 0;
    __syncthreads();
#endif
    bool clean = false;
    uint64_t pf_w0 = 0, pf_w1 = 0;
    ST pf_st = 0;
    uint64_t nx_beg = 0;
    uint32_t nx_n = 0;
    uint64_t r2_beg_v = 0, r2_n_v = 0;
    auto load_range = [&](uint32_t bucket) {
        uint32_t vb = bucket;
        asm volatile("" : "+v"(vb));
        r2_beg_v = 0;
        r2_n_v = 0;
        if (vb < n_buckets) {
            const auto &a = *fresh_args2(argp);
// ... 529 lines not shown
```

Baseline: 59.05 billion k-mers/s.

## Queue build stages ahead without host syncs using device-side totals and guards

```diff
diff --git a/py-debruijn_amd/_dbg.py b/py-debruijn_amd/_dbg.py
--- a/py-debruijn_amd/_dbg.py
+++ b/py-debruijn_amd/_dbg.py
@@ -82,7 +82,7 @@
 
 COUNTERS = ("extract_presplit_fallbacks", "extract_presplit_rehists", "resolve_direct_hits", "resolve_keyed",
             "refine_crowded", "pull_crowded", "lookup_index_builds", "lookup_dir_calls", "lookup_index_calls",
-            "part_lookup_calls")
+            "part_lookup_calls", "build_host_waits", "build_speculation_discards")
 
 
 class DbgError(RuntimeError):
diff --git a/py-debruijn_amd/csrc/dbg_hip.hip b/py-debruijn_amd/csrc/dbg_hip.hip
--- a/py-debruijn_amd/csrc/dbg_hip.hip
+++ b/py-debruijn_amd/csrc/dbg_hip.hip
@@ -5,7 +5,9 @@
 #include <cstdlib>
 #include <cstdio>
 #include <cstring>
+#include <memory>
 #include <string>
+#include <utility>
 #include <vector>
 
 #include <cerrno>
@@ -17,6 +19,7 @@
 
 #include "../../include/dbg.h"
 #include "dbg_device.h"
+#include "dbg_stage.h"
 #include "dbg_sk.h"
 #include "dbg_sk2.h"
 #include "dbg_sk3.h"
@@ -166,6 +169,17 @@
     bool wide_owner = false;
     bool borrowed_stream = false;
     bool arena_freed = false;
+    int build_queue_ahead = 1;
+    bool qa_on = false;
+    uint64_t build_waits = 0;
+    uint64_t spec_discards = 0;
+    hipEvent_t qa_ev[10] = {};
+    bool qa_made = false;
+    StageBlock stage;
+    Buf tab_iota, tab_segstart;
+    LinearTableKey key_iota, key_segstart;
+    std::vector<std::pair<const void *, int>> lds_attr;
+    int n_cu = 0;
     std::vector<uint64_t> host_seg_cnt;
     std::vector<uint64_t> host_scpre;
     uint64_t shard_node_limit = 0;
@@ -243,6 +257,7 @@
 }
 static void pool_trim(dbg *h) {
     if (!h->arena_freed) return;
+    ++h->build_waits;
     (void)hipStreamSynchronize(h->stream);
     hipMemPool_t pool;
     if (hipDeviceGetDefaultMemPool(&pool, h->device) == hipSuccess) (void)hipMemPoolTrimTo(pool, 0);
@@ -283,13 +298,15 @@
 struct Timer {
     hipEvent_t a = nullptr, b = nullptr;
     hipStream_t s;
-    explicit Timer(hipStream_t st) : s(st) {
+    uint64_t *waits;
+    explicit Timer(hipStream_t st, uint64_t *host_waits = nullptr) : s(st), waits(host_waits) {
         (void)hipEventCreate(&a);
         (void)hipEventCreate(&b);
         (void)hipEventRecord(a, s);
     }
     double stop() {
         (void)hipEventRecord(b, s);
+        if (waits) ++*waits;
         (void)hipEventSynchronize(b);
         float ms = 0;
         (void)hipEventElapsedTime(&ms, a, b);
@@ -301,11 +318,96 @@
     }
 };
 
+enum QaEvent {
+    EV_TOTAL_A, EV_TOTAL_B, EV_EXTRACT_A, EV_EXTRACT_B, EV_PART_A, EV_PART_B, EV_COUNT_A, EV_COUNT_B, EV_SUCC_A, EV_SUCC_B,
+    QA_EVENTS
+};
+static_assert(QA_EVENTS <= sizeof(dbg::qa_ev) / sizeof(dbg::qa_ev[0]), "event pool");
+
+static void *stage_host_alloc(size_t bytes) {
+    void *p = nullptr;
+    if (hipHostMalloc(&p, bytes, hipHostMallocDefault) != hipSuccess) { (void)hipGetLastError(); return nullptr; }
+    return p;
+}
+static void stage_host_free(void *p) { (void)hipHostFree(p); }
+
+static int qa_prepare(dbg *h) {
+    if (!h->qa_made) {
+        for (int i = 0; i < QA_EVENTS; ++i) HIPCHK(h, hipEventCreate(&h->qa_ev[i]));
+        h->stage.alloc = stage_host_alloc;
+        h->stage.release = stage_host_free;
+        h->qa_made = true;
+    }
+    h->stage.reset();
+    return DBG_OK;
+}
+static void qa_destroy(dbg *h) {
+    if (!h->qa_made) return;
+    for (int i = 0; i < QA_EVENTS; ++i) (void)hipEventDestroy(h->qa_ev[i]);
+    h->stage.destroy();
+    h->qa_made = false;
+}
+static int qa_mark(dbg *h, QaEvent e) {
+    HIPCHK(h, hipEventRecord(h->qa_ev[e], h->stream));
+    return DBG_OK;
+}
+static double qa_ms(dbg *h, QaEvent a, QaEvent b) {
+    float ms = 0;
+    if (hipEventElapsedTime(&ms, h->qa_ev[a], h->qa_ev[b]) != hipSuccess) { (void)hipGetLastError(); return 0.0; }
+    return ms;
+}
+template <class T>
+static int stage_take(dbg *h, T **p, uint64_t count) {
+    *p = (T *)h->stage.take((size_t)(count * sizeof(T)));
+    if (!*p) { h->err = "hipHostMalloc: the build's pinned staging block"; return DBG_E_NOMEM; }
+    return DBG_OK;
+}
+static int build_wait(dbg *h) {
+    ++h->build_waits;
+    HIPCHK(h, hipStreamSynchronize(h->stream));
+    return DBG_OK;
+}
+static int linear_table(dbg *h, dbg::Buf &buf, LinearTableKey &key, uint64_t stride, uint64_t len, const uint64_t **out) {
+    if (!key.serves(stride, len, buf.p) || buf.bytes < len * 8) {
+        key.clear();
+        CHK(buf_ensure(h, buf, len * 8));
+        uint64_t *stg = nullptr;
+        CHK(stage_take(h, &stg, len));
+        for (uint64_t i = 0; i < len; ++i) stg[i] = i * stride;
+        HIPCHK(h, hipMemcpyAsync(buf.p, stg, len * 8, hipMemcpyHostToDevice, h->stream));
+        key.set(stride, len, buf.p);
+    }
+    *out = (const uint64_t *)buf.p;
+    return DBG_OK;
+}
+static int lds_limit(dbg *h, const void *kernel, size_t bytes) {
+    for (const auto &e : h->lds_attr)
+        if (e.first == kernel && e.second >= (int)bytes) return DBG_OK;
+    HIPCHK(h, hipFuncSetAttribute(kernel, hipFuncAttributeMaxDynamicSharedMemorySize, (int)bytes));
+    h->lds_attr.emplace_back(kernel, (int)bytes);
+    return DBG_OK;
+}
+static int cu_count(dbg *h) {
+    if (!h->n_cu) {
+        int n = 0;
+        if (hipDeviceGetAttribute(&n, hipDeviceAttributeMultiprocessorCount, h->device) != hipSuccess || n <= 0) { (void)hipGetLastError(); n = 256; }
+        h->n_cu = n;
+    }
+    return h->n_cu;
+}
+
 constexpr int SCAN_ITEMS = 16;
 constexpr int SCAN_TILE = 256 * SCAN_ITEMS;
 
+struct ScanGuard {
+    const unsigned long long *status;
+    unsigned long long fail;
+    __device__ bool stops() const { return status && (*status & fail); }
+};
+
 template <class F>
-__global__ __launch_bounds__(256) void k_scan_reduce(uint64_t n, F f, uint64_t *partial) {
+__global__ __launch_bounds__(256) void k_scan_reduce(uint64_t n, F f, uint64_t *partial, ScanGuard G = ScanGuard{nullptr, 0}) {
+    if (G.stops()) return;
     uint64_t base = (uint64_t)blockIdx.x * SCAN_TILE + (uint64_t)threadIdx.x * SCAN_ITEMS;
     uint64_t s = 0;
 #pragma unroll
@@ -316,7 +418,8 @@
     if (threadIdx.x == 0) partial[blockIdx.x] = tot;
 }
 
-__global__ __launch_bounds__(256) void k_scan_partials(uint64_t *partial, uint64_t nblk, uint64_t *total) {
+__global__ __launch_bounds__(256) void k_scan_partials(uint64_t *partial, uint64_t nblk, uint64_t *total, ScanGuard G = ScanGuard{nullptr, 0}) {
+    if (G.stops()) return;
     uint64_t carry = 0;
     for (uint64_t base = 0; base < nblk; base += 256) {
         uint64_t i = base + threadIdx.x;
@@ -330,7 +433,8 @@
 }
 
 template <class F, class OutT>
-__global__ __launch_bounds__(256) void k_scan_write(uint64_t n, F f, const uint64_t *partial, OutT *out) {
+__global__ __launch_bounds__(256) void k_scan_write(uint64_t n, F f, const uint64_t *partial, OutT *out, ScanGuard G = ScanGuard{nullptr, 0}) {
+    if (G.stops()) return;
     uint64_t base = (uint64_t)blockIdx.x * SCAN_TILE + (uint64_t)threadIdx.x * SCAN_ITEMS;
     uint64_t v[SCAN_ITEMS];
     uint64_t s = 0;
@@ -349,17 +453,20 @@
 }
 
 template <class F, class OutT>
-static int exclusive_scan(dbg *h, uint64_t n, F f, OutT *out, uint64_t *h_total) {
+static int exclusive_scan(dbg *h, uint64_t n, F f, OutT *out, uint64_t *h_total, ScanGuard G = ScanGuard{nullptr, 0},
+                          const uint64_t **d_total_out = nullptr) {
     uint64_t nblk = (n + SCAN_TILE - 1) / SCAN_TILE;
     if (nblk == 0) nblk = 1;
     CHK(buf_ensure(h, h->ar_scan, (nblk + 1) * 8));
     uint64_t *partial = (uint64_t *)h->ar_scan.p;
     uint64_t *d_total = partial + nblk;
-    hipLaunchKernelGGL(HIP_KERNEL_NAME(k_scan_reduce<F>), dim3((unsigned)nblk), dim3(256), 0, h->stream, n, f, partial);
-    hipLaunchKernelGGL(k_scan_partials, dim3(1), dim3(256), 0, h->stream, partial, nblk, d_total);
+    hipLaunchKernelGGL(HIP_KERNEL_NAME(k_scan_reduce<F>), dim3((unsigned)nblk), dim3(256), 0, h->stream, n, f, partial, G);
+    hipLaunchKernelGGL(k_scan_partials, dim3(1), dim3(256), 0, h->stream, partial, nblk, d_total, G);
     hipLaunchKernelGGL(HIP_KERNEL_NAME(k_scan_write<F, OutT>), dim3((unsigned)nblk), dim3(256), 0, h->stream, n, f,
-                       partial, out);
+                       partial, out, G);
+    if (d_total_out) *d_total_out = d_total;
     if (!h_total) return DBG_OK;
+    ++h->build_waits;
     hipError_t e = hipMemcpyAsync(h_total, d_total, 8, hipMemcpyDeviceToHost, h->stream);
     if (e == hipSuccess) e = hipStreamSynchronize(h->stream);
     if (e != hipSuccess) {
@@ -1534,9 +1641,12 @@
     for (auto &b : h->ar_tips) buf_free(h, b);
     for (auto &lvl : h->ar_part) for (auto &b : lvl) buf_free(h, b);
     buf_free(h, h->ar_scan);
+    buf_free(h, h->tab_iota);
+    buf_free(h, h->tab_segstart);
     dev_free(h->d_scalars);
     delete (ShardState *)h->shard_state;
     (void)hipStreamSynchronize(h->stream);
+    qa_destroy(h);
     if (!h->borrowed_stream) (void)hipStreamDestroy(h->stream);
     delete h;
 }
@@ -2304,6 +2414,7 @@
     if (n == "resolve_sorted" && value >= 0 && value <= 2) { h->resolve_sorted = (int)value; return DBG_OK; }
     if (n == "resolve_direct" && (value == 0 || value == 1)) { h->resolve_direct = (int)value; return DBG_OK; }
     if (n == "resolve_count" && (value == 0 || value == 1)) { h->resolve_count = (int)value; return DBG_OK; }
+    if (n == "build_queue_ahead" && (value == 0 || value == 1)) { h->build_queue_ahead = (int)value; return DBG_OK; }
     if (n == "wcount_kernel" && (value == 1 || value == 2)) { h->wcount_kernel = (int)value; return DBG_OK; }
     if (n == "count_kernel_u64" && value >= 1 && value <= 3) { h->count_kernel_u64 = (int)value; return DBG_OK; }
     if (n == "lookup_index" && (value == 0 || value == 1)) { h->lookup_index = (int)value; return DBG_OK; }
@@ -2413,6 +2524,23 @@
     return rc;
 }
 
+struct BuildClock {
+    dbg *h;
+    std::unique_ptr<Timer> t;
+    bool ok = true;
+    BuildClock(dbg *h_, bool queue_ahead) : h(h_) {
+        if (queue_ahead) {
+            ok = qa_prepare(h) == DBG_OK && qa_mark(h, EV_TOTAL_A) == DBG_OK;
+            h->qa_on = ok;
+        } else {
+            t.reset(new Timer(h->stream, &h->build_waits));
+        }
+    }
+    void stop() {
+        if (t) h->stats.ms_build_total = t->stop();
+    }
+};
+
 extern "C" int dbg_build(dbg_t *h, int k, uint64_t table_capacity_hint) {
     if (!h) return DBG_E_ARG;
     if (k < 1 || k > 63) { h->err = "k must be in 1..63 (k-mers of at most two 64-bit words)"; return DBG_E_ARG; }
@@ -2427,8 +2555,12 @@
     const bool tentative = !h->alpha_known && h->engine == 0 && h->n_bytes > 0;
     if (tentative) h->is_dna = true;
     else CHK(compute_alphabet(h));
+    h->build_waits = 0;
+    const bool queue_ahead = h->build_queue_ahead && k <= 31 && h->engine == 0 && !h->resolve_sorted && !h->phase_limit;
+    struct QaScope { dbg *h; ~QaScope() { h->qa_on = false; } } qa_scope{h};
     if (tentative) {
-        Timer t_total(h->stream);
+        BuildClock t_total(h, queue_ahead);
+        if (!t_total.ok) return DBG_E_HIP;
         int rc;
         bool lds_engine = true;
         if (k > 31) {
@@ -2451,11 +2583,12 @@
             h->alpha_known = true;
             h->is_dna = true;
             h->dir_valid = lds_engine;
-            h->stats.ms_build_total = t_total.stop();
+            t_total.stop();
             if (k <= 31) pool_trim(h);
             return DBG_OK;
         }
         if (rc != DBG_E_ALPHABET) { const std::string keep = h->err; free_build(h); h->err = keep; return rc; }
+        h->qa_on = false;
         free_build(h);
         h->k = k;
         h->stats = dbg_stats_t{};
@@ -2489,12 +2622,13 @@
         return DBG_OK;
     }
     if (h->engine == 0) {
-        Timer t_total(h->stream);
+        BuildClock t_total(h, queue_ahead);
+        if (!t_total.ok) return DBG_E_HIP;
         int rc = build_sk(h, k, table_capacity_hint);
         if (rc == DBG_OK) rc = finish_graph(h);
         if (rc != DBG_OK) { const std::string keep = h->err; free_build(h); h->err = keep; return rc; }
         h->dir_valid = true;
-        h->stats.ms_build_total = t_total.stop();
+        t_total.stop();
         pool_trim(h);
         return DBG_OK;
     }
@@ -3200,6 +3334,8 @@
     if (n == "pull_crowded") { *out = h->pull_crowded; return DBG_OK; }
     if (n == "resolve_direct_hits") { *out = h->resolve_direct_hits; return DBG_OK; }
     if (n == "resolve_keyed") { *out = h->resolve_keyed; return DBG_OK; }
+    if (n == "build_host_waits") { *out = h->build_waits; return DBG_OK; }
+    if (n == "build_speculation_discards") { *out = h->spec_discards; return DBG_OK; }
     if (n == "lookup_index_builds") { *out = h->lookup_index_builds; return DBG_OK; }
     if (n == "lookup_dir_calls") { *out = h->lookup_dir_calls; return DBG_OK; }
     if (n == "lookup_index_calls") { *out = h->lookup_index_calls; return DBG_OK; }
@@ -3640,25 +3776,36 @@
                             uint64_t *out_w0, uint64_t *out_w1, ST *out_st, int shift, int nb, uint64_t *c_start,
                             uint64_t *c_cnt, dbg::Buf &b_scpre, dbg::Buf &b_cmat, dbg::Buf &b_offs, int fbits = 0,
                             const uint64_t *seg_add = nullptr, unsigned long long *d_sums = nullptr,
-                            const uint64_t *host_cnt = nullptr, const uint32_t *ready_cmat = nullptr) {
+                            const uint64_t *host_cnt = nullptr, const uint32_t *ready_cmat = nullptr,
+                            const MsGuard *spec = nullptr) {
     CHK(buf_ensure(h, b_scpre, (uint64_t)(n_seg + 1) * 8));
-    uint64_t *sc_pre = (uint64_t *)b_scpre.p;
+    const uint64_t *sc_pre = (const uint64_t *)b_scpre.p;
     uint64_t nsc = 0;
-    if (ready_cmat) {
+    const ScanGuard sg{spec ? spec->status : nullptr, spec ? spec->fail : 0};
+    const MsGuard mg = spec ? *spec : MsGuard{nullptr, 0, 0};
+    if (ready_cmat && h->qa_on) {
+        CHK(linear_table(h, h->tab_iota, h->key_iota, 1, (uint64_t)n_seg + 1, &sc_pre));
+        nsc = n_seg;
+    } else if (!host_cnt && h->qa_on) {
+        const uint64_t *d_nsc = nullptr;
+        CHK(exclusive_scan(h, n_seg, CeilDiv{p_cnt, (uint64_t)MS_SC}, (uint64_t *)b_scpre.p, (uint64_t *)nullptr, sg, &d_nsc));
+        HIPCHK(h, hipMemcpyAsync((uint64_t *)b_scpre.p + n_seg, d_nsc, 8, hipMemcpyDeviceToDevice, h->stream));
+        nsc = (uint64_t)n_seg + total / MS_SC;
+    } else if (ready_cmat) {
         std::vector<uint64_t> &pre = h->host_scpre;
         pre.resize((size_t)n_seg + 1);
         for (uint32_t i = 0; i <= n_seg; ++i) pre[i] = i;
         nsc = n_seg;
-        HIPCHK(h, hipMemcpyAsync(sc_pre, pre.data(), pre.size() * 8, hipMemcpyHostToDevice, h->stream));
+        HIPCHK(h, hipMemcpyAsync(b_scpre.p, pre.data(), pre.size() * 8, hipMemcpyHostToDevice, h->stream));
     } else if (host_cnt) {
         std::vector<uint64_t> &pre = h->host_scpre;
         pre.resize((size_t)n_seg + 1);
         for (uint32_t i = 0; i < n_seg; ++i) { pre[i] = nsc; nsc += (host_cnt[i] + MS_SC - 1) / MS_SC; }
         pre[n_seg] = nsc;
-        HIPCHK(h, hipMemcpyAsync(sc_pre, pre.data(), pre.size() * 8, hipMemcpyHostToDevice, h->stream));
+        HIPCHK(h, hipMemcpyAsync(b_scpre.p, pre.data(), pre.size() * 8, hipMemcpyHostToDevice, h->stream));
     } else {
-        CHK(exclusive_scan(h, n_seg, CeilDiv{p_cnt, (uint64_t)MS_SC}, sc_pre, &nsc));
-        HIPCHK(h, hipMemcpyAsync(sc_pre + n_seg, &nsc, 8, hipMemcpyHostToDevice, h->stream));
+        CHK(exclusive_scan(h, n_seg, CeilDiv{p_cnt, (uint64_t)MS_SC}, (uint64_t *)b_scpre.p, &nsc));
+        HIPCHK(h, hipMemcpyAsync((uint64_t *)b_scpre.p + n_seg, &nsc, 8, hipMemcpyHostToDevice, h->stream));
     }
     MsParents P{p_start, p_cnt, sc_pre, n_seg, spg};
     const uint64_t n_log = nsc * (uint64_t)nb;
@@ -3666,6 +3813,7 @@
     CHK(buf_ensure(h, b_offs, n_log * 8));
     const uint32_t *cmat = ready_cmat ? ready_cmat : (const uint32_t *)b_cmat.p;
     uint64_t *offs = (uint64_t *)b_offs.p;
+    const uint64_t *d_total = nullptr;
     if (nsc) {
         if (ready_cmat)
             ;
@@ -3676,17 +3824,18 @@
             hipLaunchKernelGGL(HIP_KERNEL_NAME(k_ms_hist<false>), dim3((unsigned)nsc), dim3(256), 0, h->stream, P, in_w1, shift, nb,
                                fbits, (uint32_t *)b_cmat.p, (unsigned long long *)nullptr);
         HIPCHK(h, hipGetLastError());
-        CHK(exclusive_scan(h, n_log, MsLogical{P, cmat, nb}, offs, (uint64_t *)nullptr));
-    }
+        CHK(exclusive_scan(h, n_log, MsLogical{P, cmat, nb}, offs, (uint64_t *)nullptr, sg, spec ? &d_total : nullptr));
+    }
+    if (spec && !d_total) { h->err = "internal: a multisplit level queued on a guess has nothing to scan"; return DBG_E_ARG; }
     const uint64_t n_child = (uint64_t)(n_seg / spg) * nb;
     hipLaunchKernelGGL(k_ms_children, dim3(grid_for(n_child, 256)), dim3(256), 0, h->stream, P, offs, nb, total, c_start,
-                       c_cnt);
+                       c_cnt, d_total, mg);
     if (nsc) {
         auto kern = k_ms_scatter<ST, HAS_ST, STI, STHI>;
         const size_t lds = sizeof(MsLds<ST>);
-        HIPCHK(h, hipFuncSetAttribute((const void *)kern, hipFuncAttributeMaxDynamicSharedMemorySize, (int)lds));
+        CHK(lds_limit(h, (const void *)kern, lds));
         hipLaunchKernelGGL(kern, dim3((unsigned)nsc), dim3(MS_NT), lds, h->stream, P, in_w0, in_w1, in_st, seg_add, shift, nb,
-                           fbits, offs, out_w0, out_w1, out_st);
+                           fbits, offs, out_w0, out_w1, out_st, mg);
     }
     HIPCHK(h, hipGetLastError());
     return DBG_OK;
@@ -3714,7 +3863,47 @@
     uint32_t n_wg = 0;
     int l1 = 0;
     const uint32_t *cmat = nullptr;
+    bool spec_l1 = false;
+    bool spec_est = false;
+    uint64_t est[2] = {0, 0};
+    uint64_t est_set_cap = 0;
 };
+
+static uint64_t sk_estimate_set_cap(uint64_t n_inst, double own, int nb1) {
+    const uint64_t inst_bucket = (uint64_t)((double)n_inst * own / nb1) * 2 + 1024;
+    uint64_t set_cap = 1024;
+    while (set_cap < inst_bucket * 2) set_cap <<= 1;
+    return set_cap;
+}
+
+template <class ST>
+static int sk_extract_speculate(dbg *h, int k, ExtractSplit *xs, const uint64_t *seg_start, const uint64_t *seg_cnt, uint32_t n_seg,
+                                uint64_t seg_cap, uint64_t *w0[2], uint64_t *w1[2], ST *st[2]) {
+    const int l1 = xs->l1, nb1 = 1 << l1, top = 6 + SK_BUCKET_BITS;
+    unsigned long long *sc_dev = (unsigned long long *)h->d_scalars;
+    const MsGuard guard{sc_dev, STATUS_BAD_BASE | STATUS_SEGMENT_FULL, seg_cap};
+    CHK(qa_mark(h, EV_PART_A));
+    CHK(buf_ensure(h, h->ar_misc[MISC_L1_CHILDREN], (uint64_t)nb1 * 16));
+    uint64_t *c1_start = (uint64_t *)h->ar_misc[MISC_L1_CHILDREN].p, *c1_cnt = c1_start + nb1;
+    CHK((multisplit_level<ST, true>(h, seg_start, seg_cnt, n_seg, xs->n_wg, 0, w0[0], w1[0], st[0], w0[1], w1[1], st[1], top - l1,
+                                    nb1 >> xs->f0, c1_start, c1_cnt, h->ar_misc[MISC_MS_SCPRE], h->ar_misc[MISC_MS_CMAT],
+                                    h->ar_misc[MISC_MS_OFFS], 0, nullptr, nullptr, nullptr, xs->cmat, &guard)));
+    xs->spec_l1 = true;
+    if (h->bucket_bits == 0 && l1 >= 9) {
+        const uint64_t cut = h->n_reads * (uint64_t)(k - 1);
+        xs->est_set_cap = sk_estimate_set_cap(h->n_bytes > cut ? h->n_bytes - cut : 0, 1.0, nb1);
+        CHK(buf_ensure(h, h->ar_misc[MISC_ESTIMATE_SET], xs->est_set_cap * 8));
+        unsigned long long *set = (unsigned long long *)h->ar_misc[MISC_ESTIMATE_SET].p;
+        HIPCHK(h, hipMemsetAsync(set, 0xFF, xs->est_set_cap * 8, h->stream));
+        const MsGuard eg{guard.status, guard.fail, seg_cap * (uint64_t)n_seg};
+        hipLaunchKernelGGL(HIP_KERNEL_NAME(k_estimate_distinct<ST>), dim3(512), dim3(256), 0, h->stream, (const uint64_t *)c1_start,
+                           (const uint64_t *)c1_cnt, 0u, (const uint64_t *)w0[1], (const uint64_t *)w1[1], k, set,
+                           xs->est_set_cap - 1, sc_dev + SC_ESTIMATE, eg);
+        HIPCHK(h, hipGetLastError());
+        xs->spec_est = true;
+    }
+    return DBG_OK;
+}
 
 template <class ST>
 static int sk_extract(dbg *h, int k, uint64_t *w0[2], uint64_t *w1[2], ST *st[2], uint64_t **seg_start_out,
@@ -3740,8 +3929,7 @@
         const uint64_t F0 = 1ull << f0;
         const double per_tile = (w == 1 ? 1.0 : density) * TILE * PS_SLACK / (double)F0;
         const uint64_t tpw_max = std::max<uint64_t>(1, (uint64_t)((double)(MS_SC - 64) / per_tile));
-        int n_cu = 0;
-        HIPCHK(h, hipDeviceGetAttribute(&n_cu, hipDeviceAttributeMultiprocessorCount, h->device));
+        const int n_cu = cu_count(h);
         n_wg = (uint32_t)std::max<uint64_t>(std::min<uint64_t>(tiles, (uint64_t)n_cu * DBG_PS_WG_PER_CU), (tiles + tpw_max - 1) / tpw_max);
         tiles_per_wg = (tiles + n_wg - 1) / n_wg;
         seg_cap = std::min<uint64_t>(MS_SC, (uint64_t)((double)tiles_per_wg * per_tile) + 64);
@@ -3755,11 +3943,16 @@
     uint64_t *seg_start = nullptr, *seg_cnt = nullptr, *seg_nk = nullptr, *seg_ne = nullptr;
     uint32_t *ps_cmat = nullptr;
     uint64_t n_rec = 0;
-    Timer t(h->stream);
+    const bool qa = h->qa_on && xs && n_parts == 1;
+    uint64_t *rb = nullptr;
+    bool speculated = false;
+    std::unique_ptr<Timer> t;
+    if (qa) { CHK(stage_take(h, &rb, SC_ESTIMATE + 2)); CHK(qa_mark(h, EV_EXTRACT_A)); }
+    else t.reset(new Timer(h->stream, &h->build_waits));
     for (int attempt = 0; attempt < 3; ++attempt) {
         CHK(buf_ensure(h, h->ar_misc[MISC_SEGMENTS], (n_seg * 2 + (uint64_t)n_wg * 2) * 8));
         seg_start = (uint64_t *)h->ar_misc[MISC_SEGMENTS].p; seg_cnt = seg_start + n_seg; seg_nk = seg_cnt + n_seg; seg_ne = seg_nk + n_wg;
-        hseg.assign((size_t)(n_seg * 2 + (uint64_t)n_wg * 2), 0);
+        if (!qa) hseg.assign((size_t)(n_seg * 2 + (uint64_t)n_wg * 2), 0);
         if (f0 && ps_l1) {
             CHK(buf_ensure(h, h->ar_misc[MISC_MS_CMAT], n_seg * 4 << (ps_l1 - f0)));
             ps_cmat = (uint32_t *)h->ar_misc[MISC_MS_CMAT].p;
@@ -3773,8 +3966,14 @@
             w1[set] = (uint64_t *)h->ar_rec[set][1].p;
             st[set] = (ST *)h->ar_rec[set][2].p;
         }
-        for (uint64_t g = 0; g < n_seg; ++g) hseg[g] = g * seg_cap;
-        HIPCHK(h, hipMemcpyAsync(seg_start, hseg.data(), (size_t)n_seg * 8, hipMemcpyHostToDevice, h->stream));
+        if (qa) {
+            const uint64_t *tab = nullptr;
+            CHK(linear_table(h, h->tab_segstart, h->key_segstart, seg_cap, n_seg, &tab));
+            seg_start = const_cast<uint64_t *>(tab);
+        } else {
+            for (uint64_t g = 0; g < n_seg; ++g) hseg[g] = g * seg_cap;
+            HIPCHK(h, hipMemcpyAsync(seg_start, hseg.data(), (size_t)n_seg * 8, hipMemcpyHostToDevice, h->stream));
+        }
         HIPCHK(h, hipMemsetAsync(seg_cnt, 0, (size_t)(n_seg + (uint64_t)n_wg * 2) * 8, h->stream));
         HIPCHK(h, hipMemsetAsync(h->d_scalars, 0, 64 * 8, h->stream));
         if (tiles) {
@@ -3802,10 +4001,32 @@
                                    seg_ne, sc_dev, tile_first);
             HIPCHK(h, hipGetLastError());
         }
-        HIPCHK(h, hipMemcpyAsync(sc, h->d_scalars, 8, hipMemcpyDeviceToHost, h->stream));
-        HIPCHK(h, hipMemcpyAsync(hseg.data() + n_seg, seg_cnt, (size_t)(n_seg + (uint64_t)n_wg * 2) * 8, hipMemcpyDeviceToHost,
-                                 h->stream));
-        HIPCHK(h, hipStreamSynchronize(h->stream));
+        if (qa) {
+            hipLaunchKernelGGL(k_seg_totals, dim3(grid_for(std::min<uint64_t>(n_seg, 8192), 256)), dim3(256), 0, h->stream, seg_cnt, (uint32_t)n_seg, seg_nk, seg_ne, n_wg,
+                               sc_dev + SC_EXTRACT_TOTALS);
+            HIPCHK(h, hipGetLastError());
+            CHK(qa_mark(h, EV_EXTRACT_B));
+            xs->spec_l1 = xs->spec_est = false;
+            speculated = false;
+            if (attempt == 0 && f0 && ps_l1) {
+                xs->f0 = f0; xs->n_wg = n_wg; xs->l1 = ps_l1; xs->cmat = ps_cmat;
+                CHK((sk_extract_speculate<ST>(h, k, xs, seg_start, seg_cnt, (uint32_t)n_seg, seg_cap, w0, w1, st)));
+                speculated = true;
+            }
+            HIPCHK(h, hipMemcpyAsync(rb, h->d_scalars, (SC_ESTIMATE + 2) * 8, hipMemcpyDeviceToHost, h->stream));
+            CHK(build_wait(h));
+            sc[0] = rb[0];
+        } else {
+            HIPCHK(h, hipMemcpyAsync(sc, h->d_scalars, 8, hipMemcpyDeviceToHost, h->stream));
+            HIPCHK(h, hipMemcpyAsync(hseg.data() + n_seg, seg_cnt, (size_t)(n_seg + (uint64_t)n_wg * 2) * 8, hipMemcpyDeviceToHost,
+                                     h->stream));
+            ++h->build_waits;
+            HIPCHK(h, hipStreamSynchronize(h->stream));
+        }
+        if (speculated && (sc[0] & (STATUS_BAD_BASE | STATUS_SEGMENT_FULL))) {
+            xs->spec_l1 = xs->spec_est = false;
+            ++h->spec_discards;
+        }
         if (sc[0] & STATUS_BAD_BASE) { h->err = "reads hold a byte outside ACGT"; return DBG_E_ALPHABET; }
         if (!(sc[0] & STATUS_SEGMENT_FULL)) break;
         if (f0) {
@@ -3820,14 +4041,22 @@
         seg_cap = tiles_per_wg * TILE;
     }
     h->n_kmer_inst = h->n_edge_inst = 0;
-    for (uint64_t g = 0; g < n_seg; ++g) n_rec += hseg[n_seg + g];
-    for (uint32_t g = 0; g < n_wg; ++g) {
-        h->n_kmer_inst += hseg[2 * n_seg + g];
-        h->n_edge_inst += hseg[2 * n_seg + n_wg + g];
-    }
-    h->stats.ms_extract = t.stop();
+    if (qa) {
+        n_rec = rb[SC_EXTRACT_TOTALS];
+        h->n_kmer_inst = rb[SC_EXTRACT_TOTALS + 1];
+        h->n_edge_inst = rb[SC_EXTRACT_TOTALS + 2];
+        if (xs->spec_est) { xs->est[0] = rb[SC_ESTIMATE]; xs->est[1] = rb[SC_ESTIMATE + 1]; }
+        h->host_seg_cnt.clear();
+    } else {
+        for (uint64_t g = 0; g < n_seg; ++g) n_rec += hseg[n_seg + g];
+        for (uint32_t g = 0; g < n_wg; ++g) {
+            h->n_kmer_inst += hseg[2 * n_seg + g];
+            h->n_edge_inst += hseg[2 * n_seg + n_wg + g];
+        }
+        h->stats.ms_extract = t->stop();
+        h->host_seg_cnt.assign(hseg.begin() + n_seg, hseg.begin() + 2 * (size_t)n_seg);
+    }
     h->stats.n_records = n_rec;
-    h->host_seg_cnt.assign(hseg.begin() + n_seg, hseg.begin() + 2 * (size_t)n_seg);
     if (xs) { xs->f0 = f0; xs->n_wg = n_wg; xs->l1 = ps_l1; xs->cmat = ps_l1 ? ps_cmat : nullptr; }
     *seg_start_out = seg_start;
     *seg_cnt_out = seg_cnt;
@@ -3882,7 +4111,15 @@
     int where = 0;
     double est_distinct = 0.0;
     const int top = 6 + SK_BUCKET_BITS;
-    Timer t_part(h->stream);
+    const bool qa = h->qa_on && xs && !pre;
+    bool spec_l1 = qa && xs->spec_l1;
+    if (spec_l1 && xs->l1 != l1) {
+        spec_l1 = false;
+        ++h->spec_discards;
+    }
+    std::unique_ptr<Timer> t_part;
+    if (!qa) t_part.reset(new Timer(h->stream, &h->build_waits));
+    else if (!spec_l1) CHK(qa_mark(h, EV_PART_A));
     const int bps = pre ? nb1 >> shard_bits : 0;
     const uint64_t b_lo = pre ? (uint64_t)my_shard * bps : 0;
     uint64_t *ps_start = nullptr, *ps_cnt = nullptr, *ps_add = nullptr;
@@ -3905,6 +4142,8 @@
         ps_start = (uint64_t *)h->ar_misc[MISC_SEGMENTS].p; ps_cnt = ps_start + ps_n; ps_add = ps_cnt + ps_n;
         HIPCHK(h, hipMemcpyAsync(ps_start, hs.data(), hs.size() * 8, hipMemcpyHostToDevice, h->stream));
         HIPCHK(h, hipStreamSynchronize(h->stream));
+    } else if (spec_l1) {
+        where = 1;
     } else {
         if (xs && xs->f0 && l1 >= xs->f0) {
             if (xs->l1 != l1) ++h->presplit_rehists;
@@ -3919,22 +4158,25 @@
     }
     if (auto_T && l1 >= 9 && n_rec) {
         const uint32_t probe_bucket = (pp.probe_first_owned && shard_bits) ? (uint32_t)my_shard << (l1 - shard_bits) : 0u;
-        const uint64_t inst_bucket = (uint64_t)((double)n_inst * own / nb1) * 2 + 1024;
-        uint64_t set_cap = 1024;
-        while (set_cap < inst_bucket * 2) set_cap <<= 1;
-        CHK(buf_ensure(h, h->ar_misc[MISC_ESTIMATE_SET], set_cap * 8));
-        unsigned long long *set = (unsigned long long *)h->ar_misc[MISC_ESTIMATE_SET].p;
-        unsigned long long *d_est = (unsigned long long *)(h->d_scalars + SC_ESTIMATE);
-        HIPCHK(h, hipMemsetAsync(set, 0xFF, set_cap * 8, h->stream));
-        HIPCHK(h, hipMemsetAsync(d_est, 0, 16, h->stream));
-        if (pre) {
-            for (int r = 0; r < pre->n_senders; ++r) pp.estimate(128u, ps_start, ps_cnt, (uint32_t)r, in_w0, in_w1, set, set_cap - 1, d_est);
+        const uint64_t set_cap = sk_estimate_set_cap(n_inst, own, nb1);
+        uint64_t est[2] = {0, 0};
+        if (spec_l1 && xs->spec_est && xs->est_set_cap >= set_cap) {
+            est[0] = xs->est[0];
+            est[1] = xs->est[1];
         } else {
-            pp.estimate(512u, c1_start, c1_cnt, probe_bucket, w0[1], w1[1], set, set_cap - 1, d_est);
-        }
-        uint64_t est[2] = {0, 0};
-        HIPCHK(h, hipMemcpyAsync(est, d_est, 16, hipMemcpyDeviceToHost, h->stream));
-        HIPCHK(h, hipStreamSynchronize(h->stream));
+            CHK(buf_ensure(h, h->ar_misc[MISC_ESTIMATE_SET], set_cap * 8));
+            unsigned long long *set = (unsigned long long *)h->ar_misc[MISC_ESTIMATE_SET].p;
+            unsigned long long *d_est = (unsigned long long *)(h->d_scalars + SC_ESTIMATE);
+            HIPCHK(h, hipMemsetAsync(set, 0xFF, set_cap * 8, h->stream));
+            HIPCHK(h, hipMemsetAsync(d_est, 0, 16, h->stream));
+            if (pre) {
+                for (int r = 0; r < pre->n_senders; ++r) pp.estimate(128u, ps_start, ps_cnt, (uint32_t)r, in_w0, in_w1, set, set_cap - 1, d_est);
+            } else {
+                pp.estimate(512u, c1_start, c1_cnt, probe_bucket, w0[1], w1[1], set, set_cap - 1, d_est);
+            }
+            HIPCHK(h, hipMemcpyAsync(est, d_est, 16, hipMemcpyDeviceToHost, h->stream));
+            CHK(build_wait(h));
+        }
         if (est[0]) {
             double distinct = (double)n_inst * own * (double)est[1] / (double)est[0];
             if (pre) {
@@ -4013,7 +4255,8 @@
         HIPCHK(h, hipMemcpyAsync(b_start, c1_start, (size_t)nb1 * 8, hipMemcpyDeviceToDevice, h->stream));
         HIPCHK(h, hipMemcpyAsync(b_cnt, c1_cnt, (size_t)nb1 * 8, hipMemcpyDeviceToDevice, h->stream));
     }
-    h->stats.ms_partition = t_part.stop();
+    if (qa) CHK(qa_mark(h, EV_PART_B));
+    else h->stats.ms_partition = t_part->stop();
     h->stats.n_buckets = n_buckets;
     *out = SkPartition{b_start, b_cnt, n_buckets, where, l1, l2 > 0 ? nb2 : 1, fb2, l2_pow, nb3, fb3, est_distinct, n_inst, n_edge_inst};
     return DBG_OK;
@@ -4095,6 +4338,10 @@
     bool use_count2 = CAP == 4096 && h->count_kernel >= 2 && !h->phase_limit && (sizeof(ST) == 4 || h->count_kernel_u64 >= 2);
     const bool use_count3 = use_count2 && ((sizeof(ST) == 8 && h->count_kernel_u64 == 3) || h->count_kernel == 3);
     int extra_attempts = 0;
+    const SkGeom geom{k, m, P.l1, P.nb2, P.fb2, P.l2_pow, P.nb3, P.fb3, shard_bits, my_shard, own_lo, own_cnt};
+    const bool qa = h->qa_on && xs && !pre && !shard_bits;
+    uint64_t *rbc = nullptr;
+    if (qa) CHK(stage_take(h, &rbc, 10));
     for (int attempt = 0; attempt < 3 + extra_attempts; ++attempt) {
         CHK(ensure_node_arrays());
         for (int set = 0; set < 2; ++set) {
@@ -4106,8 +4353,10 @@
             qc[set] = (uint32_t *)h->ar_q[set][2].p;
             if (!shard_bits && !h->resolve_sorted) break;
         }
-        Timer t(h->stream);
-        HIPCHK(h, hipMemsetAsync(h->d_scalars, 0, 64 * 8, h->stream));
+        std::unique_ptr<Timer> t;
+        if (qa) CHK(qa_mark(h, EV_COUNT_A));
+        else t.reset(new Timer(h->stream, &h->build_waits));
+        HIPCHK(h, hipMemsetAsync(h->d_scalars, 0, (qa ? 128 : 64) * 8, h->stream));
         HIPCHK(h, hipMemsetAsync(ranges, 0, n_buckets * sizeof(SkRange), h->stream));
         HIPCHK(h, hipMemsetAsync(dirs, 0, own_cnt * (CAP / 64) * sizeof(SkDirEnt), h->stream));
         SkCountOut out{h->d_keys, h->d_stamps_st, h->d_flags, node_cap, h->d_rowptr32, h->d_col, h->d_ecnt, edge_cap,
@@ -4118,24 +4367,28 @@
         if (use_count2 && n_rec) {
             auto kern2 = use_count3 ? k_sk_count3<ST> : k_sk_count2<ST>;
             const size_t lds2 = use_count3 ? sizeof(Cnt3Lds<ST>) : sizeof(Cnt2Lds<ST>);
-            HIPCHK(h, hipFuncSetAttribute((const void *)kern2, hipFuncAttributeMaxDynamicSharedMemorySize, (int)lds2));
-            int n_cu = 256;
-            (void)hipDeviceGetAttribute(&n_cu, hipDeviceAttributeMultiprocessorCount, h->device);
-            const unsigned grid = (unsigned)std::min<uint64_t>(n_buckets, (uint64_t)n_cu);
+            CHK(lds_limit(h, (const void *)kern2, lds2));
+            const unsigned grid = (unsigned)std::min<uint64_t>(n_buckets, (uint64_t)cu_count(h));
             SkCount2Args a2{out, b_start, b_cnt, w0[where], w1[where], (const void *)st[where], n_buckets, split_recs, k};
             SkCount2Args *d_a2 = (SkCount2Args *)(h->d_scalars + SC_DESCRIPTOR);
             static_assert(sizeof(SkCount2Args) <= (SK2_QUERY_CURSOR - SC_DESCRIPTOR) * 8, "the query cursor sits behind the descriptor");
-            HIPCHK(h, hipMemcpyAsync(d_a2, &a2, sizeof(a2), hipMemcpyHostToDevice, h->stream));
-            HIPCHK(h, hipMemsetAsync(h->d_scalars + SK2_QUERY_CURSOR, 0, 8, h->stream));
+            const SkCount2Args *src2 = &a2;
+            if (qa) {
+                SkCount2Args *stg = nullptr;
+                CHK(stage_take(h, &stg, 1));
+                *stg = a2;
+                src2 = stg;
+            }
+            HIPCHK(h, hipMemcpyAsync(d_a2, src2, sizeof(a2), hipMemcpyHostToDevice, h->stream));
+            if (!qa) HIPCHK(h, hipMemsetAsync(h->d_scalars + SK2_QUERY_CURSOR, 0, 8, h->stream));
             hipLaunchKernelGGL(kern2, dim3(grid), dim3(Cnt2Cfg<ST>::NT), lds2, h->stream, (const SkCount2Args *)d_a2);
             HIPCHK(h, hipGetLastError());
         }
         auto kern = k_sk_count<ST, CAP>;
         const size_t lds = sizeof(CntLds<ST, CAP>);
-        HIPCHK(h, hipFuncSetAttribute((const void *)kern, hipFuncAttributeMaxDynamicSharedMemorySize, (int)lds));
         if (n_rec && !use_count2) {
-            int n_cu = 256;
-            (void)hipDeviceGetAttribute(&n_cu, hipDeviceAttributeMultiprocessorCount, h->device);
+            CHK(lds_limit(h, (const void *)kern, lds));
+            const int n_cu = cu_count(h);
             constexpr int NT = CntCfg<ST, CAP>::NT;
             const uint64_t per_cu = std::max<uint64_t>(1, std::min<uint64_t>(2048 / NT, (160 * 1024) / lds));
             const unsigned grid = (unsigned)std::min<uint64_t>(n_buckets, (uint64_t)n_cu * per_cu);
@@ -4147,11 +4400,20 @@
             HIPCHK(h, hipGetLastError());
         }
         h->stats.count_launches = n_rec ? (uint64_t)(attempt + 1) : 0;
-        HIPCHK(h, hipMemcpyAsync(sc, h->d_scalars, 64, hipMemcpyDeviceToHost, h->stream));
-        uint64_t q2 = 0;
-        if (use_count2 && n_rec) HIPCHK(h, hipMemcpyAsync(&q2, h->d_scalars + SK2_QUERY_CURSOR, 8, hipMemcpyDeviceToHost, h->stream));
-        h->stats.ms_count = t.stop();
-        if (use_count2 && n_rec) sc[5] = q2;
+        if (qa) {
+            CHK(qa_mark(h, EV_COUNT_B));
+            HIPCHK(h, hipMemcpyAsync(rbc, h->d_scalars, 8 * 8, hipMemcpyDeviceToHost, h->stream));
+            HIPCHK(h, hipMemcpyAsync(rbc + 8, h->d_scalars + SK2_QUERY_CURSOR, 8, hipMemcpyDeviceToHost, h->stream));
+            CHK(build_wait(h));
+            memcpy(sc, rbc, sizeof(sc));
+            if (use_count2 && n_rec) sc[5] = rbc[8];
+        } else {
+            HIPCHK(h, hipMemcpyAsync(sc, h->d_scalars, 64, hipMemcpyDeviceToHost, h->stream));
+            uint64_t q2 = 0;
+            if (use_count2 && n_rec) HIPCHK(h, hipMemcpyAsync(&q2, h->d_scalars + SK2_QUERY_CURSOR, 8, hipMemcpyDeviceToHost, h->stream));
+            h->stats.ms_count = t->stop();
+            if (use_count2 && n_rec) sc[5] = q2;
+        }
         if (h->phase_limit) { h->err = "ablation run (phase_limit set): timing only"; return DBG_E_ARG; }
         if (sc[0] & (STATUS_BUCKET_TOO_BIG | STATUS_RANGE_CAP)) break;
         bool again = false;
@@ -4183,10 +4445,11 @@
     uint64_t n_q = sc[5];
     const uint64_t n_ranges = n_buckets + sc[6];
     h->stats.n_queries = n_q;
-    SkGeom geom{k, m, P.l1, P.nb2, P.fb2, P.l2_pow, P.nb3, P.fb3, shard_bits, my_shard, own_lo, own_cnt};
 
     {
-        Timer t(h->stream);
+        std::unique_ptr<Timer> t;
+        if (qa) CHK(qa_mark(h, EV_SUCC_A));
+        else t.reset(new Timer(h->stream, &h->build_waits));
         uint64_t root[2] = {0, n_q};
         int qset = 0;
         if (shard_bits && n_q) {
@@ -4242,12 +4505,28 @@
                                qk[qset] + root[0], qc[qset] + root[0], n_q, geom, ranges, n_buckets, n_ranges, dirs, h->d_keys,
                                h->n_nodes, h->d_col, id_tag, sc_dev, q_meta, sc_dev + SC_RESOLVE_COUNTS);
             HIPCHK(h, hipGetLastError());
-            HIPCHK(h, hipMemcpyAsync(sc, h->d_scalars, 8, hipMemcpyDeviceToHost, h->stream));
+            if (!qa) {
+                HIPCHK(h, hipMemcpyAsync(sc, h->d_scalars, 8, hipMemcpyDeviceToHost, h->stream));
+                CHK(resolve_counts_in(h));
+                CHK(build_wait(h));
+                if (sc[0] & STATUS_SUCC_MISSING) { h->err = "internal: a successor k-mer was not found in its bucket"; return DBG_E_HIP; }
+            }
+        }
+        if (qa) {
+            CHK(qa_mark(h, EV_SUCC_B));
+            CHK(qa_mark(h, EV_TOTAL_B));
+            HIPCHK(h, hipMemcpyAsync(rbc + 9, h->d_scalars, 8, hipMemcpyDeviceToHost, h->stream));
             CHK(resolve_counts_in(h));
-            HIPCHK(h, hipStreamSynchronize(h->stream));
-            if (sc[0] & STATUS_SUCC_MISSING) { h->err = "internal: a successor k-mer was not found in its bucket"; return DBG_E_HIP; }
-        }
-        h->stats.ms_succ = t.stop();
+            CHK(build_wait(h));
+            if (n_q && (rbc[9] & STATUS_SUCC_MISSING)) { h->err = "internal: a successor k-mer was not found in its bucket"; return DBG_E_HIP; }
+            h->stats.ms_extract = qa_ms(h, EV_EXTRACT_A, EV_EXTRACT_B);
+            h->stats.ms_partition = qa_ms(h, EV_PART_A, EV_PART_B);
+            h->stats.ms_count = qa_ms(h, EV_COUNT_A, EV_COUNT_B);
+            h->stats.ms_succ = qa_ms(h, EV_SUCC_A, EV_SUCC_B);
+            h->stats.ms_build_total = qa_ms(h, EV_TOTAL_A, EV_TOTAL_B);
+        } else {
+            h->stats.ms_succ = t->stop();
+        }
     }
     int T = 0;
     while ((1ull << T) < n_buckets) ++T;
@@ -4577,7 +4856,7 @@
     ExtractSplit xs;
     xs.target = SK_TARGET_DISTINCT<CAP>;
     CHK(sk_extract<ST>(h, k, w0, w1, st, &seg_start, &seg_cnt, &n_seg, &n_rec, 0, 1, &xs));
-    return sk_count_from_segments<ST, CAP>(h, k, seg_start, seg_cnt, n_seg, h->host_seg_cnt.data(), n_rec, h->n_kmer_inst, h->n_edge_inst, w0[0],
+    return sk_count_from_segments<ST, CAP>(h, k, seg_start, seg_cnt, n_seg, h->qa_on ? nullptr : h->host_seg_cnt.data(), n_rec, h->n_kmer_inst, h->n_edge_inst, w0[0],
                                            w1[0], st[0], w0, w1, st, node_capacity_hint, 0, 0, nullptr, &xs);
 }
 
diff --git a/py-debruijn_amd/csrc/dbg_sk.h b/py-debruijn_amd/csrc/dbg_sk.h
--- a/py-debruijn_amd/csrc/dbg_sk.h
+++ b/py-debruijn_amd/csrc/dbg_sk.h
@@ -403,6 +403,7 @@
 __global__ __launch_bounds__(256) void k_ms_hist(MsParents P, const uint64_t *__restrict__ w1, int shift, int nb, int fbits,
                                                  uint32_t *cmat, unsigned long long *sums) {
     __shared__ uint32_t hist[MS_MAX_NB];
+    if (blockIdx.x >= P.sc_pre[P.n_seg]) return;
     uint32_t seg;
     uint64_t sidx;
     ms_locate(P, blockIdx.x, &seg, &sidx);
@@ -433,6 +434,7 @@
     const uint32_t *cmat;
     int nb;
     __device__ uint64_t operator()(uint64_t L) const {
+        if (L >= (uint64_t)nb * P.sc_pre[P.n_seg]) return 0;
         const uint32_t n_groups = P.n_seg / P.spg;
         uint32_t lo = 0, hi = n_groups;
         while (hi - lo > 1) {
@@ -447,8 +449,18 @@
     }
 };
 
+struct MsGuard {
+    const unsigned long long *status;
+    unsigned long long fail;
+    uint64_t seg_cap;
+};
+__device__ inline bool ms_guard_stops(const MsGuard &G) { return G.status && (*G.status & G.fail); }
+
 __global__ __launch_bounds__(256) void k_ms_children(MsParents P, const uint64_t *__restrict__ offs, int nb,
-                                                     uint64_t total, uint64_t *c_start, uint64_t *c_cnt) {
+                                                     uint64_t total, uint64_t *c_start, uint64_t *c_cnt,
+                                                     const uint64_t *total_dev = nullptr, MsGuard G = MsGuard{nullptr, 0, 0}) {
+    if (ms_guard_stops(G)) return;
+    if (total_dev) total = *total_dev;
     const uint64_t i = (uint64_t)blockIdx.x * blockDim.x + threadIdx.x;
     const uint32_t n_groups = P.n_seg / P.spg;
     const uint64_t n_child = (uint64_t)n_groups * nb;
@@ -487,9 +499,12 @@
                                                     const uint64_t *__restrict__ in_w1, const STI *__restrict__ in_st,
                                                     const uint64_t *__restrict__ seg_add,
                                                     int shift, int nb, int fbits, const uint64_t *__restrict__ offs,
-                                                    uint64_t *out_w0, uint64_t *out_w1, ST *out_st) {
+                                                    uint64_t *out_w0, uint64_t *out_w1, ST *out_st,
+                                                    MsGuard G = MsGuard{nullptr, 0, 0}) {
     extern __shared__ __attribute__((aligned(16))) unsigned char ms_raw[];
     MsLds<ST> &s = *reinterpret_cast<MsLds<ST> *>(ms_raw);
+    if (ms_guard_stops(G)) return;
+    if (blockIdx.x >= P.sc_pre[P.n_seg]) return;
     constexpr int CH = MsChunk<ST>::CH;
     static_assert(CH % MS_NT == 0 && sizeof(MsLds<ST>) <= 160 * 1024, "multisplit chunk");
 #ifdef DBG_MS_PROF
@@ -506,7 +521,8 @@
     const uint64_t lbase = (uint64_t)nb * g_lo;
     for (int b = threadIdx.x; b < nb; b += MS_NT) s.run[b] = offs[lbase + (uint64_t)b * nsc + gidx];
     const uint64_t beg = P.start[seg] + sidx * MS_SC;
-    const uint64_t end = min(P.start[seg] + P.cnt[seg], beg + (uint64_t)MS_SC);
+    const uint64_t seg_n = G.status ? min(P.cnt[seg], G.seg_cap) : P.cnt[seg];
+    const uint64_t end = min(P.start[seg] + seg_n, beg + (uint64_t)MS_SC);
     for (uint64_t c0 = beg; c0 < end; c0 += CH) {
         const int n = (int)min((uint64_t)CH, end - c0);
         for (int b = threadIdx.x; b < nb; b += MS_NT) s.hist[b] = 0;
@@ -589,8 +605,11 @@
                                                            const uint64_t *__restrict__ rec_w0,
                                                            const uint64_t *__restrict__ rec_w1, int k,
                                                            unsigned long long *set, uint64_t set_mask,
-                                                           unsigned long long *out ) {
-    const uint64_t beg = b_start[bucket], n = b_cnt[bucket];
+                                                           unsigned long long *out ,
+                                                           MsGuard G = MsGuard{nullptr, 0, 0}) {
+    if (ms_guard_stops(G)) return;
+    const uint64_t beg = b_start[bucket];
+    const uint64_t n = G.status ? min(b_cnt[bucket], G.seg_cap > beg ? G.seg_cap - beg : 0) : b_cnt[bucket];
     uint64_t inst = 0, fresh = 0;
     for (uint64_t r = (uint64_t)blockIdx.x * blockDim.x + threadIdx.x; r < n; r += (uint64_t)gridDim.x * blockDim.x) {
         const uint64_t w0 = rec_w0[beg + r], w1 = rec_w1[beg + r];
@@ -616,6 +635,23 @@
     if ((threadIdx.x & 63) == 0) {
         if (inst) atomicAdd(&out[0], (unsigned long long)inst);
         if (fresh) atomicAdd(&out[1], (unsigned long long)fresh);
+    }
+}
+
+__global__ __launch_bounds__(256) void k_seg_totals(const uint64_t *__restrict__ seg_cnt, uint32_t n_seg,
+                                                    const uint64_t *__restrict__ seg_nk, const uint64_t *__restrict__ seg_ne,
+                                                    uint32_t n_wg, unsigned long long *out) {
+    const uint32_t first = blockIdx.x * 256 + threadIdx.x, stride = gridDim.x * 256;
+    uint64_t a = 0, b = 0, c = 0;
+    for (uint32_t i = first; i < n_seg; i += stride) a += seg_cnt[i];
+    for (uint32_t i = first; i < n_wg; i += stride) { b += seg_nk[i]; c += seg_ne[i]; }
+    a = wave_sum_u64(a);
+    b = wave_sum_u64(b);
+    c = wave_sum_u64(c);
+    if ((threadIdx.x & 63) == 0) {
+        if (a) atomicAdd(&out[0], (unsigned long long)a);
+        if (b) atomicAdd(&out[1], (unsigned long long)b);
+        if (c) atomicAdd(&out[2], (unsigned long long)c);
     }
 }
 
diff --git a/py-debruijn_amd/csrc/dbg_sk2.h b/py-debruijn_amd/csrc/dbg_sk2.h
--- a/py-debruijn_amd/csrc/dbg_sk2.h
+++ b/py-debruijn_amd/csrc/dbg_sk2.h
@@ -43,6 +43,7 @@
     static constexpr int PEND = sizeof(ST) == 8 ? 2048 : 4096;
 };
 
+constexpr int SC_EXTRACT_TOTALS = 8;
 constexpr int SC_ESTIMATE = 40;
 constexpr int SC_RESOLVE_COUNTS = 48;
 constexpr int SC_L2_SUMS = 56;
diff --git a/py-debruijn_amd/csrc/dbg_stage.h b/py-debruijn_amd/csrc/dbg_stage.h
--- /dev/null
+++ b/py-debruijn_amd/csrc/dbg_stage.h
@@ -0,0 +1,67 @@
+#pragma once
+#include <cstddef>
+#include <cstdint>
+#include <vector>
+
+namespace dbgk {
+
+struct StageBlock {
+    typedef void *(*alloc_fn)(size_t bytes);
+    typedef void (*free_fn)(void *p);
+    static constexpr size_t ALIGN = 64;
+    static constexpr size_t MIN_BYTES = 1 << 16;
+
+    alloc_fn alloc = nullptr;
+    free_fn release = nullptr;
+    unsigned char *base = nullptr;
+    size_t cap = 0, used = 0;
+    std::vector<void *> retired;
+    uint64_t grows = 0;
+
+    static size_t grown(size_t cap_now, size_t used_now, size_t want) {
+        size_t need = used_now + want, c = cap_now ? cap_now : MIN_BYTES;
+        while (c < need) c *= 2;
+        return c;
+    }
+    static size_t round_up(size_t n) { return (n + ALIGN - 1) / ALIGN * ALIGN; }
+
+    void *take(size_t bytes) {
+        const size_t want = round_up(bytes ? bytes : 1);
+        if (used + want > cap) {
+            const size_t c = grown(cap, 0, want);
+            void *p = alloc ? alloc(c) : nullptr;
+            if (!p) return nullptr;
+            if (base) retired.push_back(base);
+            base = (unsigned char *)p;
+            cap = c;
+            used = 0;
+            ++grows;
+        }
+        void *out = base + used;
+        used += want;
+        return out;
+    }
+    void reset() {
+        for (void *p : retired) release(p);
+        retired.clear();
+        used = 0;
+    }
+    void destroy() {
+        reset();
+        if (base) release(base);
+        base = nullptr;
+        cap = 0;
+    }
+};
+
+struct LinearTableKey {
+    uint64_t stride = 0, len = 0;
+    const void *where = nullptr;
+    bool serves(uint64_t want_stride, uint64_t want_len, const void *buffer) const {
+        return where != nullptr && where == buffer && stride == want_stride && len >= want_len;
+    }
+    void set(uint64_t s, uint64_t n, const void *buffer) { stride = s; len = n; where = buffer; }
+    void clear() { stride = 0; len = 0; where = nullptr; }
+};
+
+}
```

After: 59.88 billion k-mers/s (median of 6 runs). Within noise of the previous version (+1.4%).
